# NVlabs/InstantSplat

Measured on AMD Instinct MI355X. Metric: train_iters_per_sec, higher is better.
Workload: dtype f32

## Files before the change

### include/mi355gs.h

```cpp
#ifndef MI355GS_H
#define MI355GS_H

#include <stddef.h>
#include <stdint.h>

#ifdef __cplusplus
extern "C" {
#endif

#define MI355GS_ABI_VERSION 10

#define MI355GS_OK 0
#define MI355GS_EINVAL (-1)
#define MI355GS_ELAUNCH (-2)
#define MI355GS_EOVERFLOW (-3)

int mi355gs_abi_version(void);
const char* mi355gs_error_string(int code);

size_t mi355gs_raster_geom_bytes(int P);
size_t mi355gs_raster_tiles_bytes(int W, int H);
size_t mi355gs_raster_binning_bytes(int64_t num_instances, int W, int H);

int mi355gs_raster_forward_preprocess(
    void* stream, int P, int D, int M, int W, int H,
    const float* means3D, const float* shs, const float* shs_rest, const float* colors_precomp, const float* opacities,
    const float* scales, float scale_modifier, const float* rotations, const float* cov3D_precomp,
    const float* viewmatrix, const float* projmatrix, const float* campos,
    float tanfovx, float tanfovy, int prefiltered,
    int32_t* radii, void* geom, void* tiles, int32_t* num_rendered, uint8_t* visible, void* grad_scratch, int debug);

int mi355gs_raster_forward_render(
    void* stream, int P, int W, int H, int64_t capacity, const float* bg,
    const void* geom, void* tiles, void* binning, float* out_color, int debug);

size_t mi355gs_raster_binning_bytes_render_only(int64_t num_instances, int W, int H);
int mi355gs_raster_forward_render_only(
    void* stream, int P, int W, int H, int64_t capacity, const float* bg,
    const void* geom, void* tiles, void* binning, float* out_color, int debug);

size_t mi355gs_raster_grad_scratch_bytes(int P);
size_t mi355gs_raster_grad_gate_offset(int P);
int mi355gs_raster_backward(
    void* stream, int P, int D, int M, int W, int H, const float* bg,
    const float* means3D, const float* shs, const float* shs_rest, const float* colors_precomp, const float* opacities,
    const float* scales, float scale_modifier, const float* rotations, const float* cov3D_precomp,
    const float* viewmatrix, const float* projmatrix, const float* campos,
    float tanfovx, float tanfovy,
    const void* geom, void* tiles, const void* binning, int64_t capacity, const int32_t* radii,
    const float* out_color, const float* dL_dpix, void* grad_scratch,
    float* dL_dmeans3D, float* dL_dmeans2D, float* dL_dshs, float* dL_dshs_rest, float* dL_dcolors, float* dL_dopacities,
    float* dL_dscales, float* dL_drotations, float* dL_dcov3D, int grad_scratch_is_clear, int debug);

int mi355gs_raster_mark_visible(void* stream, int P, const float* means3D, const float* viewmatrix,
                                const float* projmatrix, uint8_t* present);

int mi355gs_raster_frame_stats(void* stream, int W, int H, const void* tiles, int64_t* stats);

int mi355gs_tune_min_units(int min_units);

int mi355gs_tune_deterministic(int on);

int mi355gs_tune_scale_grad(int mode);

int mi355gs_profile_begin(void);
int mi355gs_profile_set_period(int every);
int mi355gs_profile_work_counters(void* counters);
int mi355gs_profile_read(int kind, double* total_ms, int* launches);
int mi355gs_profile_end(void);
int mi355gs_profile_ranges(int on);

size_t mi355gs_ssim_scratch_bytes(int B, int C, int H, int W);
int mi355gs_ssim_forward(void* stream, int B, int C, int H, int W, const float* img1, const float* img2,
                         float* dm_dmu1, float* dm_dsigma1_sq, float* dm_dsigma12,
                         void* scratch, float* ssim_mean, float* l1_mean, int padding_valid);
int mi355gs_ssim_backward(void* stream, int B, int C, int H, int W, const float* img1, const float* img2,
                          const float* dm_dmu1, const float* dm_dsigma1_sq, const float* dm_dsigma12,
                          const float* ssim_grad_scale, const float* l1_grad_scale, float* dL_dimg1, int padding_valid);
int mi355gs_l1_ssim_loss_fused(void* stream, int B, int C, int H, int W, const float* img1, const float* img2, void* scratch,
                               float lambda_dssim, float* ssim_mean, float* l1_mean, float* loss, float* dloss_dimg1);

size_t mi355gs_l1_scratch_bytes(int64_t n);
int mi355gs_l1_loss_forward(void* stream, int64_t n, const float* a, const float* b, void* scratch, float* mean_out);
int mi355gs_l1_loss_backward(void* stream, int64_t n, const float* a, const float* b, const float* grad_scale, float* d_a);
#define MI355GS_LOSS_PROGRAM_MAX 16
#define MI355GS_LOSS_OP_L1 0
#define MI355GS_LOSS_OP_SSIM 1
#define MI355GS_LOSS_OP_MULK 2
#define MI355GS_LOSS_OP_ADDK 3
#define MI355GS_LOSS_OP_RSUBK 4
#define MI355GS_LOSS_OP_DIVK 5
#define MI355GS_LOSS_OP_NEG 6
#define MI355GS_LOSS_OP_ADD 7
#define MI355GS_LOSS_OP_SUB 8
int mi355gs_l1_ssim_pair_forward(void* stream, int B, int C, int H, int W, const float* img1, const float* img2, void* scratch,
                                 float* dssim_dimg1);
int mi355gs_l1_ssim_pair_backward(void* stream, int64_t n, const float* img1, const float* img2, const float* dssim_dimg1,
                                  const float* g_l1, float c_l1, const float* g_ssim, float c_ssim, float* d_img1);
int mi355gs_loss_program_eval(void* stream, int n_ops, const int32_t* ops, const float* consts, int B, int C, int H, int W,
                              const void* scratch, float* ssim_mean, float* l1_mean, float* out, float* host_out, float ticket);
int mi355gs_loss_program_eval_grad(void* stream, int n_ops, const int32_t* ops, const float* consts, int B, int C, int H, int W,
                                   const void* scratch, float* ssim_mean, float* l1_mean, float* out, float* host_out, float ticket,
                                   const float* img1, const float* img2, const float* dssim_dimg1, float c_l1, float c_ssim, float* d_img1);

size_t mi355gs_knn_scratch_bytes(int N);
int mi355gs_knn_dist2(void* stream, int N, const float* points, float* mean_dist2, void* scratch);

int mi355gs_adam_step(void* stream, int64_t n, int row, float* param, const float* grad, float* exp_avg,
                      float* exp_avg_sq, const float* per_point_lr, const float* grad_sumsq,
                      float lr, float beta1, float beta2, float eps, int step);

int mi355gs_adam_multi_step(void* stream, int ntensors, const int64_t* numel, const int32_t* row, float* const* params,
                            const float* const* grads, float* const* exp_avg, float* const* exp_avg_sq,
                            const float* const* per_point_lr, const float* lr, float beta1, float beta2, float eps,
                            const int32_t* step, float* scratch, const float* gate, const int32_t* gate_index,
                            uint32_t* live, uint32_t seq);

int mi355gs_pose_forward(void* stream, int P, const float* xyz, const float* rot, const float* scaling,
                         const float* opacity_logit, const float* pose, float* means_cam, float* rot_cam, float* scales,
                         float* opac);
int mi355gs_pose_backward(void* stream, int P, const float* xyz, const float* rot, const float* scales, const float* opac,
                          const float* pose, const float* g_means, const float* g_rot, const float* g_scales,
                          const float* g_opac, float* d_xyz, float* d_rot, float* d_scaling, float* d_opacity_logit,
                          float* d_pose, float* scratch);

int mi355gs_posed_forward_preprocess(void* stream, int P, int D, int W, int H, const float* xyz, const float* f_dc,
                                     const float* f_rest, const float* opacity_logit, const float* log_scales, float scale_modifier,
                                     const float* rotation, const float* pose, const float* view_identity, const float* projmatrix,
                                     const float* origin, float tanfovx, float tanfovy, int32_t* radii, void* geom, void* tiles,
                                     int32_t* num_rendered, uint8_t* visible, void* grad_scratch, int debug);
int mi355gs_posed_backward(void* stream, int P, int D, int W, int H, const float* bg, const float* xyz, const float* f_dc,
                           const float* f_rest, const float* opacity_logit, const float* log_scales, float scale_modifier,
                           const float* rotation, const float* pose, const float* view_identity, const float* projmatrix,
                           const float* origin, float tanfovx, float tanfovy, const void* geom, void* tiles, const void* binning,
                           int64_t capacity, const int32_t* radii, const float* out_color, const float* dL_dpix,
                           void* grad_scratch, float* pose_scratch, float* d_xyz, float* d_means2D, float* d_f_dc, float* d_f_rest,
                           float* d_opacity_logit, float* d_log_scales, float* d_rotation, float* d_pose, int pose_rows, int pose_row,
                           int grad_scratch_is_clear, int debug);

size_t mi355gs_trainer_workspace_bytes(int P, int W, int H, int V, int64_t capacity);
void* mi355gs_trainer_create(int P, int W, int H, int V, int64_t capacity, float* xyz, float* f_dc, float* f_rest, float* opacity,
                             float* scaling, float* rotation, float* poses, float* const* exp_avg, float* const* exp_avg_sq,
                             const float* per_point_lr, void* workspace);
int mi355gs_trainer_step(void* trainer, void* stream, int view, int sh_degree, const float* gt_image, const float* projmatrix,
                         float tanfovx, float tanfovy, const float* bg, const float* lr, const int32_t* step, float beta1, float beta2, float eps,
                         float lambda_dssim, int do_optimizer_step, float* loss_out, int32_t* num_rendered_out);
int mi355gs_trainer_optimizer_step(void* trainer, void* stream, const float* lr, const int32_t* step, float beta1, float beta2,
                                   float eps, int commit_gate);
void mi355gs_trainer_destroy(void* trainer);
const float* mi355gs_trainer_grad(void* trainer, int k);

#define MI355GS_TRACKER_STATE_FLOATS 40
#define MI355GS_TRACKER_POSE 0
#define MI355GS_TRACKER_EXP_AVG 8
#define MI355GS_TRACKER_EXP_AVG_SQ 16
#define MI355GS_TRACKER_BEST 24
#define MI355GS_TRACKER_INITIAL 25
#define MI355GS_TRACKER_FLAG 26
#define MI355GS_TRACKER_COUNT 27
#define MI355GS_TRACKER_CAND 32
size_t mi355gs_tracker_workspace_bytes(int P, int W, int H, int64_t capacity);
void* mi355gs_tracker_create(int P, int M, int W, int H, int64_t capacity, const float* xyz, const float* f_dc, const float* f_rest,
                             const float* opacity, const float* scaling, const float* rotation, void* workspace);
int mi355gs_tracker_count(void* tracker, void* stream, int sh_degree, const float* projmatrix, float tanfovx, float tanfovy,
                          const float* pose, int32_t* count_out);
int mi355gs_tracker_run(void* tracker, void* stream, int sh_degree, const float* gt_image, const float* projmatrix, float tanfovx,
                        float tanfovy, const float* bg, const float* sched, int num_iter, int first_iter, int n_iters, float* state,
                        float* pose_trace, float* loss_trace, float* grad_trace);
void mi355gs_tracker_destroy(void* tracker);

int mi355gs_rgb8_from_planar(void* stream, int H, int W, const float* img, uint8_t* out);
size_t mi355gs_path_workspace_bytes(int P, int W, int H, int64_t capacity);
void* mi355gs_path_create(int P, int M, int W, int H, int64_t capacity, const float* xyz, const float* f_dc, const float* f_rest,
                          const float* opacity, const float* scaling, const float* rotation, void* workspace);
int mi355gs_path_render(void* path, void* stream, int sh_degree, const float* projmatrix, float tanfovx, float tanfovy,
                        const float* bg, const float* poses, int first, int n, uint8_t* frames, int32_t* counts);
void mi355gs_path_destroy(void* path);

size_t mi355gs_metrics_rgb8_scratch_bytes(int N, int H, int W);
int mi355gs_metrics_rgb8(void* stream, int N, int H, int W, const uint8_t* a, const uint8_t* b, void* scratch, int64_t* sq_sum,
                         float* ssim_mean);

size_t mi355gs_lpips_vgg_scratch_bytes(int N, int H, int W, const int channels[5]);
int mi355gs_lpips_vgg_rgb8(void* stream, int N, int H, int W, const uint8_t* a, const uint8_t* b, const int channels[5],
                           const float* weights, void* scratch, float* lpips, float* taps);

typedef struct mi355gs_vit_config {
  int enc_dim, enc_depth, enc_heads;
  int dec_dim, dec_depth, dec_heads;
  int patch;
  int hooks[4];
} mi355gs_vit_config;
size_t mi355gs_vit_encode_scratch_bytes(const mi355gs_vit_config* cfg, int Ht, int Wt, int V);
int mi355gs_vit_encode(void* stream, const mi355gs_vit_config* cfg, const float* weights, const float* rope, int Ht, int Wt, int V,
                       const float* images, void* scratch, float* feat);
size_t mi355gs_vit_decode_scratch_bytes(const mi355gs_vit_config* cfg, int Ht, int Wt, int E);
int mi355gs_vit_decode(void* stream, const mi355gs_vit_config* cfg, const float* weights, const float* rope, int Ht, int Wt, int V, int E,
                       const int32_t* edges, const float* feat, void* scratch, float* const out1[4], float* const out2[4]);

typedef struct mi355gs_dpt_config {
  int dim_tokens[4];
  int layer_dims[4];
  int feature_dim, last_dim;
  int mlp_hidden, local_feat_dim, two_confs;
  float conf_vmin, conf_vmax;
  float desc_conf_vmin, desc_conf_vmax;
} mi355gs_dpt_config;
size_t mi355gs_dpt_head_scratch_bytes(const mi355gs_dpt_config* cfg, int Ht, int Wt, int E);
size_t mi355gs_dpt_head_tap_offset(const mi355gs_dpt_config* cfg, int Ht, int Wt, int E, int which);
int mi355gs_dpt_head(void* stream, const mi355gs_dpt_config* cfg, const float* weights, int Ht, int Wt, int E, const float* const hooks[4],
                     void* scratch, float* pts3d, float* conf, float* raw4);
size_t mi355gs_local_features_scratch_bytes(const mi355gs_dpt_config* cfg, int Ht, int Wt, int E);
int mi355gs_local_features(void* stream, const mi355gs_dpt_config* cfg, const float* weights, int Ht, int Wt, int E, const float* hook0,
                           const float* hook3, void* scratch, float* desc, float* desc_conf);

size_t mi355gs_png_rgb8_scratch_bytes(int N, int H, int W, int rows_per_block);
size_t mi355gs_png_rgb8_stream_bytes(int N, int H, int W, int rows_per_block);
int mi355gs_png_rgb8(void* stream, int N, int H, int W, int rows_per_block, const uint8_t* frames, void* scratch, uint8_t* out,
                     int64_t* offsets);

size_t mi355gs_jpeg_rgb8_scratch_bytes(int N, int H, int W, int subsampling);
size_t mi355gs_jpeg_rgb8_stream_bytes(int N, int H, int W, int subsampling);
int mi355gs_jpeg_rgb8(void* stream, int N, int H, int W, int subsampling, const uint8_t* qtables, const uint8_t* frames, void* scratch,
                      uint8_t* out, size_t out_bytes, int64_t* offsets);

size_t mi355gs_pointmap_stats_scratch_bytes(int V, int H, int W);
int mi355gs_pointmap_stats(void* stream, int V, int H, int W, const float* depthmaps, const float* confidences, uint8_t* overlap,
                           void* scratch, double* stats);
int mi355gs_covis_masks(void* stream, int V, int H, int W, const int32_t* order, const float* pointmaps, const float* depthmaps,
                        const float* intrinsics, const float* w2c, const double* stats, float depth_threshold, uint8_t* overlap);
size_t mi355gs_compact_scratch_bytes(int64_t n);
int mi355gs_compact_pointmaps(void* stream, int64_t n, const uint8_t* overlap, const float* pointmaps, const float* images,
                              const float* confidences, void* scratch, float* out_points, uint8_t* out_rgb8, float* out_confidence,
                              int32_t* count_dev, int32_t* count_host);

#define MI355GS_ALIGN_OPT_DEPTH 1
#define MI355GS_ALIGN_OPT_IM_POSES 2
#define MI355GS_ALIGN_OPT_FOCALS 4
#define MI355GS_ALIGN_OPT_PW_POSES 8
#define MI355GS_ALIGN_NORM_PW_SCALE 16
size_t mi355gs_align_workspace_bytes(int V, int H, int W, int E, int flags);
void* mi355gs_align_create(void* workspace, int V, int H, int W, const int32_t* edges, int E, int flags, float base_scale);
void mi355gs_align_destroy(void* handle);
int mi355gs_align_pack(void* handle, void* stream, const float* pred_i, const float* pred_j, const float* conf_i, const float* conf_j);
int mi355gs_align_grad(void* handle, void* stream, const float* depth_log, const float* im_pose, const float* focal_log, const float* pp_raw,
                       const float* pw_pose, float* g_depth_log, float* g_im_pose, float* g_focal_log, float* g_pw_pose, float* loss);
int mi355gs_align_run(void* handle, void* stream, int niter, const float* step_table, float* depth_log, float* im_pose, float* focal_log,
                      const float* pp_raw, float* pw_pose, float* m_depth_log, float* v_depth_log, float* m_im_pose, float* v_im_pose,
                      float* m_focal_log, float* v_focal_log, float* m_pw_pose, float* v_pw_pose, float* losses);
int mi355gs_align_points(void* handle, void* stream, const float* depth_log, const float* im_pose, const float* focal_log,
                         const float* pp_raw, const float* pw_pose, float* pts3d, float* depth);
const float* mi355gs_align_records(void* handle);

size_t mi355gs_align_init_workspace_bytes(int B, int n);
int mi355gs_align_init_means(void* workspace, void* stream, int rows, int n, const float* x, float* means);
int mi355gs_align_init_register(void* workspace, void* stream, int B, int n, const float* src, const int32_t* src_idx, long long src_job_stride,
                                int src_pt_stride, const float* tgt, const int32_t* tgt_idx, long long tgt_job_stride, const float* weights,
                                const int32_t* w_idx, long long w_job_stride, float* srt, float* pw_pose);
int mi355gs_align_init_apply(void* stream, int n, const float* src, int src_pt_stride, const float* srt, float* dst);
int mi355gs_align_init_focals(void* workspace, void* stream, int B, int H, int W, const float* src, const int32_t* src_idx,
                              long long src_job_stride, int src_pt_stride, float* focals);
int mi355gs_align_init_state(void* workspace, void* stream, int V, int E, int H, int W, int norm_pw_scale, float base_scale, int focal_mode,
                             float known_focal, const float* srt, const int32_t* pose_row, const float* focals, const int32_t* focal_row,
                             const float* pw_pose, float* pts3d, float* depth_log, float* im_pose, float* focal_log);

#define MI355GS_DENSITY_CLONE 1
#define MI355GS_DENSITY_SPLIT 2
#define MI355GS_DENSITY_PRUNE 4
#define MI355GS_DENSITY_SCREEN 8
#define MI355GS_DENSITY_XYZ 0
#define MI355GS_DENSITY_F_DC 1
#define MI355GS_DENSITY_F_REST 2
#define MI355GS_DENSITY_OPACITY 3
#define MI355GS_DENSITY_SCALING 4
#define MI355GS_DENSITY_ROTATION 5
#define MI355GS_DENSITY_EXP_AVG 6
#define MI355GS_DENSITY_EXP_AVG_SQ 12
#define MI355GS_DENSITY_PER_POINT_LR 18
#define MI355GS_DENSITY_GRAD_ACCUM 19
#define MI355GS_DENSITY_DENOM 20
#define MI355GS_DENSITY_MAX_RADII 21
#define MI355GS_DENSITY_TENSORS 22
int mi355gs_density_stats(void* stream, int P, const float* grad, int grad_stride, const uint8_t* filter, const int32_t* radii,
                          float* grad_accum, float* denom, float* max_radii);
size_t mi355gs_density_scratch_bytes(int P, int N);
int mi355gs_density_plan(void* stream, int P, int N, int flags, const float* grad_accum, const float* denom, const float* grads,
                         int64_t n_grads, const uint8_t* mask, const float* max_radii, const float* scaling, const float* opacity,
                         float max_grad, float dense_limit, float min_opacity, float max_screen_size, float world_limit,
                         float child_div, uint32_t* code, void* scratch, int32_t* totals_host);
int mi355gs_density_apply(void* stream, int P, int N, int flags, int rest_width, const uint32_t* code, const void* scratch,
                          const float* noise, int64_t noise_rows, int64_t n_selected, float child_div, const void* const* in,
                          void* const* out, int64_t out_rows);
int mi355gs_reset_opacity(void* stream, int P, float* opacity, float* exp_avg, float* exp_avg_sq);

size_t mi355gs_resample_rgb8_scratch_bytes(int N, int rows, int w);
int mi355gs_resample_rgb8(void* stream, int N, int H, int W, int Hout, int Wout, const uint8_t* images, const int32_t* kx,
                          const int32_t* bx, int ksize_x, const int32_t* ky, const int32_t* by, int ksize_y, int x0, int y0, int w,
                          int h, int row0, int rows, void* scratch, uint8_t* rgb8, float* unit, float* normalized);

#ifdef __cplusplus
}
#endif
#endif
```

### instantsplat_amd/_lib.py

```python
from __future__ import annotations

import ctypes
import os
from ctypes import c_float, c_int, c_int64, c_size_t, c_void_p

import torch

_HERE = os.path.dirname(os.path.abspath(__file__))
LIB_PATH = os.path.join(_HERE, "lib", "libmi355gs.so")
_LIB = None
_TEST_MODE = False

_P = c_void_p
_SIGNATURES = {
    "mi355gs_abi_version": (c_int, []),
    "mi355gs_error_string": (ctypes.c_char_p, [c_int]),
    "mi355gs_raster_geom_bytes": (c_size_t, [c_int]),
    "mi355gs_raster_tiles_bytes": (c_size_t, [c_int, c_int]),
    "mi355gs_raster_binning_bytes": (c_size_t, [c_int64, c_int, c_int]),
    "mi355gs_raster_grad_scratch_bytes": (c_size_t, [c_int]),
    "mi355gs_raster_grad_gate_offset": (c_size_t, [c_int]),
    "mi355gs_raster_forward_preprocess": (c_int, [_P, c_int, c_int, c_int, c_int, c_int, _P, _P, _P, _P, _P, _P, c_float, _P, _P,
                                                  _P, _P, _P, c_float, c_float, c_int, _P, _P, _P, _P, _P, _P, c_int]),
    "mi355gs_raster_forward_render": (c_int, [_P, c_int, c_int, c_int, c_int64, _P, _P, _P, _P, _P, c_int]),
    "mi355gs_raster_binning_bytes_render_only": (c_size_t, [c_int64, c_int, c_int]),
    "mi355gs_raster_forward_render_only": (c_int, [_P, c_int, c_int, c_int, c_int64, _P, _P, _P, _P, _P, c_int]),
    "mi355gs_raster_backward": (c_int, [_P, c_int, c_int, c_int, c_int, c_int, _P, _P, _P, _P, _P, _P, _P, c_float, _P, _P, _P, _P,
                                        _P, c_float, c_float, _P, _P, _P, c_int64, _P, _P, _P, _P, _P, _P, _P, _P, _P, _P, _P, _P, _P,
                                        c_int, c_int]),
    "mi355gs_raster_mark_visible": (c_int, [_P, c_int, _P, _P, _P, _P]),
    "mi355gs_raster_frame_stats": (c_int, [_P, c_int, c_int, _P, _P]),
    "mi355gs_tune_min_units": (c_int, [c_int]),
    "mi355gs_tune_scale_grad": (c_int, [c_int]),
    "mi355gs_tune_deterministic": (c_int, [c_int]),
    "mi355gs_profile_begin": (c_int, []),
    "mi355gs_profile_set_period": (c_int, [c_int]),
    "mi355gs_profile_work_counters": (c_int, [_P]),
    "mi355gs_profile_read": (c_int, [c_int, ctypes.POINTER(ctypes.c_double), ctypes.POINTER(c_int)]),
    "mi355gs_profile_end": (c_int, []),
    "mi355gs_profile_ranges": (c_int, [c_int]),
    "mi355gs_ssim_scratch_bytes": (c_size_t, [c_int, c_int, c_int, c_int]),
    "mi355gs_ssim_forward": (c_int, [_P, c_int, c_int, c_int, c_int, _P, _P, _P, _P, _P, _P, _P, _P, c_int]),
    "mi355gs_ssim_backward": (c_int, [_P, c_int, c_int, c_int, c_int, _P, _P, _P, _P, _P, _P, _P, _P, c_int]),
    "mi355gs_l1_ssim_loss_fused": (c_int, [_P, c_int, c_int, c_int, c_int, _P, _P, _P, c_float, _P, _P, _P, _P]),
    "mi355gs_l1_ssim_pair_forward": (c_int, [_P, c_int, c_int, c_int, c_int, _P, _P, _P, _P]),
    "mi355gs_l1_ssim_pair_backward": (c_int, [_P, c_int64, _P, _P, _P, _P, c_float, _P, c_float, _P]),
    "mi355gs_loss_program_eval": (c_int, [_P, c_int, _P, _P, c_int, c_int, c_int, c_int, _P, _P, _P, _P, _P, c_float]),
    "mi355gs_loss_program_eval_grad": (c_int, [_P, c_int, _P, _P, c_int, c_int, c_int, c_int, _P, _P, _P, _P, _P, c_float, _P, _P, _P, c_float,
                                               c_float, _P]),
    "mi355gs_knn_scratch_bytes": (c_size_t, [c_int]),
    "mi355gs_knn_dist2": (c_int, [_P, c_int, _P, _P, _P]),
    "mi355gs_adam_step": (c_int, [_P, c_int64, c_int, _P, _P, _P, _P, _P, _P, c_float, c_float, c_float, c_float, c_int]),
    "mi355gs_adam_multi_step": (c_int, [_P, c_int, _P, _P, _P, _P, _P, _P, _P, _P, c_float, c_float, c_float, _P, _P, _P, _P, _P,
                                        ctypes.c_uint32]),
    "mi355gs_pose_forward": (c_int, [_P, c_int, _P, _P, _P, _P, _P, _P, _P, _P, _P]),
    "mi355gs_pose_backward": (c_int, [_P, c_int, _P, _P, _P, _P, _P, _P, _P, _P, _P, _P, _P, _P, _P, _P, _P]),
    "mi355gs_posed_forward_preprocess": (c_int, [_P, c_int, c_int, c_int, c_int, _P, _P, _P, _P, _P, c_float, _P, _P, _P, _P, _P,
                                                 c_float, c_float, _P, _P, _P, _P, _P, _P, c_int]),
    "mi355gs_posed_backward": (c_int, [_P, c_int, c_int, c_int, c_int, _P, _P, _P, _P, _P, _P, c_float, _P, _P, _P, _P, _P, c_float,
                                       c_float, _P, _P, _P, c_int64, _P, _P, _P, _P, _P, _P, _P, _P, _P, _P, _P, _P, _P, c_int, c_int, c_int, c_int]),
    "mi355gs_l1_scratch_bytes": (c_size_t, [c_int64]),
    "mi355gs_l1_loss_forward": (c_int, [_P, c_int64, _P, _P, _P, _P]),
    "mi355gs_l1_loss_backward": (c_int, [_P, c_int64, _P, _P, _P, _P]),
    "mi355gs_trainer_workspace_bytes": (c_size_t, [c_int, c_int, c_int, c_int, c_int64]),
    "mi355gs_trainer_create": (c_void_p, [c_int, c_int, c_int, c_int, c_int64, _P, _P, _P, _P, _P, _P, _P, _P, _P, _P, _P]),
    "mi355gs_trainer_step": (c_int, [_P, _P, c_int, c_int, _P, _P, c_float, c_float, _P, _P, _P, c_float, c_float, c_float, c_float,
                                     c_int, _P, _P]),
    "mi355gs_trainer_optimizer_step": (c_int, [_P, _P, _P, _P, c_float, c_float, c_float, c_int]),
    "mi355gs_trainer_destroy": (None, [_P]),
    "mi355gs_trainer_grad": (_P, [_P, c_int]),
    "mi355gs_tracker_workspace_bytes": (c_size_t, [c_int, c_int, c_int, c_int64]),
    "mi355gs_tracker_create": (c_void_p, [c_int, c_int, c_int, c_int, c_int64, _P, _P, _P, _P, _P, _P, _P]),
    "mi355gs_tracker_count": (c_int, [_P, _P, c_int, _P, c_float, c_float, _P, _P]),
    "mi355gs_tracker_run": (c_int, [_P, _P, c_int, _P, _P, c_float, c_float, _P, _P, c_int, c_int, c_int, _P, _P, _P, _P]),
    "mi355gs_tracker_destroy": (None, [_P]),
    "mi355gs_rgb8_from_planar": (c_int, [_P, c_int, c_int, _P, _P]),
    "mi355gs_path_workspace_bytes": (c_size_t, [c_int, c_int, c_int, c_int64]),
    "mi355gs_path_create": (c_void_p, [c_int, c_int, c_int, c_int, c_int64, _P, _P, _P, _P, _P, _P, _P]),
    "mi355gs_path_render": (c_int, [_P, _P, c_int, _P, c_float, c_float, _P, _P, c_int, c_int, _P, _P]),
    "mi355gs_path_destroy": (None, [_P]),
    "mi355gs_metrics_rgb8_scratch_bytes": (c_size_t, [c_int, c_int, c_int]),
    "mi355gs_metrics_rgb8": (c_int, [_P, c_int, c_int, c_int, _P, _P, _P, _P, _P]),
    "mi355gs_png_rgb8_scratch_bytes": (c_size_t, [c_int, c_int, c_int, c_int]),
    "mi355gs_png_rgb8_stream_bytes": (c_size_t, [c_int, c_int, c_int, c_int]),
    "mi355gs_png_rgb8": (c_int, [_P, c_int, c_int, c_int, c_int, _P, _P, _P, _P]),
    "mi355gs_jpeg_rgb8_scratch_bytes": (c_size_t, [c_int, c_int, c_int, c_int]),
    "mi355gs_jpeg_rgb8_stream_bytes": (c_size_t, [c_int, c_int, c_int, c_int]),
    "mi355gs_jpeg_rgb8": (c_int, [_P, c_int, c_int, c_int, c_int, _P, _P, _P, _P, c_size_t, _P]),
    "mi355gs_lpips_vgg_scratch_bytes": (c_size_t, [c_int, c_int, c_int, _P]),
    "mi355gs_lpips_vgg_rgb8": (c_int, [_P, c_int, c_int, c_int, _P, _P, _P, _P, _P, _P, _P]),
    "mi355gs_vit_encode_scratch_bytes": (c_size_t, [_P, c_int, c_int, c_int]),
    "mi355gs_vit_encode": (c_int, [_P, _P, _P, _P, c_int, c_int, c_int, _P, _P, _P]),
    "mi355gs_vit_decode_scratch_bytes": (c_size_t, [_P, c_int, c_int, c_int]),
    "mi355gs_vit_decode": (c_int, [_P, _P, _P, _P, c_int, c_int, c_int, c_int, _P, _P, _P, _P, _P]),
    "mi355gs_dpt_head_scratch_bytes": (c_size_t, [_P, c_int, c_int, c_int]),
    "mi355gs_dpt_head_tap_offset": (c_size_t, [_P, c_int, c_int, c_int, c_int]),
    "mi355gs_dpt_head": (c_int, [_P, _P, _P, c_int, c_int, c_int, _P, _P, _P, _P, _P]),
    "mi355gs_local_features_scratch_bytes": (c_size_t, [_P, c_int, c_int, c_int]),
    "mi355gs_local_features": (c_int, [_P, _P, _P, c_int, c_int, c_int, _P, _P, _P, _P, _P]),
    "mi355gs_pointmap_stats_scratch_bytes": (c_size_t, [c_int, c_int, c_int]),
    "mi355gs_pointmap_stats": (c_int, [_P, c_int, c_int, c_int, _P, _P, _P, _P, _P]),
    "mi355gs_covis_masks": (c_int, [_P, c_int, c_int, c_int, _P, _P, _P, _P, _P, _P, c_float, _P]),
    "mi355gs_compact_scratch_bytes": (c_size_t, [c_int64]),
    "mi355gs_compact_pointmaps": (c_int, [_P, c_int64, _P, _P, _P, _P, _P, _P, _P, _P, _P, _P]),
    "mi355gs_align_workspace_bytes": (c_size_t, [c_int, c_int, c_int, c_int, c_int]),
    "mi355gs_align_create": (c_void_p, [_P, c_int, c_int, c_int, _P, c_int, c_int, c_float]),
    "mi355gs_align_destroy": (None, [_P]),
    "mi355gs_align_pack": (c_int, [_P, _P, _P, _P, _P, _P]),
    "mi355gs_align_grad": (c_int, [_P] * 12),
    "mi355gs_align_run": (c_int, [_P, _P, c_int] + [_P] * 15),
    "mi355gs_align_points": (c_int, [_P] * 9),
    "mi355gs_align_records": (c_void_p, [_P]),
    "mi355gs_align_init_workspace_bytes": (c_size_t, [c_int, c_int]),
    "mi355gs_align_init_means": (c_int, [_P, _P, c_int, c_int, _P, _P]),
    "mi355gs_align_init_register": (c_int, [_P, _P, c_int, c_int, _P, _P, c_int64, c_int, _P, _P, c_int64, _P, _P, c_int64, _P, _P]),
    "mi355gs_align_init_apply": (c_int, [_P, c_int, _P, c_int, _P, _P]),
    "mi355gs_align_init_focals": (c_int, [_P, _P, c_int, c_int, c_int, _P, _P, c_int64, c_int, _P]),
    "mi355gs_align_init_state": (c_int, [_P, _P, c_int, c_int, c_int, c_int, c_int, c_float, c_int, c_float] + [_P] * 9),
    "mi355gs_density_stats": (c_int, [_P, c_int, _P, c_int, _P, _P, _P, _P, _P]),
    "mi355gs_density_scratch_bytes": (c_size_t, [c_int, c_int]),
    "mi355gs_density_plan": (c_int, [_P, c_int, c_int, c_int, _P, _P, _P, c_int64, _P, _P, _P, _P, c_float, c_float, c_float, c_float,
                                     c_float, c_float, _P, _P, _P]),
    "mi355gs_density_apply": (c_int, [_P, c_int, c_int, c_int, c_int, _P, _P, _P, c_int64, c_int64, c_float, _P, _P, c_int64]),
    "mi355gs_reset_opacity": (c_int, [_P, c_int, _P, _P, _P]),
    "mi355gs_resample_rgb8_scratch_bytes": (c_size_t, [c_int, c_int, c_int]),
    "mi355gs_resample_rgb8": (c_int, [_P, c_int, c_int, c_int, c_int, c_int, _P, _P, _P, c_int, _P, _P, c_int, c_int, c_int, c_int, c_int,
                                      c_int, c_int, _P, _P, _P, _P]),
}
EXPORTED_SYMBOLS = tuple(_SIGNATURES)


ABI_VERSION = 10


def _bind(path: str):
    lib = ctypes.CDLL(path)
    for name, (res, args) in _SIGNATURES.items():
        fn = getattr(lib, name)
        fn.restype, fn.argtypes = res, args
    got = lib.mi355gs_abi_version()
    if got != ABI_VERSION:
        raise RuntimeError(f"{path} implements ABI v{got}, this package binds v{ABI_VERSION}: rebuild it with "
                           "`python -c 'import __graft_entry__ as g; g.build()'`")
    return lib


def lib():
    global _LIB
    if _LIB is None:
        if not os.path.exists(LIB_PATH):
            raise RuntimeError(
                f"{LIB_PATH} is missing: build it with `python -c 'import __graft_entry__ as g; g.build()'` "
                "(hipcc --offload-arch=gfx950). instantsplat_amd has no CPU or PyTorch fallback.")
        _LIB = _bind(LIB_PATH)
        if os.environ.get("MI355GS_DETERMINISTIC", "0") == "1":
            _LIB.mi355gs_tune_deterministic(1)
    return _LIB


def _use_library_for_testing(path: str | None):
    global _LIB, _TEST_MODE, _EXT_BOUND_TO
    if path is None:
        _LIB, _TEST_MODE = None, False
    else:
        _LIB, _TEST_MODE = _bind(path), True
    _EXT_BOUND_TO = None


BINDING = os.environ.get("MI355GS_BINDING", "compiled")
EXT_PATH = os.path.join(_HERE, "lib", "_mi355gs_torch.so")
_EXT = None
_EXT_BOUND_TO = None


def compiled():
    global _EXT, _EXT_BOUND_TO
    if BINDING != "compiled":
        return None
    L = lib()
    if _EXT_BOUND_TO is L:
        return _EXT
    if _EXT is None:
        if not os.path.exists(EXT_PATH):
            raise RuntimeError(f"{EXT_PATH} is missing: build it with `python -c 'import __graft_entry__ as g; g.build()'` "
                               "(or set MI355GS_BINDING=ctypes to use the Python binding)")
        import importlib.util
        spec = importlib.util.spec_from_file_location("_mi355gs_torch", EXT_PATH)
        _EXT = importlib.util.module_from_spec(spec)
        spec.loader.exec_module(_EXT)
    _EXT.forget_gates()
    _EXT.bind({name: ctypes.cast(getattr(L, name), ctypes.c_void_p).value for name in _EXT.abi_symbols()}, _TEST_MODE)
    _EXT_BOUND_TO = L
    return _EXT


def check(code: int, what: str):
    if code != 0:
        raise RuntimeError(f"mi355gs: {what} failed: {lib().mi355gs_error_string(code).decode()} ({code})")


def ptr(t: torch.Tensor | None):
    return None if t is None else t.data_ptr()


STREAM = object()


def call(dev, name: str, *args):
    fn = getattr(lib(), "mi355gs_" + name)
    with on_device(dev):
        check(fn(*[stream_ptr(dev) if a is STREAM else a.data_ptr() if isinstance(a, torch.Tensor) else a for a in args]), name)


def scratch(dev, name: str, *sizes, what: str | None):
    nbytes = int(getattr(lib(), "mi355gs_" + name)(*sizes))
    if not nbytes and what is not None:
        raise ValueError(what)
    return torch.empty(max(nbytes, 1), dtype=torch.uint8, device=dev)


def gpu_only(who: str = "instantsplat_amd operators run") -> str:
    return f"{who} on the GPU only (got a CPU tensor; there is no CPU fallback)"


_F32 = torch.float32


def f32c_on_one_device(*tensors):
    out, dev = [], None
    for t in tensors:
        if t.dtype is not _F32:
            raise RuntimeError(f"expected float32, got {t.dtype}")
        if not t.is_contiguous():
            t = t.contiguous()
        d = t.device
        if dev is None:
            if d.type != "cuda" and not _TEST_MODE:
                raise RuntimeError(gpu_only())
            dev = d
        elif d != dev:
            raise RuntimeError(f"tensors on different devices: {dev} vs {d}")
        out.append(t)
    return out, dev


def require_device(*tensors: torch.Tensor | None):
    dev = None
    for t in tensors:
        if t is None:
            continue
        if not t.is_cuda and not _TEST_MODE:
            raise RuntimeError(gpu_only())
        if not t.is_contiguous():
            raise RuntimeError("instantsplat_amd operators need contiguous tensors")
        if dev is None:
            dev = t.device
        elif t.device != dev:
            raise RuntimeError(f"tensors on different devices: {dev} vs {t.device}")
    return dev


class _NoGuard:
    def __enter__(self):
        return None

    def __exit__(self, *a):
        return False


_NO_GUARD = _NoGuard()


def on_device(device):
    if device is not None and device.type == "cuda" and device.index is not None and device.index != torch.cuda.current_device():
        return torch.cuda.device(device)
    return _NO_GUARD


def stream_ptr(device):
    if device is not None and device.type == "cuda":
        return torch.cuda.current_stream(device).cuda_stream
    return None


def f32c(t: torch.Tensor | None):
    if t is None:
        return None
    if t.dtype != torch.float32:
        raise RuntimeError(f"expected float32, got {t.dtype}")
    return t.contiguous()
```

### instantsplat_amd/csrc/api.hip

```cpp
#include <stdio.h>
#include "common.h"
#include <dlfcn.h>
#include <cstdlib>

int gs_launch_preprocess_fwd(hipStream_t, int, int, int, const float*, const float*, const float*, const float*, const float*, const float*,
                             const float*, const float*, const CamParams&, int32_t*, GsRec*, float*, uint2*, uint8_t*, float*, uint8_t*,
                             const GsPosed&, const GsPrologue&);
int gs_launch_count_tiles(hipStream_t, int, int, int, const uint2*, uint32_t*, uint32_t*, uint32_t*);
int gs_launch_preprocess_bwd(hipStream_t, int, int, int, const float*, const float*, const float*, const float*, const float*, int, int,
                             const CamParams&, const int32_t*, const GsRec*, const float*, const uint8_t*, const GsGrad*, float*, float*,
                             float*, float*, float*, float*, float*, float*, float*, const GsPosed&, float*, bool);
int gs_launch_mark_visible(hipStream_t, int, const float*, const float*, uint8_t*);
int gs_launch_scan_tiles(hipStream_t, int, const uint32_t*, uint32_t*, int32_t*, uint32_t*, uint32_t*, uint32_t*, uint32_t*, int);
int gs_launch_binning(hipStream_t, int, int, int, const float*, const uint2*, const uint32_t*, uint32_t*, uint64_t*, uint32_t*, uint32_t,
                      const uint32_t*, const uint32_t*, const uint32_t*);
int gs_launch_composite_fwd(hipStream_t, int, int, int, int, uint32_t, const uint32_t*, const uint32_t*, const GsRec*, const float*,
                            float*, float*, uint32_t*, const uint32_t*, const uint32_t*, const uint32_t*, uint4*, float4*, uint32_t,
                            const uint32_t*, unsigned long long*, uint32_t, uint32_t*, unsigned long long*, bool);
int gs_launch_composite_bwd(hipStream_t, int, int, int, uint32_t, const uint32_t*, const uint32_t*, const GsRec*, const float*,
                            const float*, const uint32_t*, const float*, GsGrad*, const float*, const uint4*,
                            const float4*, const uint32_t*, uint32_t, bool, const unsigned long long*, uint32_t, const uint32_t*,
                            unsigned long long*, const uint32_t*, float*);
int gs_launch_det_prepare(hipStream_t, int, int, int, uint32_t, const uint32_t*, const uint32_t*, const uint2*, char*, uint32_t*, float*);
int gs_launch_det_gather(hipStream_t, int, uint32_t, const char*, const float*, GsGrad*);
int gs_launch_frame_stats(hipStream_t, int, int, int, int, const uint32_t*, const uint32_t*, int64_t*);

namespace {
constexpr int PROF_KINDS = 6, PROF_MAX = 8192;
struct ProfState {
  bool on = false;
  unsigned long long* work_counters = nullptr;
  hipEvent_t ev[PROF_KINDS][PROF_MAX][2];
  int created[PROF_KINDS] = {};
  int used[PROF_KINDS] = {};
  int period = 1;
  int seen[PROF_KINDS] = {};
} g_prof;
}

GsProfScope::GsProfScope(int kind, hipStream_t stream) : s(stream) {
  if (!g_prof.on || kind < 0 || kind >= PROF_KINDS || g_prof.used[kind] >= PROF_MAX) return;
  if (g_prof.seen[kind]++ % g_prof.period != 0) return;
  const int i = g_prof.used[kind];
  if (i >= g_prof.created[kind]) {
    if (hipEventCreate(&g_prof.ev[kind][i][0]) != hipSuccess || hipEventCreate(&g_prof.ev[kind][i][1]) != hipSuccess) return;
    g_prof.created[kind] = i + 1;
  }
  (void)hipEventRecord(g_prof.ev[kind][i][0], s);
  stop = g_prof.ev[kind][i][1];
  g_prof.used[kind] = i + 1;
  active = true;
}
GsProfScope::~GsProfScope() { if (active) (void)hipEventRecord(stop, s); }
typedef GsProfScope ProfScope;

bool g_ranges_on = false;
thread_local bool g_krange_open = false;
namespace {
struct Roctx {
  int (*push)(const char*) = nullptr;
  int (*pop)() = nullptr;
  bool tried = false;
  unsigned long long pushed = 0;
} g_roctx;
bool roctx_open() {
  if (!g_roctx.tried) {
    g_roctx.tried = true;
    for (const char* name : {"librocprofiler-sdk-roctx.so", "librocprofiler-sdk-roctx.so.1", "libroctx64.so", "libroctx64.so.4"}) {
      void* h = dlopen(name, RTLD_NOW | RTLD_GLOBAL);
      if (!h) continue;
      g_roctx.push = (int (*)(const char*))dlsym(h, "roctxRangePushA");
      g_roctx.pop = (int (*)())dlsym(h, "roctxRangePop");
      if (g_roctx.push && g_roctx.pop) break;
      g_roctx.push = nullptr; g_roctx.pop = nullptr;
    }
  }
  return g_roctx.push != nullptr;
}
struct RoctxEnv {
  RoctxEnv() { const char* e = getenv("MI355GS_ROCTX"); if (e && e[0] == '1' && roctx_open()) g_ranges_on = true; }
} g_roctx_env;
}
void gs_range_push(const char* name) { ++g_roctx.pushed; (void)g_roctx.push(name); }
void gs_range_pop() { (void)g_roctx.pop(); }

void gs_log_error(const char* where, const char* what) { fprintf(stderr, "[mi355gs] %s failed: %s\n", where, what); }

static int g_scale_grad_exact = 0;
static int g_deterministic = 0;
GsKnobs gs_knobs() { return GsKnobs{gs_min_units(), g_deterministic}; }

static CamParams make_cam(const float* view, const float* proj, const float* campos, float tanfovx, float tanfovy,
                          float scale_modifier, int W, int H) {
  CamParams cp;
  cp.view = view; cp.proj = proj; cp.campos = campos;
  cp.tanfovx = tanfovx; cp.tanfovy = tanfovy;
  cp.focal_x = W / (2.0f * tanfovx); cp.focal_y = H / (2.0f * tanfovy);
  cp.scale_modifier = scale_modifier;
  cp.scale_grad_factor = g_scale_grad_exact ? scale_modifier : 1.0f;
  cp.W = W; cp.H = H;
  cp.gx = (W + GS_TILE - 1) / GS_TILE; cp.gy = (H + GS_TILE - 1) / GS_TILE;
  return cp;
}

static inline uint32_t clamp_capacity(int64_t c) { return c <= 0 ? 0u : (c > 0x7fffffffLL ? 0x7fffffffu : (uint32_t)c); }

namespace {
__global__ void k_view_consts(float* consts) {
  const int i = threadIdx.x;
  if (i < 16) consts[i] = (i % 5 == 0) ? 1.f : 0.f;
  else if (i < 19) consts[i] = 0.f;
}
}
int gs_write_view_consts(hipStream_t stream, float* consts, const char* name) {
  const int debug = 0;
  GS_KRANGE(name);
  hipLaunchKernelGGL(k_view_consts, dim3(1), dim3(64), 0, stream, consts);
  GS_CHECK_LAUNCH(name);
  return MI355GS_OK;
}


int gs_frame_project(hipStream_t stream, const GsScene& sc, const GsView& vw, const GsFrameBufs& fb, const GsFrameCtx& cx,
                     int32_t* num_rendered, uint8_t* visible, int debug) {
  GsRange range("mi355gs_raster_forward_preprocess");
  const int P = sc.P, D = sc.D, M = sc.M, W = vw.W, H = vw.H;
  if (P < 0 || W <= 0 || H <= 0 || W > 65535 * GS_TILE || H > 65535 * GS_TILE || D < 0 || D > 3) return MI355GS_EINVAL;
  if (!fb.geom || !fb.tiles || !num_rendered || !vw.view || !vw.proj || !vw.campos) return MI355GS_EINVAL;
  if (P > 0 && (!sc.means3D || !sc.opacities || !fb.radii)) return MI355GS_EINVAL;
  if (P > 0 && ((sc.shs == nullptr) == (sc.colors_precomp == nullptr))) return MI355GS_EINVAL;
  if (P > 0 && sc.shs && M < (D + 1) * (D + 1)) return MI355GS_EINVAL;
  if (sc.shs_rest && (!sc.shs || M < 2)) return MI355GS_EINVAL;
  if (P > 0 && !sc.cov3D_precomp && (!sc.scales || !sc.rotations)) return MI355GS_EINVAL;
  const GeomLayout gl(P);
  const TilesLayout tl(W, H);
  char* g = (char*)fb.geom;
  char* t = (char*)fb.tiles;
  GsPrologue pro;
  if (cx.prologue) {
    pro = *cx.prologue;
  } else {
    pro.tile_counters = (uint32_t*)(t + tl.count); pro.n_counters = (int)((tl.start - tl.count) / 4);
    if (fb.grad_scratch) { pro.grad_records = (float4*)fb.grad_scratch; pro.n_vec = gs_grad_gate_offset(P) / 16 + 2; }
    if (P <= 0) {
      if (hipMemsetAsync(t + tl.count, 0, tl.start - tl.count, stream) != hipSuccess) return MI355GS_ELAUNCH;
      if (fb.grad_scratch && hipMemsetAsync(fb.grad_scratch, 0, gs_grad_gate_offset(P) + 32, stream) != hipSuccess) return MI355GS_ELAUNCH;
    }
  }
  const CamParams cp = make_cam(vw.view, vw.proj, vw.campos, vw.tanfovx, vw.tanfovy, sc.scale_modifier, W, H);
  GS_KRANGE("preprocess_fwd");
  gs_launch_preprocess_fwd(stream, P, D, M, sc.means3D, sc.shs, sc.shs_rest, sc.colors_precomp, sc.opacities, sc.scales, sc.rotations,
                           sc.cov3D_precomp, cp, fb.radii, (GsRec*)(g + gl.rec), (float*)(g + gl.cov3D), (uint2*)(g + gl.rect),
                           (uint8_t*)(g + gl.clamped), (float*)(g + gl.depth), visible, cx.posed, pro);
  GS_CHECK_LAUNCH("preprocess_fwd");
  GS_KRANGE("count_tiles");
  gs_launch_count_tiles(stream, P, tl.T, tl.gx, (const uint2*)(g + gl.rect), (uint32_t*)(t + tl.count), (uint32_t*)(g + gl.bin_entries),
                        (uint32_t*)(g + gl.bin_n));
  GS_CHECK_LAUNCH("count_tiles");
  GS_KRANGE("scan_tiles");
  gs_launch_scan_tiles(stream, tl.T, (const uint32_t*)(t + tl.count), (uint32_t*)(t + tl.start), num_rendered,
                       (uint32_t*)(t + tl.order), (uint32_t*)(t + tl.meta), (uint32_t*)(t + tl.seg_first), (uint32_t*)(t + tl.part_first),
                       fb.knobs.min_units);
  GS_CHECK_LAUNCH("scan_tiles");
  return MI355GS_OK;
}

int gs_frame_render(hipStream_t stream, int P, const GsView& vw, const GsFrameBufs& fb, const float* bg, float* out_color, bool train,
                    int debug) {
  GsRange range(train ? "mi355gs_raster_forward_render" : "mi355gs_raster_forward_render_only");
  const int W = vw.W, H = vw.H;
  if (P < 0 || W <= 0 || H <= 0 || !fb.geom || !fb.tiles || !bg || !out_color) return MI355GS_EINVAL;
  const uint32_t cap = clamp_capacity(fb.capacity);
  if (cap > 0 && !fb.binning) return MI355GS_EINVAL;
  const GeomLayout gl(P);
  const TilesLayout tl(W, H);
  const BinningLayout bl(fb.capacity, tl.T, fb.knobs);
  const char* g = (const char*)fb.geom;
  char* t = (char*)fb.tiles;
  char* b = (char*)fb.binning;
  GS_KRANGE("binning");
  gs_launch_binning(stream, P, tl.T, tl.gx, (const float*)(g + gl.depth), (const uint2*)(g + gl.rect),
                    (const uint32_t*)(t + tl.start), (uint32_t*)(t + tl.cursor), (uint64_t*)(b + bl.keys),
                    (uint32_t*)(b + bl.list), cap, (const uint32_t*)(t + tl.order), (const uint32_t*)(g + gl.bin_entries),
                    (const uint32_t*)(g + gl.bin_n));
  GS_CHECK_LAUNCH("binning");
  {
    ProfScope prof(train ? 0 : 2, stream);
    GS_KRANGE("composite_fwd");
    gs_launch_composite_fwd(stream, tl.T, tl.gx, W, H, cap, (const uint32_t*)(t + tl.start), (const uint32_t*)(b + bl.list),
                            (const GsRec*)(g + gl.rec), bg, out_color, (float*)(t + tl.final_T), (uint32_t*)(t + tl.n_contrib),
                            (const uint32_t*)(t + tl.order), (const uint32_t*)(t + tl.seg_first), (const uint32_t*)(t + tl.part_first),
                            train ? (uint4*)(b + bl.unit_tile) : nullptr, train ? (float4*)(b + bl.bstate) : nullptr, bl.max_units,
                            (const uint32_t*)(t + tl.meta), train ? (unsigned long long*)(b + bl.hitmask) : nullptr, bl.max_chunks,
                            (uint32_t*)(t + tl.qmax), train ? g_prof.work_counters : nullptr, train);
  }
  GS_CHECK_LAUNCH("composite_fwd");
  return MI355GS_OK;
}

int gs_frame_backward(hipStream_t stream, const GsScene& sc, const GsView& vw, const GsFrameBufs& fb, const GsFrameCtx& cx,
                      const float* bg, const float* out_color, const float* dL_dpix, const GsGradOut& o, bool grad_scratch_is_clear,
                      int debug) {
  GsRange range("mi355gs_raster_backward");
  const int P = sc.P, D = sc.D, W = vw.W, H = vw.H;
  if (P < 0 || W <= 0 || H <= 0 || D < 0 || D > 3) return MI355GS_EINVAL;
  if (!fb.geom || !fb.tiles || !dL_dpix || !out_color || !fb.grad_scratch || !bg || !vw.view || !vw.proj || !vw.campos) return MI355GS_EINVAL;
  const bool outs = !(cx.pose_only && cx.posed.pose);
  if (P > 0 && (!sc.means3D || !fb.radii || (outs && (!o.means3D || !o.means2D || !o.opacities)))) return MI355GS_EINVAL;
  const int use_shs = sc.shs != nullptr, use_cov = sc.cov3D_precomp != nullptr;
  if (P > 0 && outs && use_shs && !o.shs) return MI355GS_EINVAL;
  if (sc.shs_rest && !use_shs) return MI355GS_EINVAL;
  if (P > 0 && outs && !use_shs && !o.colors) return MI355GS_EINVAL;
  if (P > 0 && !use_cov && (!sc.scales || !sc.rotations || (outs && (!o.scales || !o.rotations)))) return MI355GS_EINVAL;
  if (P > 0 && outs && use_cov && !o.cov3D) return MI355GS_EINVAL;
  if (P == 0) return MI355GS_OK;
  const uint32_t cap = clamp_capacity(fb.capacity);
  if (cap > 0 && !fb.binning) return MI355GS_EINVAL;
  const GeomLayout gl(P);
  const TilesLayout tl(W, H);
  const BinningLayout bl(fb.capacity, tl.T, fb.knobs);
  const char* g = (const char*)fb.geom;
  const char* t = (const char*)fb.tiles;
  char* b = (char*)fb.binning;
  GsGrad* grads = (GsGrad*)fb.grad_scratch;
  const size_t clear_bytes = cx.gate_tail ? gs_grad_gate_offset(P) + 8 * sizeof(float) : (size_t)P * sizeof(GsGrad);
  if (!cx.prologue && !grad_scratch_is_clear && hipMemsetAsync(grads, 0, clear_bytes, stream) != hipSuccess) return MI355GS_ELAUNCH;
  if (cap > 0) {
    const bool det = fb.knobs.det != 0;
    char* det_scratch = (char*)fb.grad_scratch + gs_grad_gate_offset(P) + 256;
    uint32_t* rowidx = det ? (uint32_t*)(b + bl.det_rowidx) : nullptr;
    float* rows = det ? (float*)(b + bl.det_rows) : nullptr;
    if (det) {
      GS_KRANGE("det_prepare");
      const int rc = gs_launch_det_prepare(stream, P, tl.T, tl.gx, cap, (const uint32_t*)(t + tl.start), (const uint32_t*)(b + bl.list),
                                           (const uint2*)(g + gl.rect), det_scratch, rowidx, rows);
      GS_CHECK_LAUNCH("det_prepare");
      if (rc != 0) return MI355GS_ELAUNCH;
    }
    {
      ProfScope prof(1, stream);
      GS_KRANGE("composite_bwd");
      gs_launch_composite_bwd(stream, tl.gx, W, H, cap, (const uint32_t*)(t + tl.start), (const uint32_t*)(b + bl.list),
                              (const GsRec*)(g + gl.rec), bg, (const float*)(t + tl.final_T), (const uint32_t*)(t + tl.n_contrib),
                              dL_dpix, grads, out_color, (const uint4*)(b + bl.unit_tile),
                              (const float4*)(b + bl.bstate), (const uint32_t*)(t + tl.meta), bl.max_units, bl.may_loop,
                              (const unsigned long long*)(b + bl.hitmask), bl.max_chunks, (const uint32_t*)(t + tl.qmax),
                              det ? nullptr : g_prof.work_counters, rowidx, rows);
    }
    GS_CHECK_LAUNCH("composite_bwd");
    if (det) {
      GS_KRANGE("det_gather");
      gs_launch_det_gather(stream, P, cap, det_scratch, rows, grads);
      GS_CHECK_LAUNCH("det_gather");
    }
  }
  const CamParams cp = make_cam(vw.view, vw.proj, vw.campos, vw.tanfovx, vw.tanfovy, sc.scale_modifier, W, H);
  GS_KRANGE("preprocess_bwd");
  gs_launch_preprocess_bwd(stream, P, D, sc.M, sc.means3D, sc.shs, sc.shs_rest, sc.scales, sc.rotations, use_shs, use_cov, cp, fb.radii,
                           (const GsRec*)(g + gl.rec), (const float*)(g + gl.cov3D), (const uint8_t*)(g + gl.clamped), grads, o.means3D,
                           o.means2D, o.shs, o.shs_rest, o.colors, o.opacities, o.scales, o.rotations, o.cov3D, cx.posed, cx.gate,
                           cx.pose_only);
  GS_CHECK_LAUNCH("preprocess_bwd");
  return MI355GS_OK;
}

extern "C" {

int mi355gs_abi_version(void) { return MI355GS_ABI_VERSION; }

const char* mi355gs_error_string(int code) {
  switch (code) {
    case MI355GS_OK: return "ok";
    case MI355GS_EINVAL: return "invalid argument";
    case MI355GS_ELAUNCH: return "HIP launch or runtime failure";
    case MI355GS_EOVERFLOW: return "instance capacity exceeded";
    default: return "unknown error";
  }
}

size_t mi355gs_raster_geom_bytes(int P) { return GeomLayout(P).total; }
size_t mi355gs_raster_tiles_bytes(int W, int H) { return (W > 0 && H > 0) ? TilesLayout(W, H).total : 0; }
size_t mi355gs_raster_binning_bytes(int64_t n, int W, int H) { return (W > 0 && H > 0) ? gs_binning_bytes(n, W, H, gs_knobs(), true) : 0; }
size_t mi355gs_raster_binning_bytes_render_only(int64_t n, int W, int H) { return (W > 0 && H > 0) ? gs_binning_bytes(n, W, H, gs_knobs(), false) : 0; }
size_t mi355gs_raster_grad_gate_offset(int P) { return gs_grad_gate_offset(P); }
size_t mi355gs_raster_grad_scratch_bytes(int P) { return gs_grad_scratch_bytes(P, g_deterministic); }

int mi355gs_raster_forward_preprocess(void* stream, int P, int D, int M, int W, int H, const float* means3D, const float* shs,
                                      const float* shs_rest, const float* colors_precomp, const float* opacities, const float* scales,
                                      float scale_modifier, const float* rotations, const float* cov3D_precomp,
                                      const float* viewmatrix, const float* projmatrix, const float* campos, float tanfovx,
                                      float tanfovy, int prefiltered, int32_t* radii, void* geom, void* tiles,
                                      int32_t* num_rendered, uint8_t* visible, void* grad_scratch, int debug) {
  (void)prefiltered;
  return gs_frame_project((hipStream_t)stream, {P, D, M, means3D, shs, shs_rest, colors_precomp, opacities, scales, rotations, cov3D_precomp, scale_modifier},
                          {W, H, viewmatrix, projmatrix, campos, tanfovx, tanfovy}, {geom, tiles, nullptr, 0, radii, grad_scratch, gs_knobs()},
                          GsFrameCtx(), num_rendered, visible, debug);
}

int mi355gs_raster_forward_render(void* stream, int P, int W, int H, int64_t capacity, const float* bg, const void* geom,
                                  void* tiles, void* binning, float* out_color, int debug) {
  return gs_frame_render((hipStream_t)stream, P, {W, H}, {const_cast<void*>(geom), tiles, binning, capacity, nullptr, nullptr, gs_knobs()}, bg,
                         out_color, true, debug);
}

int mi355gs_raster_forward_render_only(void* stream, int P, int W, int H, int64_t capacity, const float* bg, const void* geom,
                                       void* tiles, void* binning, float* out_color, int debug) {
  return gs_frame_render((hipStream_t)stream, P, {W, H}, {const_cast<void*>(geom), tiles, binning, capacity, nullptr, nullptr, gs_knobs()}, bg,
                         out_color, false, debug);
}

int mi355gs_raster_backward(void* stream, int P, int D, int M, int W, int H, const float* bg, const float* means3D,
                            const float* shs, const float* shs_rest, const float* colors_precomp, const float* opacities, const float* scales,
                            float scale_modifier, const float* rotations, const float* cov3D_precomp, const float* viewmatrix,
                            const float* projmatrix, const float* campos, float tanfovx, float tanfovy, const void* geom,
                            void* tiles, const void* binning, int64_t capacity, const int32_t* radii, const float* out_color,
                            const float* dL_dpix, void* grad_scratch, float* dL_dmeans3D, float* dL_dmeans2D, float* dL_dshs,
                            float* dL_dshs_rest, float* dL_dcolors, float* dL_dopacities, float* dL_dscales, float* dL_drotations, float* dL_dcov3D,
                            int grad_scratch_is_clear, int debug) {
  const GsGradOut o = {dL_dmeans3D, dL_dmeans2D, dL_dshs, dL_dshs_rest, dL_dcolors, dL_dopacities, dL_dscales, dL_drotations, dL_dcov3D};
  return gs_frame_backward((hipStream_t)stream, {P, D, M, means3D, shs, shs_rest, colors_precomp, opacities, scales, rotations, cov3D_precomp, scale_modifier},
                           {W, H, viewmatrix, projmatrix, campos, tanfovx, tanfovy},
                           {const_cast<void*>(geom), tiles, const_cast<void*>(binning), capacity, const_cast<int32_t*>(radii), grad_scratch, gs_knobs()},
                           GsFrameCtx(), bg, out_color, dL_dpix, o, grad_scratch_is_clear != 0, debug);
}

int mi355gs_tune_deterministic(int on) {
  const int old = g_deterministic;
  if (on >= 0) g_deterministic = on ? 1 : 0;
  return old;
}

int mi355gs_tune_scale_grad(int mode) {
  const int old = g_scale_grad_exact;
  if (mode >= 0) g_scale_grad_exact = mode ? 1 : 0;
  return old;
}

int mi355gs_raster_frame_stats(void* stream_, int W, int H, const void* tiles, int64_t* stats) {
  GS_RANGE();
  hipStream_t stream = (hipStream_t)stream_;
  const int debug = 0;
  if (W <= 0 || H <= 0 || !tiles || !stats) return MI355GS_EINVAL;
  const TilesLayout tl(W, H);
  const char* t = (const char*)tiles;
  if (hipMemsetAsync(stats, 0, 2 * sizeof(int64_t), stream) != hipSuccess) return MI355GS_ELAUNCH;
  GS_KRANGE("frame_stats");
  gs_launch_frame_stats(stream, tl.T, tl.gx, W, H, (const uint32_t*)(t + tl.start), (const uint32_t*)(t + tl.n_contrib), stats);
  GS_CHECK_LAUNCH("frame_stats");
  return MI355GS_OK;
}

int mi355gs_profile_begin(void) {
  g_prof.on = true;
  for (int k = 0; k < PROF_KINDS; ++k) g_prof.used[k] = g_prof.seen[k] = 0;
  return MI355GS_OK;
}

int mi355gs_profile_set_period(int every) {
  const int old = g_prof.period;
  if (every > 0) g_prof.period = every;
  return old;
}

int mi355gs_profile_work_counters(void* counters) {
  g_prof.work_counters = (unsigned long long*)counters;
  return MI355GS_OK;
}

int mi355gs_profile_read(int kind, double* total_ms, int* launches) {
  if (kind < 0 || kind >= PROF_KINDS || !total_ms || !launches) return MI355GS_EINVAL;
  double tot = 0.0;
  for (int i = 0; i < g_prof.used[kind]; ++i) {
    float ms = 0.f;
    if (hipEventSynchronize(g_prof.ev[kind][i][1]) != hipSuccess) return MI355GS_ELAUNCH;
    if (hipEventElapsedTime(&ms, g_prof.ev[kind][i][0], g_prof.ev[kind][i][1]) != hipSuccess) return MI355GS_ELAUNCH;
    tot += ms;
  }
  *total_ms = tot;
  *launches = g_prof.used[kind];
  return MI355GS_OK;
}

int mi355gs_profile_end(void) {
  g_prof.on = false;
  return MI355GS_OK;
}

int mi355gs_profile_ranges(int on) {
  if (on == 1) {
    if (!roctx_open()) return MI355GS_EINVAL;
    g_ranges_on = true;
  } else if (on == 0) {
    g_ranges_on = false;
  }
  return (int)(g_roctx.pushed & 0x7fffffffull);
}

int mi355gs_raster_mark_visible(void* stream_, int P, const float* means3D, const float* viewmatrix, const float* projmatrix,
                                uint8_t* present) {
  GS_RANGE();
  (void)projmatrix;
  const int debug = 0;
  void* stream = stream_;
  if (P < 0 || (P > 0 && (!means3D || !viewmatrix || !present))) return MI355GS_EINVAL;
  GS_KRANGE("mark_visible");
  gs_launch_mark_visible((hipStream_t)stream, P, means3D, viewmatrix, present);
  GS_CHECK_LAUNCH("mark_visible");
  return MI355GS_OK;
}

}
```

### instantsplat_amd/csrc/binning.hip

```cpp
#include "common.h"

namespace {

constexpr int SCAN_THREADS = 1024;
constexpr size_t SCAN_STAGE_MAX_BYTES = 48 * 1024;
constexpr int SORT_THREADS = 256;
constexpr int SORT_SMALL_CAP = GS_SORT_SMALL_CAP;
constexpr int SORT_LDS_CAP = 8192;

#ifdef GS_SCAN_PROBE
__device__ long long g_scan_probe[16];
#define SCAN_STAMP(k) do { if (threadIdx.x == 0) g_scan_probe[k] = wall_clock64(); } while (0)
#else
#define SCAN_STAMP(k) do { } while (0)
#endif
constexpr int SCAN_PER_MAX = (int)(SCAN_STAGE_MAX_BYTES / (SCAN_THREADS * 4));

template <bool STAGED>
__global__ __launch_bounds__(SCAN_THREADS) void k_scan_tiles(int T, const uint32_t* count, uint32_t* start, int32_t* num_rendered,
                                                               uint32_t* __restrict__ order, uint32_t* __restrict__ meta,
                                                               uint32_t* __restrict__ seg_first, uint32_t* __restrict__ part_first,
                                                               uint32_t min_units) {
  __shared__ uint32_t wave_tot[SCAN_THREADS / GS_WAVE];
  HIP_DYNAMIC_SHARED(uint32_t, s_stage)
  const int tid = threadIdx.x, lane = tid & 63, wave = tid >> 6;
  const int per = (T + SCAN_THREADS - 1) / SCAN_THREADS;
  const int lo = tid * per, hi = min(T, lo + per);
  SCAN_STAMP(0);
  uint32_t own[STAGED ? SCAN_PER_MAX : 1];
  if constexpr (STAGED) {
    for (int e = tid; e < T; e += SCAN_THREADS) s_stage[e] = count[e];
    __syncthreads();
#pragma unroll
    for (int k = 0; k < SCAN_PER_MAX; ++k) own[k] = lo + k < hi ? s_stage[lo + k] : 0u;
  }
  auto for_own = [&](auto&& f) {
    if constexpr (STAGED) {
#pragma unroll
      for (int k = 0; k < SCAN_PER_MAX; ++k)
        if (lo + k < hi) f(lo + k, own[k]);
    } else {
      for (int i = lo; i < hi; ++i) f(i, count[i]);
    }
  };
  auto emit = [&](uint32_t* out, auto&& value) {
    if constexpr (STAGED) {
      __syncthreads();
      for_own([&](int i, uint32_t c) { s_stage[i] = value(i, c); });
      __syncthreads();
      for (int e = tid; e < T; e += SCAN_THREADS) out[e] = s_stage[e];
    } else {
      for_own([&](int i, uint32_t c) { out[i] = value(i, c); });
    }
  };
  SCAN_STAMP(1);
  uint32_t local = 0;
  for_own([&](int, uint32_t c) { local += c; });
  const uint32_t incl = gs_wave_scan_incl_u32(local);
  if (lane == 63) wave_tot[wave] = incl;
  __syncthreads();
  uint32_t wave_off = 0, total = 0;
#pragma unroll
  for (int w = 0; w < SCAN_THREADS / GS_WAVE; ++w) {
    const uint32_t v = wave_tot[w];
    if (w < wave) wave_off += v;
    total += v;
  }
  SCAN_STAMP(2);
  if (order) {
    __shared__ uint32_t hist[SCAN_THREADS];
    __shared__ uint32_t s_max;
    uint32_t mx = 0;
    for_own([&](int, uint32_t c) { mx = max(mx, c); });
    mx = gs_wave_max_u32(mx);
    hist[tid] = 0u;
    if (tid == 0) s_max = 0u;
    __syncthreads();
    if (lane == 0) atomicMax(&s_max, mx);
    __syncthreads();
    const uint32_t cmax = max(s_max, 1u);
    const float bscale = (float)(SCAN_THREADS - 1) / (float)cmax;
    auto bucket = [&](uint32_t c) { return (uint32_t)(SCAN_THREADS - 1) - min((uint32_t)(SCAN_THREADS - 1), (uint32_t)((float)c * bscale)); };
    SCAN_STAMP(3);
    for_own([&](int, uint32_t c) { atomicAdd(&hist[bucket(c)], 1u); });
    __syncthreads();
    SCAN_STAMP(4);
    const uint32_t h = hist[tid];
    const uint32_t hi_ = gs_wave_scan_incl_u32(h);
    __shared__ uint32_t hist_wave[SCAN_THREADS / GS_WAVE];
    if (lane == 63) hist_wave[wave] = hi_;
    __syncthreads();
    uint32_t hoff = 0;
#pragma unroll
    for (int w = 0; w < SCAN_THREADS / GS_WAVE; ++w)
      if (w < wave) hoff += hist_wave[w];
    hist[tid] = hoff + hi_ - h;
    __syncthreads();
    SCAN_STAMP(5);
    if constexpr (STAGED) {
      for_own([&](int i, uint32_t c) { s_stage[atomicAdd(&hist[bucket(c)], 1u)] = (uint32_t)i; });
      __syncthreads();
      for (int e = tid; e < T; e += SCAN_THREADS) order[e] = s_stage[e];
    } else {
      for_own([&](int i, uint32_t c) { order[atomicAdd(&hist[bucket(c)], 1u)] = (uint32_t)i; });
    }
    __syncthreads();
    SCAN_STAMP(6);
  }
  if (seg_first) {
    const uint32_t level = (uint32_t)gs_unit_level_for((long long)total, (long long)min_units);
    const uint32_t chunks = 1u << level;
    const uint32_t seg_len = chunks * GS_SEG;
    static_assert((GS_SEG & (GS_SEG - 1)) == 0, "GS_SEG must be a power of two");
    const uint32_t seg_shift = level + (uint32_t)__builtin_ctz(GS_SEG), seg_mask = seg_len - 1u;
    auto units_of = [&](uint32_t c) { return (c + seg_mask) >> seg_shift; };
    auto short_of = [&](uint32_t c) { return (uint32_t)((c & seg_mask) != 0u); };
    uint32_t lseg = 0, lpart = 0;
    for_own([&](int, uint32_t c) { lseg += units_of(c); lpart += short_of(c); });
    const uint32_t iseg = gs_wave_scan_incl_u32(lseg), ipart = gs_wave_scan_incl_u32(lpart);
    __shared__ uint32_t seg_wave[SCAN_THREADS / GS_WAVE];
    __shared__ uint32_t part_wave[SCAN_THREADS / GS_WAVE];
    if (lane == 63) { seg_wave[wave] = iseg; part_wave[wave] = ipart; }
    __syncthreads();
    uint32_t soff = 0, stot = 0, poff = 0, ptot = 0;
#pragma unroll
    for (int w = 0; w < SCAN_THREADS / GS_WAVE; ++w) {
      if (w < wave) { soff += seg_wave[w]; poff += part_wave[w]; }
      stot += seg_wave[w]; ptot += part_wave[w];
    }
    uint32_t srun = soff + iseg - lseg, prun = poff + ipart - lpart;
    emit(seg_first, [&](int, uint32_t c) { const uint32_t v = srun; srun += units_of(c); return v; });
    emit(part_first, [&](int, uint32_t c) { const uint32_t v = prun; prun += short_of(c); return v; });
    if (tid == 0) { part_first[T] = ptot; meta[3] = ptot; }
    if (tid == 0) { seg_first[T] = stot; meta[1] = stot; meta[2] = chunks; }
  }
  SCAN_STAMP(7);
  uint32_t run = wave_off + incl - local;
  emit(start, [&](int, uint32_t c) { const uint32_t v = run; run += c; return v; });
  if (tid == 0) {
    start[T] = total;
    *num_rendered = (int32_t)total;
  }
  SCAN_STAMP(8);
}

constexpr int SCAN_CHUNK = 4096;

template <bool RECT>
__device__ __forceinline__ uint32_t scan_input(const uint32_t* __restrict__ in, int i, int n) {
  if (i >= n) return 0u;
  if constexpr (!RECT) return in[i];
  else {
    if (i == n - 1) return 0u;
    const uint2 r = reinterpret_cast<const uint2*>(in)[i];
    const int x0 = r.x & 0xffff, y0 = r.x >> 16, x1 = r.y & 0xffff, y1 = r.y >> 16;
    return (x1 > x0 && y1 > y0) ? (uint32_t)((x1 - x0) * (y1 - y0)) : 0u;
  }
}

template <bool RECT>
__global__ __launch_bounds__(256) void k_scan_block_sums(int n, const uint32_t* __restrict__ in, uint32_t* __restrict__ sums) {
  __shared__ uint32_t s_red[4];
  const int base = blockIdx.x * SCAN_CHUNK;
  uint32_t acc = 0;
  for (int i = threadIdx.x; i < SCAN_CHUNK; i += 256) acc += scan_input<RECT>(in, base + i, n);
#pragma unroll
  for (int m = 32; m >= 1; m >>= 1) acc += __shfl_xor(acc, m);
  if ((threadIdx.x & 63) == 0) s_red[threadIdx.x >> 6] = acc;
  __syncthreads();
  if (threadIdx.x == 0) sums[blockIdx.x] = s_red[0] + s_red[1] + s_red[2] + s_red[3];
}

template <bool RECT>
__global__ __launch_bounds__(256) void k_scan_apply(int n, const uint32_t* __restrict__ in, const uint32_t* __restrict__ block_off,
                                                    uint32_t* __restrict__ out) {
  __shared__ uint32_t s_wave[4];
  const int tid = threadIdx.x, lane = tid & 63, wave = tid >> 6;
  uint32_t run = block_off[blockIdx.x];
  for (int it = 0; it < SCAN_CHUNK / 256; ++it) {
    const int i = blockIdx.x * SCAN_CHUNK + it * 256 + tid;
    const uint32_t v = scan_input<RECT>(in, i, n);
    const uint32_t incl = gs_wave_scan_incl_u32(v);
    __syncthreads();
    if (lane == 63) s_wave[wave] = incl;
    __syncthreads();
    uint32_t woff = 0;
#pragma unroll
    for (int w = 0; w < 4; ++w) woff += w < wave ? s_wave[w] : 0u;
    if (i < n) out[i] = run + woff + incl - v;
    run += s_wave[0] + s_wave[1] + s_wave[2] + s_wave[3];
  }
}

constexpr int BIN_CHUNK = GS_BIN_CHUNK;
static_assert(BIN_CHUNK == 512, "two Gaussians per thread (own_depth selection in k_scatter_lds)");
constexpr int BIN_MAX_LDS_TILES = 16384;
static_assert(BIN_MAX_LDS_TILES <= 64 * 256, "k_count_tiles_lds keeps one bit per bin of a thread in a 64-bit mask");

__device__ __forceinline__ bool unpack_rect(uint2 r, int& x0, int& y0, int& x1, int& y1) {
  x0 = r.x & 0xffff; y0 = r.x >> 16; x1 = r.y & 0xffff; y1 = r.y >> 16;
  return x1 > x0 && y1 > y0;
}

constexpr int BIN_WIDE = 8;

constexpr int BIN_PER_THREAD = BIN_CHUNK / 256;

template <class F>
__device__ __forceinline__ void for_each_instance(int lo, int hi, const uint2 (&own)[BIN_PER_THREAD], const uint2* __restrict__ rects,
                                                  uint32_t* s_wide, uint2* s_wide_rect, uint32_t* s_nwide, F&& f) {
  const int tid = threadIdx.x;
#pragma unroll
  for (int j = 0; j < BIN_PER_THREAD; ++j) {
    const int i = lo + tid + 256 * j;
    int x0, y0, x1, y1;
    if (i >= hi || !unpack_rect(own[j], x0, y0, x1, y1)) continue;
    if ((x1 - x0) * (y1 - y0) > BIN_WIDE) {
      const uint32_t slot = atomicAdd(s_nwide, 1u);
      s_wide[slot] = (uint32_t)i; s_wide_rect[slot] = own[j];
      continue;
    }
    for (int y = y0; y < y1; ++y)
      for (int x = x0; x < x1; ++x) f(i, j, x, y);
  }
  __syncthreads();
  const int nwide = (int)*s_nwide;
  for (int q = tid >> 4; q < nwide; q += 16) {
    const int i = (int)s_wide[q];
    int x0, y0, x1, y1;
    unpack_rect(s_wide_rect[q], x0, y0, x1, y1);
    const int w = x1 - x0, n = w * (y1 - y0);
    const int dq = 16 / w, dr = 16 - dq * w;
    int j = tid & 15, row = j / w, col = j - row * w;
    for (; j < n; j += 16) {
      f(i, -1, x0 + col, y0 + row);
      col += dr; row += dq;
      if (col >= w) { col -= w; row += 1; }
    }
  }
}

__global__ __launch_bounds__(256) void k_count_tiles_lds(int P, int T, int gx, const uint2* __restrict__ rects,
                                                          uint32_t* __restrict__ tile_count, uint32_t* __restrict__ entries,
                                                          uint32_t* __restrict__ entry_n) {
  HIP_DYNAMIC_SHARED(uint32_t, s_bins)
  __shared__ uint32_t s_wide[BIN_CHUNK];
  __shared__ uint2 s_wide_rect[BIN_CHUNK];
  __shared__ uint32_t s_nwide;
  __shared__ uint32_t s_wave_nz[4];
  const int tid = threadIdx.x;
  const int lo = blockIdx.x * BIN_CHUNK, hi = min(P, lo + BIN_CHUNK);
  uint2 own[BIN_PER_THREAD];
#pragma unroll
  for (int j = 0; j < BIN_PER_THREAD; ++j) own[j] = rects[min(lo + tid + 256 * j, P - 1)];
  for (int t = tid; t < T; t += 256) s_bins[t] = 0;
  if (tid == 0) s_nwide = 0;
  __syncthreads();
  for_each_instance(lo, hi, own, rects, s_wide, s_wide_rect, &s_nwide, [&](int, int, int x, int y) { atomicAdd(&s_bins[y * gx + x], 1u); });
  __syncthreads();
  unsigned long long mask = 0ull;
  {
    int k = 0;
    for (int t = tid; t < T; t += 256, ++k) {
      const uint32_t c = s_bins[t];
      if (c) { atomicAdd(&tile_count[t], c); mask |= 1ull << k; }
    }
  }
  const uint32_t nz = (uint32_t)__popcll(mask);
  const uint32_t incl = gs_wave_scan_incl_u32(nz);
  if ((tid & 63) == 63) s_wave_nz[tid >> 6] = incl;
  __syncthreads();
  uint32_t off = incl - nz, total = 0;
#pragma unroll
  for (int w = 0; w < 4; ++w) {
    if (w < (tid >> 6)) off += s_wave_nz[w];
    total += s_wave_nz[w];
  }
  if (tid == 0) entry_n[blockIdx.x] = total <= (uint32_t)GS_BIN_ENTRIES ? total : 0xffffffffu;
  if (total > (uint32_t)GS_BIN_ENTRIES) return;
  uint32_t* mine = entries + (size_t)blockIdx.x * GS_BIN_ENTRIES + off;
  while (mask) {
    const int t = tid + 256 * (__ffsll((long long)mask) - 1);
    mask &= mask - 1ull;
    *mine++ = (uint32_t)t | (s_bins[t] << 16);
  }
}

__global__ __launch_bounds__(256) void k_scatter_lds(int P, int T, int gx, const float* __restrict__ depths,
                                                      const uint2* __restrict__ rects, const uint32_t* __restrict__ start,
                                                      uint32_t* __restrict__ cursor, uint64_t* __restrict__ keys, uint32_t capacity,
                                                      const uint32_t* __restrict__ entries, const uint32_t* __restrict__ entry_n) {
  HIP_DYNAMIC_SHARED(uint32_t, s_bins)
  __shared__ uint32_t s_wide[BIN_CHUNK];
  __shared__ uint2 s_wide_rect[BIN_CHUNK];
  __shared__ uint32_t s_nwide;
  const int tid = threadIdx.x;
  const int lo = blockIdx.x * BIN_CHUNK, hi = min(P, lo + BIN_CHUNK);
  uint2 own[BIN_PER_THREAD];
  uint32_t own_depth[BIN_PER_THREAD];
#pragma unroll
  for (int j = 0; j < BIN_PER_THREAD; ++j) {
    const int ic = min(lo + tid + 256 * j, P - 1);
    own[j] = rects[ic];
    own_depth[j] = __float_as_uint(depths[ic]);
  }
  const uint32_t n_entries = entry_n[blockIdx.x];
  if (n_entries != 0xffffffffu) {
    const uint32_t* mine = entries + (size_t)blockIdx.x * GS_BIN_ENTRIES;
    for (uint32_t e0 = 0; e0 < n_entries; e0 += 1024) {
      uint32_t en[4], r[4], st[4];
#pragma unroll
      for (int j = 0; j < 4; ++j) {
        const uint32_t e = e0 + tid + 256 * j;
        en[j] = e < n_entries ? mine[e] : 0u;
      }
#pragma unroll
      for (int j = 0; j < 4; ++j) {
        r[j] = 0u; st[j] = 0u;
        if (en[j]) { r[j] = atomicAdd(&cursor[en[j] & 0xffffu], en[j] >> 16); st[j] = start[en[j] & 0xffffu]; }
      }
#pragma unroll
      for (int j = 0; j < 4; ++j)
        if (en[j]) s_bins[en[j] & 0xffffu] = st[j] + r[j];
    }
  } else {
    for (int t = tid; t < T; t += 256) s_bins[t] = 0;
    if (tid == 0) s_nwide = 0;
    __syncthreads();
    for_each_instance(lo, hi, own, rects, s_wide, s_wide_rect, &s_nwide, [&](int, int, int x, int y) { atomicAdd(&s_bins[y * gx + x], 1u); });
    __syncthreads();
    for (int t0 = 0; t0 < T; t0 += 1024) {
      uint32_t c[4], r[4], st[4];
#pragma unroll
      for (int j = 0; j < 4; ++j) {
        const int t = t0 + tid + 256 * j;
        c[j] = t < T ? s_bins[t] : 0u;
      }
#pragma unroll
      for (int j = 0; j < 4; ++j) {
        const int t = t0 + tid + 256 * j;
        r[j] = 0u; st[j] = 0u;
        if (c[j]) { r[j] = atomicAdd(&cursor[t], c[j]); st[j] = start[t]; }
      }
#pragma unroll
      for (int j = 0; j < 4; ++j)
        if (c[j]) s_bins[t0 + tid + 256 * j] = st[j] + r[j];
    }
  }
  if (tid == 0) s_nwide = 0;
  __syncthreads();
  for_each_instance(lo, hi, own, rects, s_wide, s_wide_rect, &s_nwide, [&](int i, int j, int x, int y) {
    const uint32_t depth = j == 0 ? own_depth[0] : (j == 1 ? own_depth[BIN_PER_THREAD - 1] : __float_as_uint(depths[i]));
    const uint64_t key = ((uint64_t)depth << 32) | (uint32_t)i;
    const uint32_t pos = atomicAdd(&s_bins[y * gx + x], 1u);
    if (pos < capacity) keys[pos] = key;
  });
}

__global__ __launch_bounds__(256) void k_count_tiles_direct(int P, int gx, const uint2* __restrict__ rects,
                                                             uint32_t* __restrict__ tile_count) {
  const int i = blockIdx.x * blockDim.x + threadIdx.x;
  if (i >= P) return;
  int x0, y0, x1, y1;
  if (!unpack_rect(rects[i], x0, y0, x1, y1)) return;
  for (int y = y0; y < y1; ++y)
    for (int x = x0; x < x1; ++x) atomicAdd(&tile_count[y * gx + x], 1u);
}

__global__ __launch_bounds__(256) void k_scatter_direct(int P, int gx, const float* __restrict__ depths, const uint2* __restrict__ rects,
                                                         const uint32_t* __restrict__ start, uint32_t* __restrict__ cursor,
                                                         uint64_t* __restrict__ keys, uint32_t capacity) {
  const int i = blockIdx.x * blockDim.x + threadIdx.x;
  if (i >= P) return;
  int x0, y0, x1, y1;
  if (!unpack_rect(rects[i], x0, y0, x1, y1)) return;
  const uint64_t key = ((uint64_t)__float_as_uint(depths[i]) << 32) | (uint32_t)i;
  for (int y = y0; y < y1; ++y)
    for (int x = x0; x < x1; ++x) {
      const int t = y * gx + x;
      const uint32_t pos = start[t] + atomicAdd(&cursor[t], 1u);
      if (pos < capacity) keys[pos] = key;
    }
}

template <class KeyPtr>
__device__ __forceinline__ void bitonic_sort_any(KeyPtr a, int n, int tid, int nthreads) {
  int np2 = 1;
  while (np2 < n) np2 <<= 1;
  const int half = np2 >> 1;
  for (int k = 2; k <= np2; k <<= 1) {
    const int hk = k >> 1;
    for (int t = tid; t < half; t += nthreads) {
      const int blk = t / hk, off = t - blk * hk;
      const int i = blk * k + off, j = blk * k + (k - 1 - off);
      if (j < n) {
        const uint64_t x = a[i], y = a[j];
        if (x > y) { a[i] = y; a[j] = x; }
      }
    }
    __syncthreads();
    for (int d = hk >> 1; d >= 1; d >>= 1) {
      for (int t = tid; t < half; t += nthreads) {
        const int i = (t / d) * (2 * d) + (t % d), j = i + d;
        if (j < n) {
          const uint64_t x = a[i], y = a[j];
          if (x > y) { a[i] = y; a[j] = x; }
        }
      }
      __syncthreads();
    }
  }
}

template <int CTRL>
__device__ __forceinline__ uint32_t sort_dpp(uint32_t v) {
  return (uint32_t)__builtin_amdgcn_update_dpp(0, (int)v, CTRL, 0xF, 0xF, true);
}
template <int LM>
__device__ __forceinline__ uint32_t lane_xchg32(uint32_t v) {
  if constexpr (LM >= 16) return (uint32_t)__builtin_amdgcn_ds_bpermute((int)(((threadIdx.x & 63) ^ LM) << 2), (int)v);
  else if constexpr (LM == 1) return sort_dpp<0xB1>(v);
  else if constexpr (LM == 2) return sort_dpp<0x4E>(v);
  else if constexpr (LM == 3) return sort_dpp<0x1B>(v);
  else if constexpr (LM == 4) {
    const int lo = __builtin_amdgcn_update_dpp(0, (int)v, 0x104, 0xF, 0x5, false);
    return (uint32_t)__builtin_amdgcn_update_dpp(lo, (int)v, 0x114, 0xF, 0xA, false);
  }
  else if constexpr (LM == 7) return sort_dpp<0x141>(v);
  else if constexpr (LM == 8) return sort_dpp<0x128>(v);
  else {
    static_assert(LM == 15, "lane mask of a bitonic network inside a wave64");
    return sort_dpp<0x140>(v);
  }
}
template <int LM>
__device__ __forceinline__ uint64_t lane_xchg64(uint64_t v) {
  return ((uint64_t)lane_xchg32<LM>((uint32_t)(v >> 32)) << 32) | lane_xchg32<LM>((uint32_t)v);
}

template <int E, int KK>
__device__ __forceinline__ void sort_flip_stage(uint64_t (&k)[E], uint64_t* __restrict__ s_keys, int base) {
  constexpr int m = KK - 1;
  if constexpr (KK <= E) {
#pragma unroll
    for (int e = 0; e < E; ++e) {
      const int pe = e ^ (m & (E - 1));
      if (e < pe) { const uint64_t a = k[e], b = k[pe]; if (a > b) { k[e] = b; k[pe] = a; } }
    }
  } else if constexpr (KK <= 64 * E) {
    constexpr int lm = (m / E) & 63;
    uint64_t other[E];
#pragma unroll
    for (int e = 0; e < E; ++e) other[e] = lane_xchg64<lm>(k[E - 1 - e]);
    const bool lower = (base & (KK >> 1)) == 0;
#pragma unroll
    for (int e = 0; e < E; ++e) { const uint64_t a = k[e], b = other[e]; k[e] = ((b < a) == lower) ? b : a; }
  } else {
    __syncthreads();
#pragma unroll
    for (int e = 0; e < E; ++e) s_keys[base + e] = k[e];
    __syncthreads();
    const bool lower = (base & (KK >> 1)) == 0;
#pragma unroll
    for (int e = 0; e < E; ++e) { const uint64_t a = k[e], b = s_keys[(base + e) ^ m]; k[e] = ((b < a) == lower) ? b : a; }
  }
}

template <int E, int D>
__device__ __forceinline__ void sort_disperse_from(uint64_t (&k)[E], uint64_t* __restrict__ s_keys, int base) {
  if constexpr (D >= 1) {
    if constexpr (D < E) {
#pragma unroll
      for (int e = 0; e < E; ++e) {
        const int pe = e ^ D;
        if (e < pe) { const uint64_t a = k[e], b = k[pe]; if (a > b) { k[e] = b; k[pe] = a; } }
      }
    } else if constexpr (D < 64 * E) {
      const bool lower = (base & D) == 0;
#pragma unroll
      for (int e = 0; e < E; ++e) { const uint64_t a = k[e], b = lane_xchg64<D / E>(a); k[e] = ((b < a) == lower) ? b : a; }
    } else {
      __syncthreads();
#pragma unroll
      for (int e = 0; e < E; ++e) s_keys[base + e] = k[e];
      __syncthreads();
      const bool lower = (base & D) == 0;
#pragma unroll
      for (int e = 0; e < E; ++e) { const uint64_t a = k[e], b = s_keys[(base + e) ^ D]; k[e] = ((b < a) == lower) ? b : a; }
    }
    sort_disperse_from<E, D / 2>(k, s_keys, base);
  }
}

template <int E, int KK, int NP2>
__device__ __forceinline__ void sort_merge_from(uint64_t (&k)[E], uint64_t* __restrict__ s_keys, int base) {
  if constexpr (KK <= NP2) {
    sort_flip_stage<E, KK>(k, s_keys, base);
    sort_disperse_from<E, KK / 4>(k, s_keys, base);
    sort_merge_from<E, KK * 2, NP2>(k, s_keys, base);
  }
}

template <int E>
__device__ __forceinline__ void sort_tile_regs(uint64_t* __restrict__ s_keys, const uint64_t* keys, uint32_t* __restrict__ list,
                                               uint32_t s, int n, uint64_t* keys_out = nullptr) {
  const int tid = threadIdx.x, lane = tid & 63, wave = tid >> 6;
  const int base = wave * (64 * E) + lane * E;
  uint64_t k[E];
#pragma unroll
  for (int e = 0; e < E; ++e) k[e] = (base + e < n) ? keys[s + base + e] : ~0ull;
  sort_merge_from<E, 2, SORT_THREADS * E>(k, s_keys, base);
  if (keys_out) {
#pragma unroll
    for (int e = 0; e < E; ++e)
      if (base + e < n) keys_out[s + base + e] = k[e];
  } else {
#pragma unroll
    for (int e = 0; e < E; ++e)
      if (base + e < n) list[s + base + e] = (uint32_t)k[e];
  }
}

template <int NMAX>
__device__ __forceinline__ uint32_t sort_count_below(const uint64_t* __restrict__ run, int n, uint64_t key) {
  int lo = 0;
#pragma unroll
  for (int step = NMAX; step >= 1; step >>= 1)
    if (lo + step <= n && run[lo + step - 1] < key) lo += step;
  return (uint32_t)lo;
}
template <int EA, int EB>
__device__ __forceinline__ void sort_tile_two_runs(uint64_t* __restrict__ s_keys, const uint64_t* keys, uint32_t* __restrict__ list,
                                                   uint32_t s, int n) {
  constexpr int NA = SORT_THREADS * EA, NBMAX = SORT_THREADS * EB;
  static_assert(NA + NBMAX <= SORT_SMALL_CAP, "both sorted runs are parked in the kernel's LDS array");
  const int tid = threadIdx.x, lane = tid & 63, wave = tid >> 6;
  const int base_a = wave * (64 * EA) + lane * EA, base_b = wave * (64 * EB) + lane * EB, nb = n - NA;
  uint64_t ka[EA], kb[EB];
#pragma unroll
  for (int e = 0; e < EA; ++e) ka[e] = keys[s + base_a + e];
#pragma unroll
  for (int e = 0; e < EB; ++e) kb[e] = (base_b + e < nb) ? keys[s + NA + base_b + e] : ~0ull;
  sort_merge_from<EA, 2, NA>(ka, s_keys, base_a);
  sort_merge_from<EB, 2, NBMAX>(kb, s_keys, base_b);
  __syncthreads();
#pragma unroll
  for (int e = 0; e < EA; ++e) s_keys[base_a + e] = ka[e];
#pragma unroll
  for (int e = 0; e < EB; ++e) s_keys[NA + base_b + e] = kb[e];
  __syncthreads();
#pragma unroll
  for (int e = 0; e < EA; ++e) list[s + base_a + e + sort_count_below<NBMAX>(s_keys + NA, nb, ka[e])] = (uint32_t)ka[e];
#pragma unroll
  for (int e = 0; e < EB; ++e)
    if (base_b + e < nb) list[s + base_b + e + sort_count_below<NA>(s_keys, NA, kb[e])] = (uint32_t)kb[e];
}

__device__ __forceinline__ void sort_long_tile(uint64_t* __restrict__ s_keys, uint64_t* keys, uint32_t* __restrict__ list, uint32_t s, int n) {
  constexpr int RUN = SORT_SMALL_CAP, E = RUN / SORT_THREADS;
  const int nrun = (n + RUN - 1) / RUN, tid = threadIdx.x;
  for (int r = 0; r < nrun; ++r) {
    __syncthreads();
    sort_tile_regs<E>(s_keys, keys, list, s + (uint32_t)r * RUN, min(RUN, n - r * RUN), keys);
  }
  for (int r = 0; r < nrun; ++r) {
    const int rn = min(RUN, n - r * RUN);
    uint64_t k[E];
    uint32_t rank[E];
    __syncthreads();
#pragma unroll
    for (int e = 0; e < E; ++e) {
      const int i = tid * E + e;
      k[e] = i < rn ? keys[s + (uint32_t)r * RUN + i] : ~0ull;
      rank[e] = (uint32_t)i;
    }
    for (int r2 = 0; r2 < nrun; ++r2) {
      if (r2 == r) continue;
      const int n2 = min(RUN, n - r2 * RUN);
      __syncthreads();
      for (int i = tid; i < n2; i += SORT_THREADS) s_keys[i] = keys[s + (uint32_t)r2 * RUN + i];
      __syncthreads();
#pragma unroll
      for (int e = 0; e < E; ++e) {
        int lo = 0, hi = n2;
        while (lo < hi) {
          const int mid = (lo + hi) >> 1;
          if (s_keys[mid] < k[e]) lo = mid + 1; else hi = mid;
        }
        rank[e] += (uint32_t)lo;
      }
    }
#pragma unroll
    for (int e = 0; e < E; ++e)
      if (tid * E + e < rn) list[s + rank[e]] = (uint32_t)k[e];
  }
}

__device__ __forceinline__ void sort_one_tile(int tile, const uint32_t* __restrict__ start, uint64_t* keys,
                                              uint32_t* __restrict__ list, uint32_t capacity) {
  __shared__ uint64_t s_keys[SORT_SMALL_CAP];
  const uint32_t s = min(start[tile], capacity), e = min(start[tile + 1], capacity);
  const int n = (int)(e - s);
  if (n <= 0) return;
  if (n <= SORT_THREADS) sort_tile_regs<1>(s_keys, keys, list, s, n);
  else if (n <= SORT_THREADS * 2) sort_tile_regs<2>(s_keys, keys, list, s, n);
  else if (n <= SORT_THREADS * 3) sort_tile_two_runs<2, 1>(s_keys, keys, list, s, n);
  else if (n <= SORT_THREADS * 4) sort_tile_regs<4>(s_keys, keys, list, s, n);
  else if (n <= SORT_THREADS * 5) sort_tile_two_runs<4, 1>(s_keys, keys, list, s, n);
  else if (n <= SORT_THREADS * 6) sort_tile_two_runs<4, 2>(s_keys, keys, list, s, n);
  else if (n <= SORT_SMALL_CAP) sort_tile_regs<8>(s_keys, keys, list, s, n);
  else if (n <= SORT_LDS_CAP) sort_long_tile(s_keys, keys, list, s, n);
  else {
    uint64_t* seg = keys + s;
    bitonic_sort_any(seg, n, (int)threadIdx.x, SORT_THREADS);
    for (int i = threadIdx.x; i < n; i += SORT_THREADS) list[s + i] = (uint32_t)seg[i];
  }
}

__global__ __launch_bounds__(SORT_THREADS) void k_sort_tiles(int T, const uint32_t* __restrict__ start, uint64_t* keys,
                                                              uint32_t* __restrict__ list, uint32_t capacity,
                                                              const uint32_t* __restrict__ order) {
  sort_one_tile((int)order[blockIdx.x], start, keys, list, capacity);
}

}

static int g_min_units = GS_MIN_UNITS;
extern "C" int mi355gs_tune_min_units(int min_units) {
  const int old = g_min_units;
  if (min_units > 0) g_min_units = min_units;
  return old;
}
int gs_min_units() { return g_min_units; }

int gs_launch_scan_tiles(hipStream_t stream, int T, const uint32_t* count, uint32_t* start, int32_t* num_rendered, uint32_t* order,
                         uint32_t* meta, uint32_t* seg_first, uint32_t* part_first, int min_units) {
  const size_t stage_bytes = (size_t)((T + SCAN_THREADS - 1) / SCAN_THREADS) * SCAN_THREADS * 4;
  if (T > SCAN_THREADS && stage_bytes <= SCAN_STAGE_MAX_BYTES)
    hipLaunchKernelGGL(k_scan_tiles<true>, dim3(1), dim3(SCAN_THREADS), stage_bytes, stream, T, count, start, num_rendered, order, meta,
                       seg_first, part_first, (uint32_t)min_units);
  else
    hipLaunchKernelGGL(k_scan_tiles<false>, dim3(1), dim3(SCAN_THREADS), 0, stream, T, count, start, num_rendered, order, meta, seg_first,
                       part_first, (uint32_t)min_units);
  return 0;
}

template <bool RECT>
static int scan_large(hipStream_t stream, int n, const uint32_t* in, uint32_t* out, uint32_t* block_sums, int32_t* total) {
  const int nb = (n + SCAN_CHUNK - 1) / SCAN_CHUNK;
  hipLaunchKernelGGL(k_scan_block_sums<RECT>, dim3(nb), dim3(256), 0, stream, n, in, block_sums);
  hipLaunchKernelGGL(k_scan_tiles<false>, dim3(1), dim3(SCAN_THREADS), 0, stream, nb, (const uint32_t*)block_sums, block_sums, total,
                     (uint32_t*)nullptr, (uint32_t*)nullptr, (uint32_t*)nullptr, (uint32_t*)nullptr, 0u);
  hipLaunchKernelGGL(k_scan_apply<RECT>, dim3(nb), dim3(256), 0, stream, n, in, (const uint32_t*)block_sums, out);
  return 0;
}
int gs_launch_scan_large(hipStream_t stream, int n, const uint32_t* in, uint32_t* out, uint32_t* block_sums, int32_t* total) {
  return scan_large<false>(stream, n, in, out, block_sums, total);
}
int gs_launch_scan_rect_areas(hipStream_t stream, int P, const uint2* rects, uint32_t* off, uint32_t* block_sums, int32_t* total) {
  return scan_large<true>(stream, P + 1, reinterpret_cast<const uint32_t*>(rects), off, block_sums, total);
}

int gs_launch_count_tiles(hipStream_t stream, int P, int T, int gx, const uint2* rects, uint32_t* tile_count, uint32_t* entries,
                          uint32_t* entry_n) {
  if (P <= 0) return 0;
  if (T <= BIN_MAX_LDS_TILES) {
    GsProfScope prof(5, stream);
    hipLaunchKernelGGL(k_count_tiles_lds, dim3((P + BIN_CHUNK - 1) / BIN_CHUNK), dim3(256), (size_t)T * 4, stream, P, T, gx, rects, tile_count,
                       entries, entry_n);
  }
  else
    hipLaunchKernelGGL(k_count_tiles_direct, dim3((P + 255) / 256), dim3(256), 0, stream, P, gx, rects, tile_count);
  return 0;
}

int gs_launch_binning(hipStream_t stream, int P, int T, int gx, const float* depths, const uint2* rects, const uint32_t* start,
                      uint32_t* cursor, uint64_t* keys, uint32_t* list, uint32_t capacity, const uint32_t* order, const uint32_t* entries,
                      const uint32_t* entry_n) {
  if (P <= 0 || capacity == 0) return 0;
  if (T <= BIN_MAX_LDS_TILES)
    hipLaunchKernelGGL(k_scatter_lds, dim3((P + BIN_CHUNK - 1) / BIN_CHUNK), dim3(256), (size_t)T * 4, stream, P, T, gx, depths, rects,
                       start, cursor, keys, capacity, entries, entry_n);
  else
    hipLaunchKernelGGL(k_scatter_direct, dim3((P + 255) / 256), dim3(256), 0, stream, P, gx, depths, rects, start, cursor, keys, capacity);
  {
    GsProfScope prof(4, stream);
    hipLaunchKernelGGL(k_sort_tiles, dim3(T), dim3(SORT_THREADS), 0, stream, T, start, keys, list, capacity, order);
  }
  return 0;
}
```

### instantsplat_amd/csrc/common.h

```cpp
#pragma once
#include <hip/hip_runtime.h>
#include <stdint.h>
#include <stddef.h>
#include "../../include/mi355gs.h"
#include <type_traits>

#define GS_LOG2E 1.4426950408889634f
#define GS_TILE 16
#define GS_TILE_PIX 256
#define GS_WAVE 64

struct alignas(16) GsRec {
  float4 q0;
  float4 q1;
  float4 q2;
};

struct alignas(16) GsGrad {
  float4 g0;
  float4 g1;
  float4 g2;
};

static inline size_t gs_align(size_t x) { return (x + 255) & ~(size_t)255; }
// ... 8 lines not shown
  }
};
int gs_write_view_consts(hipStream_t stream, float* consts, const char* name);

constexpr int GS_BIN_CHUNK = 512;
constexpr int GS_BIN_ENTRIES = 1024;

struct GeomLayout {
  size_t rec, cov3D, rect, clamped, depth, bin_entries, bin_n, total;
  __host__ explicit GeomLayout(int P) {
    size_t n = P > 0 ? (size_t)P : 1, o = 0;
    rec = o; o += gs_align(n * sizeof(GsRec));
    cov3D = o; o += gs_align(n * 6 * sizeof(float));
    rect = o; o += gs_align(n * sizeof(uint2));
    clamped = o; o += gs_align(n);
    depth = o; o += gs_align(n * sizeof(float));
    const size_t chunks = (n + GS_BIN_CHUNK - 1) / GS_BIN_CHUNK;
    bin_entries = o; o += gs_align(chunks * GS_BIN_ENTRIES * sizeof(uint32_t));
    bin_n = o; o += gs_align(chunks * sizeof(uint32_t));
    total = o;
  }
};

constexpr int GS_SORT_SMALL_CAP = 2048;

constexpr int GS_UNIT_LEVELS = 4;
__host__ __device__ inline int gs_unit_level_for(long long instances, long long min_units) {
  int level = 0;
  while (level + 1 < GS_UNIT_LEVELS && (instances >> (7 + level)) >= min_units) ++level;
  return level;
}
struct GsKnobs {
  int min_units;
  int det;
};
GsKnobs gs_knobs();
struct DetScratchLayout {
  size_t off, block_sums, total;
  __host__ explicit DetScratchLayout(int P) {
    const size_t n = (size_t)(P > 0 ? P : 1) + 1;
    size_t o = 0;
    off = o; o += gs_align((n + 1) * 4);
    block_sums = o; o += gs_align(((n + 4095) / 4096 + 2) * 4);
    total = o;
  }
};
int gs_min_units();
constexpr int GS_MIN_UNITS = 40960;

struct TilesLayout {
  size_t count, start, cursor, final_T, n_contrib, order, seg_first, part_first, meta, qmax, total;
  int gx, gy, T;
  __host__ TilesLayout(int W, int H) {
    gx = (W + GS_TILE - 1) / GS_TILE; gy = (H + GS_TILE - 1) / GS_TILE; T = gx * gy;
    size_t o = 0, npix = (size_t)W * H;
    count = o; o += gs_align((size_t)T * 4);
    cursor = o; o += gs_align((size_t)T * 4);
    start = o; o += gs_align(((size_t)T + 1) * 4);
    final_T = o; o += gs_align(npix * 4);
    n_contrib = o; o += gs_align(npix * 4);
    order = o; o += gs_align((size_t)T * 4);
    seg_first = o; o += gs_align(((size_t)T + 1) * 4);
    part_first = o; o += gs_align(((size_t)T + 1) * 4);
    meta = o; o += gs_align(16);
    qmax = o; o += gs_align((size_t)T * 4 * 4);
    total = o;
  }
};

constexpr int GS_SEG = 64;

struct BinningLayout {
  size_t keys, list, unit_tile, bstate, hitmask, det_rows, det_rowidx, total;
  uint32_t max_chunks;
  uint32_t max_units;
  bool may_loop;
  __host__ BinningLayout(int64_t R, int T, const GsKnobs& knobs) {
    size_t n = R > 0 ? (size_t)R : 1, o = 0;
    keys = o; o += gs_align(n * 8);
    list = o; o += gs_align(n * 4);
    const size_t mu = (size_t)knobs.min_units, top = (size_t)GS_SEG << (GS_UNIT_LEVELS - 1);
    const size_t by_chunks = (n + GS_SEG - 1) / GS_SEG, by_rule = 2 * mu + 1, by_top = (n + top - 1) / top;
    const size_t lim = by_chunks < by_rule ? by_chunks : by_rule;
    may_loop = gs_unit_level_for((long long)n, (long long)mu) > 0;
    max_units = (uint32_t)((lim > by_top ? lim : by_top) + (size_t)(T > 0 ? T : 1));
    unit_tile = o; o += gs_align((size_t)max_units * 16);
    bstate = o; o += gs_align((size_t)max_units * 256 * sizeof(float4));
    max_chunks = (uint32_t)(by_chunks + 8 * (size_t)(T > 0 ? T : 1) + 8);
    hitmask = o; o += gs_align((size_t)max_chunks * 4 * sizeof(uint64_t));
    det_rows = det_rowidx = o;
    if (knobs.det) {
      det_rows = o; o += gs_align(n * sizeof(GsGrad));
      det_rowidx = o; o += gs_align(n * 4);
    }
    total = o;
  }
};


__device__ __forceinline__ float3 gs_tp43(const float* m, float3 p) {
  return make_float3(m[0] * p.x + m[4] * p.y + m[8] * p.z + m[12], m[1] * p.x + m[5] * p.y + m[9] * p.z + m[13],
                     m[2] * p.x + m[6] * p.y + m[10] * p.z + m[14]);
}
__device__ __forceinline__ float4 gs_tp44(const float* m, float3 p) {
  return make_float4(m[0] * p.x + m[4] * p.y + m[8] * p.z + m[12], m[1] * p.x + m[5] * p.y + m[9] * p.z + m[13],
                     m[2] * p.x + m[6] * p.y + m[10] * p.z + m[14], m[3] * p.x + m[7] * p.y + m[11] * p.z + m[15]);
}

struct CamParams {
  const float* view;
  const float* proj;
  const float* campos;
  float tanfovx, tanfovy, focal_x, focal_y, scale_modifier;
  float scale_grad_factor;
  int W, H, gx, gy;
};

template <int CTRL, int ROW_MASK = 0xF, class T>
__device__ __forceinline__ T gs_dpp(T v) {
  static_assert(sizeof(T) == 4 || sizeof(T) == 8, "one or two 32-bit moves");
  uint32_t w[sizeof(T) / 4];
  __builtin_memcpy(w, &v, sizeof(T));
  for (size_t i = 0; i < sizeof(T) / 4; ++i) w[i] = (uint32_t)__builtin_amdgcn_update_dpp(0, (int)w[i], CTRL, ROW_MASK, 0xF, false);
  __builtin_memcpy(&v, w, sizeof(T));
  return v;
}
template <class T>
__device__ __forceinline__ T gs_wave_sum_row3(T v) {
  v += gs_dpp<0xB1>(v);
  v += gs_dpp<0x4E>(v);
  v += gs_dpp<0x141>(v);
  v += gs_dpp<0x140>(v);
  v += gs_dpp<0x142, 0xA>(v);
  v += gs_dpp<0x143, 0xC>(v);
  return v;
}
__device__ __forceinline__ double gs_wave_sum_row3_f64(double v) { return gs_wave_sum_row3(v); }

__device__ __forceinline__ void gs_finish_two_means(int nblocks, double inv_n, const float* __restrict__ partial, float& mean0, float& mean1) {
  __shared__ double s_a[16], s_b[16];
  double a = 0.0, b = 0.0;
  for (int i = threadIdx.x; i < nblocks; i += 1024) { a += (double)partial[2 * i]; b += (double)partial[2 * i + 1]; }
  a = gs_wave_sum_row3(a); b = gs_wave_sum_row3(b);
  if ((threadIdx.x & 63) == 63) { s_a[threadIdx.x >> 6] = a; s_b[threadIdx.x >> 6] = b; }
  __syncthreads();
  if (threadIdx.x != 0) return;
  double ta = 0.0, tb = 0.0;
  for (int w = 0; w < 16; ++w) { ta += s_a[w]; tb += s_b[w]; }
  mean0 = (float)(ta * inv_n); mean1 = (float)(tb * inv_n);
}
__device__ __forceinline__ float gs_l1_ssim_loss(float lambda_dssim, float l1_mean, float ssim_mean) {
  return (1.0f - lambda_dssim) * l1_mean + lambda_dssim * (1.0f - ssim_mean);
}

typedef float gs_v2f __attribute__((vector_size(8)));
__device__ __forceinline__ gs_v2f gs_fma2(gs_v2f a, gs_v2f b, gs_v2f c) { return a * b + c; }

__device__ __forceinline__ uint32_t gs_wave_max_u32(uint32_t v) {
  auto dpp = [](uint32_t x, auto ctrl) { return (uint32_t)__builtin_amdgcn_update_dpp(0, (int)x, decltype(ctrl)::value, 0xF, 0xF, true); };
  v = max(v, dpp(v, std::integral_constant<int, 0xB1>{}));
  v = max(v, dpp(v, std::integral_constant<int, 0x4E>{}));
  v = max(v, dpp(v, std::integral_constant<int, 0x141>{}));
  v = max(v, dpp(v, std::integral_constant<int, 0x140>{}));
  const auto a = __builtin_amdgcn_permlane16_swap(v, v, false, false);
  v = max(a[0], a[1]);
  const auto b = __builtin_amdgcn_permlane32_swap(v, v, false, false);
  return max(b[0], b[1]);
}

__device__ __forceinline__ uint32_t gs_wave_scan_incl_u32(uint32_t v) {
  auto up = [](uint32_t x, auto ctrl, auto rows) {
    return (uint32_t)__builtin_amdgcn_update_dpp(0, (int)x, decltype(ctrl)::value, decltype(rows)::value, 0xF, false);
  };
  using all = std::integral_constant<int, 0xF>;
  v += up(v, std::integral_constant<int, 0x111>{}, all{});
  v += up(v, std::integral_constant<int, 0x112>{}, all{});
  v += up(v, std::integral_constant<int, 0x114>{}, all{});
  v += up(v, std::integral_constant<int, 0x118>{}, all{});
  v += up(v, std::integral_constant<int, 0x142>{}, std::integral_constant<int, 0xA>{});
  v += up(v, std::integral_constant<int, 0x143>{}, std::integral_constant<int, 0xC>{});
  return v;
}

__device__ __forceinline__ float gs_sum_rows(float v) {
  const unsigned u = __float_as_uint(v);
  const auto a = __builtin_amdgcn_permlane16_swap(u, u, false, false);
  const float s = __uint_as_float(a[0]) + __uint_as_float(a[1]);
  const unsigned w = __float_as_uint(s);
  const auto b = __builtin_amdgcn_permlane32_swap(w, w, false, false);
  return __uint_as_float(b[0]) + __uint_as_float(b[1]);
}

__device__ __forceinline__ uint32_t gs_physical_cu() {
  const uint32_t hw = __builtin_amdgcn_s_getreg(4 | (31 << 11));
  const uint32_t xcc = __builtin_amdgcn_s_getreg(20 | (3 << 11));
  return ((xcc & 7u) << 6) | (((hw >> 13) & 3u) << 4) | ((hw >> 8) & 15u);
}

#ifdef __clang__
typedef float lp_acc16 __attribute__((ext_vector_type(16)));
#else
struct lp_acc16 {
  float v[16];
  float& operator[](int i) { return v[i]; }
  float operator[](int i) const { return v[i]; }
};
#endif
#ifdef __clang__
typedef float lp_f4 __attribute__((ext_vector_type(4)));
#define LP_AT(v, k) ((v)[k])
#define LP_ATC(v, k) ((v)[k])
#else
typedef float4 lp_f4;
#define LP_AT(v, k) (((float*)&(v))[k])
#define LP_ATC(v, k) (((const float*)&(v))[k])
#endif

__device__ __forceinline__ void lp_mfma_32x32x2(lp_acc16& c, const float* As, int lda, const float* Bs, int ldb, int lane) {
#if defined(__HIP_DEVICE_COMPILE__)
  c = __builtin_amdgcn_mfma_f32_32x32x2f32(As[(lane & 31) * lda + (lane >> 5)], Bs[(lane >> 5) * ldb + (lane & 31)], c, 0, 0, 0);
#else
  for (int k = 0; k < 2; ++k) {
    const float b = Bs[k * ldb + (lane & 31)];
    for (int r = 0; r < 16; ++r) c[r] = fmaf(As[((r & 3) + 8 * (r >> 2) + 4 * (lane >> 5)) * lda + k], b, c[r]);
  }
#endif
}

__device__ __forceinline__ int lp_acc_row(int r, int lane) { return (r & 3) + 8 * (r >> 2) + 4 * (lane >> 5); }

extern thread_local bool g_krange_open;
void gs_range_pop();
#define GS_CHECK_LAUNCH(name)                                                   \
  do {                                                                          \
    if (g_krange_open) { g_krange_open = false; gs_range_pop(); }               \
    hipError_t e_ = hipGetLastError();                                          \
    if (e_ == hipSuccess && debug) e_ = hipStreamSynchronize((hipStream_t)stream); \
    if (e_ != hipSuccess) {                                                     \
      gs_log_error(name, hipGetErrorString(e_));                                \
      return MI355GS_ELAUNCH;                                                   \
    }                                                                           \
  } while (0)

void gs_log_error(const char* where, const char* what);

extern bool g_ranges_on;
void gs_range_push(const char* name);
void gs_range_pop();
struct GsRange {
  bool active;
  explicit GsRange(const char* name) : active(g_ranges_on) { if (active) gs_range_push(name); }
  ~GsRange() { if (active) gs_range_pop(); }
  GsRange(const GsRange&) = delete;
  GsRange& operator=(const GsRange&) = delete;
};
#define GS_RANGE() GsRange gs_range_(__func__)
extern thread_local bool g_krange_open;
#define GS_KRANGE(name) do { if (g_ranges_on) { gs_range_push(name); g_krange_open = true; } } while (0)

struct GsProfScope {
  hipStream_t s; hipEvent_t stop; bool active = false;
  GsProfScope(int kind, hipStream_t stream);
  ~GsProfScope();
};


struct GsPrologue {
  float4* grad_records = nullptr; size_t n_vec = 0;
  uint32_t* tile_counters = nullptr; int n_counters = 0;
  float* g_poses = nullptr; int n_pose = 0;
  float* pose_scratch = nullptr;
  float* adam_scratch = nullptr;
};
struct GsPosed {
  const float* pose = nullptr;
  float* acc = nullptr;
  float* partial = nullptr;
};
enum { GS_GATE_XYZ = 0, GS_GATE_SH = 1, GS_GATE_SH_REST = 2, GS_GATE_OPACITY = 3, GS_GATE_SCALING = 4, GS_GATE_ROT = 5, GS_GATE_POSE = 6 };

struct GsScene {
  int P, D, M;
  const float *means3D, *shs, *shs_rest, *colors_precomp, *opacities, *scales, *rotations, *cov3D_precomp;
  float scale_modifier;
};
struct GsView {
  int W, H;
  const float *view, *proj, *campos;
  float tanfovx, tanfovy;
};
struct GsFrameBufs {
  void *geom, *tiles, *binning;
  int64_t capacity;
  int32_t* radii;
  void* grad_scratch;
  GsKnobs knobs;
};
struct GsFrameCtx {
  const GsPrologue* prologue = nullptr;
  GsPosed posed;
  float* gate = nullptr;
  bool gate_tail = false;
  bool pose_only = false;
};
struct GsGradOut { float *means3D, *means2D, *shs, *shs_rest, *colors, *opacities, *scales, *rotations, *cov3D; };
static inline size_t gs_grad_gate_offset(int P) { return gs_align((size_t)(P > 0 ? P : 1) * sizeof(GsGrad)); }
static inline size_t gs_grad_scratch_bytes(int P, int det) { return gs_grad_gate_offset(P) + 256 + (det ? DetScratchLayout(P).total : 0); }
static inline size_t gs_binning_bytes(int64_t n, int W, int H, const GsKnobs& k, bool train) {
  const BinningLayout bl(n, TilesLayout(W, H).T, k);
  return train ? bl.total : bl.unit_tile;
}
static inline const uint32_t* gs_frame_count(const void* tiles, int W, int H) {
  const TilesLayout tl(W, H);
  return (const uint32_t*)((const char*)tiles + tl.start) + tl.T;
}
int gs_frame_project(hipStream_t stream, const GsScene& sc, const GsView& vw, const GsFrameBufs& fb, const GsFrameCtx& cx,
                     int32_t* num_rendered, uint8_t* visible, int debug);
int gs_frame_render(hipStream_t stream, int P, const GsView& vw, const GsFrameBufs& fb, const float* bg, float* out_color, bool train,
                    int debug);
int gs_frame_backward(hipStream_t stream, const GsScene& sc, const GsView& vw, const GsFrameBufs& fb, const GsFrameCtx& cx,
                      const float* bg, const float* out_color, const float* dL_dpix, const GsGradOut& out, bool grad_scratch_is_clear,
                      int debug);

struct GsAdamFused {
  uint32_t* live; uint32_t seq;
  const uint32_t* commit_count; unsigned long long commit_capacity;
  uint32_t* commit_poison;
};
int gs_adam_multi(hipStream_t stream, int ntensors, const int64_t* numel, const int32_t* row, float* const* params,
                  const float* const* grads, float* const* exp_avg, float* const* exp_avg_sq, const float* const* per_point_lr,
                  const float* lr, float beta1, float beta2, float eps, const int32_t* step, float* scratch, const float* gate,
                  const int32_t* gate_index, uint32_t* live, uint32_t seq, const GsAdamFused* fused);

struct GsFrozenScene {
  int P, M, W, H;
  int64_t capacity;
  const float *xyz, *f_dc, *f_rest, *opacity, *scaling, *rotation;
  char *geom, *tiles, *binning;
  float *image, *consts;
  int32_t *radii, *num_rendered;

  bool init(int P_, int M_, int W_, int H_, int64_t capacity_, const float* xyz_, const float* f_dc_, const float* f_rest_,
            const float* opacity_, const float* scaling_, const float* rotation_, const void* workspace) {
    if (P_ <= 0 || M_ < 1 || M_ > 16 || W_ <= 0 || H_ <= 0 || W_ > 65535 * GS_TILE || H_ > 65535 * GS_TILE || capacity_ <= 0 || !workspace)
      return false;
    if (!xyz_ || !f_dc_ || (M_ > 1 && !f_rest_) || !opacity_ || !scaling_ || !rotation_) return false;
    P = P_; M = M_; W = W_; H = H_; capacity = capacity_;
    xyz = xyz_; f_dc = f_dc_; f_rest = M_ > 1 ? f_rest_ : nullptr; opacity = opacity_; scaling = scaling_; rotation = rotation_;
    return true;
  }
  void carve(GsCarver& c, const GsKnobs& knobs, bool train) {
    geom = c.take<char>(GeomLayout(P).total);
    tiles = c.take<char>(TilesLayout(W, H).total);
    binning = c.take<char>(gs_binning_bytes(capacity, W, H, knobs, train));
    image = c.take<float>(3 * (size_t)W * H);
    consts = c.take<float>(32);
    radii = c.take<int32_t>((size_t)P);
    num_rendered = c.take<int32_t>(1);
  }
  bool degree_ok(int D) const { return D >= 0 && D <= 3 && (D + 1) * (D + 1) <= M; }
  GsScene scene(int D) const {
    return {P, D, D == 0 ? 1 : M, xyz, f_dc, D == 0 ? nullptr : f_rest, nullptr, opacity, scaling, rotation, nullptr, 1.0f};
  }
  GsView view(const float* proj, float tanfovx, float tanfovy) const { return {W, H, consts, proj, consts + 16, tanfovx, tanfovy}; }
  GsFrameBufs bufs(const GsKnobs& knobs, void* grad_scratch) const { return {geom, tiles, binning, capacity, radii, grad_scratch, knobs}; }
  const uint32_t* count() const { return gs_frame_count(tiles, W, H); }
};
```

### instantsplat_amd/csrc/trainer.hip

```cpp
#include <stdlib.h>
#include <string.h>
#include "common.h"

int gs_loss_fused(hipStream_t, int, int, int, const float*, const float*, float, float*, void*);
int gs_loss_fused_nblocks(int, int, int);
int gs_launch_pose_finish_partials(hipStream_t, const float*, const float*, int, float*, float*, const float*, int, double, float, float*, int,
                                   int);

namespace {

struct Trainer {
  int P, W, H, V;
  int64_t capacity;
  float *xyz, *f_dc, *f_rest, *opacity, *scaling, *rotation, *poses;
  float* m[7];
  float* v[7];
  const float* pplr;
  char *geom, *tiles, *binning, *grad_scratch, *ssim_scratch;
  float *image, *dL_dimg;
  int32_t* radii;
  float *g_means2D, *g_colors;
  float *g_xyz, *g_rot, *g_scaling, *g_opacity, *g_fdc, *g_frest, *g_poses;
  float *pose_scratch, *pose_partial, *adam_scratch, *consts;
  uint32_t* adam_live;
  uint32_t adam_seq;
  bool consts_ready;
  GsKnobs knobs;
};

size_t carve(Trainer& t, void* workspace) {
  GsCarver c{(char*)workspace};
  const size_t P = (size_t)(t.P > 0 ? t.P : 1), npix = (size_t)t.W * t.H;
  t.geom = c.take<char>(GeomLayout(t.P).total);
  t.tiles = c.take<char>(TilesLayout(t.W, t.H).total);
  t.binning = c.take<char>(gs_binning_bytes(t.capacity, t.W, t.H, t.knobs, true));
  t.grad_scratch = c.take<char>(gs_grad_scratch_bytes(t.P, t.knobs.det));
  t.ssim_scratch = c.take<char>(mi355gs_ssim_scratch_bytes(1, 3, t.H, t.W));
  t.image = c.take<float>(3 * npix); t.dL_dimg = c.take<float>(3 * npix);
  t.radii = c.take<int32_t>(P);
  t.g_means2D = c.take<float>(3 * P); t.g_colors = c.take<float>(3 * P);
  t.g_xyz = c.take<float>(3 * P); t.g_rot = c.take<float>(4 * P); t.g_scaling = c.take<float>(3 * P); t.g_opacity = c.take<float>(P);
  t.g_fdc = c.take<float>(3 * P); t.g_frest = c.take<float>(45 * P); t.g_poses = c.take<float>(7 * (size_t)t.V);
  t.pose_scratch = c.take<float>(32); t.pose_partial = c.take<float>(16 * ((P + 255) / 256)); t.adam_scratch = c.take<float>(8); t.consts = c.take<float>(32);
  t.adam_live = c.take<uint32_t>(16);
  return c.off;
}

int trainer_adam(Trainer* t, hipStream_t stream, const float* lr, const int32_t* step, float beta1, float beta2, float eps,
                 bool commit_gate) {
  const int P = t->P;
  const int64_t numel[7] = {3LL * P, 3LL * P, 45LL * P, (int64_t)P, 3LL * P, 4LL * P, 7LL * t->V};
  const int32_t row[7] = {3, 1, 1, 1, 1, 1, 1};
  float* params[7] = {t->xyz, t->f_dc, t->f_rest, t->opacity, t->scaling, t->rotation, t->poses};
  const float* grads[7] = {t->g_xyz, t->g_fdc, t->g_frest, t->g_opacity, t->g_scaling, t->g_rot, t->g_poses};
  const float* pplr[7] = {t->pplr, nullptr, nullptr, nullptr, nullptr, nullptr, nullptr};
  if (++t->adam_seq == 0u) t->adam_seq = 1u;
  GsAdamFused fused = {t->adam_live, t->adam_seq, nullptr, 0, nullptr};
  if (commit_gate) {
    fused.commit_count = gs_frame_count(t->tiles, t->W, t->H);
    fused.commit_capacity = (unsigned long long)t->capacity;
    fused.commit_poison = t->adam_live + 15;
  }
  return gs_adam_multi(stream, 7, numel, row, params, grads, t->m, t->v, pplr, lr, beta1, beta2, eps, step, t->adam_scratch, nullptr, nullptr,
                       nullptr, 0u, &fused);
}

GsScene posed_scene(int P, int D, const float* xyz, const float* f_dc, const float* f_rest, const float* opacity_logit,
                    const float* log_scales, float scale_modifier, const float* rotation) {
  return {P, D, D == 0 ? 1 : 16, xyz, f_dc, D == 0 ? nullptr : f_rest, nullptr, opacity_logit, log_scales, rotation, nullptr, scale_modifier};
}

}

extern "C" {

int mi355gs_posed_forward_preprocess(void* stream, int P, int D, int W, int H, const float* xyz, const float* f_dc,
                                     const float* f_rest, const float* opacity_logit, const float* log_scales, float scale_modifier,
                                     const float* rotation, const float* pose, const float* view_identity, const float* projmatrix,
                                     const float* origin, float tanfovx, float tanfovy, int32_t* radii, void* geom, void* tiles,
                                     int32_t* num_rendered, uint8_t* visible, void* grad_scratch, int debug) {
  GS_RANGE();
  if (!pose || D < 0 || D > 3 || (D > 0 && !f_rest)) return MI355GS_EINVAL;
  GsFrameCtx cx;
  cx.posed.pose = pose;
  return gs_frame_project((hipStream_t)stream, posed_scene(P, D, xyz, f_dc, f_rest, opacity_logit, log_scales, scale_modifier, rotation),
                          {W, H, view_identity, projmatrix, origin, tanfovx, tanfovy}, {geom, tiles, nullptr, 0, radii, grad_scratch, gs_knobs()},
                          cx, num_rendered, visible, debug);
}

int mi355gs_posed_backward(void* stream_, int P, int D, int W, int H, const float* bg, const float* xyz, const float* f_dc,
                           const float* f_rest, const float* opacity_logit, const float* log_scales, float scale_modifier,
                           const float* rotation, const float* pose, const float* view_identity, const float* projmatrix,
                           const float* origin, float tanfovx, float tanfovy, const void* geom, void* tiles, const void* binning,
                           int64_t capacity, const int32_t* radii, const float* out_color, const float* dL_dpix,
                           void* grad_scratch, float* pose_scratch, float* d_xyz, float* d_means2D, float* d_f_dc, float* d_f_rest,
                           float* d_opacity_logit, float* d_log_scales, float* d_rotation, float* d_pose, int pose_rows, int pose_row,
                           int grad_scratch_is_clear, int debug) {
  GS_RANGE();
  hipStream_t stream = (hipStream_t)stream_;
  if (!pose || !pose_scratch || !d_pose || D < 0 || D > 3 || (D > 0 && (!f_rest || !d_f_rest))) return MI355GS_EINVAL;
  if (pose_rows < 0 || (pose_rows > 0 && (pose_row < 0 || pose_row >= pose_rows))) return MI355GS_EINVAL;
  if (P <= 0)
    return hipMemsetAsync(d_pose, 0, (size_t)(pose_rows > 0 ? pose_rows : 1) * 7 * sizeof(float), stream) == hipSuccess ? MI355GS_OK : MI355GS_ELAUNCH;
  const int rows = (P + 255) / 256;
  float* gate = (float*)((char*)grad_scratch + gs_grad_gate_offset(P));
  GsFrameCtx cx;
  cx.posed.pose = pose;
  cx.posed.acc = pose_scratch + (size_t)16 * rows;
  cx.posed.partial = pose_scratch;
  cx.gate = gate; cx.gate_tail = true;
  const GsGradOut o = {d_xyz, d_means2D, d_f_dc, D == 0 ? nullptr : d_f_rest, nullptr, d_opacity_logit, d_log_scales, d_rotation, nullptr};
  const int rc = gs_frame_backward(stream, posed_scene(P, D, xyz, f_dc, f_rest, opacity_logit, log_scales, scale_modifier, rotation),
                                   {W, H, view_identity, projmatrix, origin, tanfovx, tanfovy},
                                   {const_cast<void*>(geom), tiles, const_cast<void*>(binning), capacity, const_cast<int32_t*>(radii), grad_scratch, gs_knobs()},
                                   cx, bg, out_color, dL_dpix, o, grad_scratch_is_clear != 0, debug);
  if (rc) return rc;
  GS_KRANGE("pose_finish");
  gs_launch_pose_finish_partials(stream, pose, pose_scratch, rows, d_pose, gate + GS_GATE_POSE, nullptr, 0, 0.0, 0.f, nullptr, pose_rows, pose_row);
  GS_CHECK_LAUNCH("pose_finish");
  return MI355GS_OK;
}

size_t mi355gs_trainer_workspace_bytes(int P, int W, int H, int V, int64_t capacity) {
  if (P < 0 || W <= 0 || H <= 0 || V <= 0 || capacity < 0) return 0;
  Trainer t;
  memset(&t, 0, sizeof(t));
  t.P = P; t.W = W; t.H = H; t.V = V; t.capacity = capacity; t.knobs = gs_knobs();
  return carve(t, nullptr);
}

void* mi355gs_trainer_create(int P, int W, int H, int V, int64_t capacity, float* xyz, float* f_dc, float* f_rest, float* opacity,
                             float* scaling, float* rotation, float* poses, float* const* exp_avg, float* const* exp_avg_sq,
                             const float* per_point_lr, void* workspace) {
  if (P <= 0 || W <= 0 || H <= 0 || V <= 0 || capacity <= 0 || !workspace || !exp_avg || !exp_avg_sq) return nullptr;
  if (!xyz || !f_dc || !f_rest || !opacity || !scaling || !rotation || !poses) return nullptr;
  Trainer* t = (Trainer*)calloc(1, sizeof(Trainer));
  if (!t) return nullptr;
  t->P = P; t->W = W; t->H = H; t->V = V; t->capacity = capacity;
  t->xyz = xyz; t->f_dc = f_dc; t->f_rest = f_rest; t->opacity = opacity; t->scaling = scaling; t->rotation = rotation; t->poses = poses;
  for (int k = 0; k < 7; ++k) {
    if (!exp_avg[k] || !exp_avg_sq[k]) { free(t); return nullptr; }
    t->m[k] = exp_avg[k]; t->v[k] = exp_avg_sq[k];
  }
  t->pplr = per_point_lr;
  t->knobs = gs_knobs();
  carve(*t, workspace);
  t->consts_ready = false;
  return t;
}

void mi355gs_trainer_destroy(void* handle) { free(handle); }

const float* mi355gs_trainer_grad(void* handle, int k) {
  Trainer* t = (Trainer*)handle;
  if (!t || k < 0 || k > 6) return nullptr;
  const float* g[7] = {t->g_xyz, t->g_fdc, t->g_frest, t->g_opacity, t->g_scaling, t->g_rot, t->g_poses};
  return g[k];
}

int mi355gs_trainer_step(void* handle, void* stream_, int view, int sh_degree, const float* gt_image, const float* projmatrix,
                         float tanfovx, float tanfovy, const float* bg, const float* lr, const int32_t* step, float beta1, float beta2, float eps,
                         float lambda_dssim, int do_optimizer_step, float* loss_out, int32_t* num_rendered_out) {
  GS_RANGE();
  Trainer* t = (Trainer*)handle;
  hipStream_t stream = (hipStream_t)stream_;
  const int debug = 0;
  if (!t || view < 0 || view >= t->V || sh_degree < 0 || sh_degree > 3 || !gt_image || !projmatrix || !bg || !lr || !step || !loss_out || !num_rendered_out)
    return MI355GS_EINVAL;
  const int P = t->P, W = t->W, H = t->H;
  if (!t->consts_ready) {
    if (int rc = gs_write_view_consts(stream, t->consts, "trainer_consts")) return rc;
    if (hipMemsetAsync(t->g_frest, 0, (size_t)P * 45 * sizeof(float), stream) != hipSuccess) return MI355GS_ELAUNCH;
    if (hipMemsetAsync(t->adam_live, 0, 16 * sizeof(uint32_t), stream) != hipSuccess) return MI355GS_ELAUNCH;
    t->consts_ready = true;
  }
  GsPrologue pro;
  {
    const TilesLayout tl(W, H);
    pro.grad_records = (float4*)t->grad_scratch; pro.n_vec = (size_t)P * 3;
    pro.tile_counters = (uint32_t*)(t->tiles + tl.count); pro.n_counters = (int)((tl.start - tl.count) / 4);
    pro.g_poses = t->g_poses; pro.n_pose = 7 * t->V; pro.pose_scratch = t->pose_scratch; pro.adam_scratch = t->adam_scratch;
  }
  const float* pose = t->poses + 7 * (size_t)view;
  GsFrameCtx cx;
  cx.prologue = &pro;
  cx.posed.pose = pose; cx.posed.acc = t->pose_scratch; cx.posed.partial = t->pose_partial;
  cx.gate = t->adam_scratch;
  const int D = sh_degree;
  const GsScene scene = posed_scene(P, D, t->xyz, t->f_dc, t->f_rest, t->opacity, t->scaling, 1.0f, t->rotation);
  const GsView vw = {W, H, t->consts, projmatrix, t->consts + 16, tanfovx, tanfovy};
  const GsFrameBufs bufs = {t->geom, t->tiles, t->binning, t->capacity, t->radii, t->grad_scratch, t->knobs};
  int rc;
  if ((rc = gs_frame_project(stream, scene, vw, bufs, cx, num_rendered_out, nullptr, 0))) return rc;
  if ((rc = gs_frame_render(stream, P, vw, bufs, bg, t->image, true, 0))) return rc;
  if ((rc = gs_loss_fused(stream, 3, H, W, t->image, gt_image, lambda_dssim, t->dL_dimg, t->ssim_scratch))) return rc;
  const GsGradOut o = {t->g_xyz, t->g_means2D, t->g_fdc, D == 0 ? nullptr : t->g_frest, t->g_colors, t->g_opacity, t->g_scaling, t->g_rot, nullptr};
  if ((rc = gs_frame_backward(stream, scene, vw, bufs, cx, bg, t->image, t->dL_dimg, o, false, 0))) return rc;
  GS_KRANGE("pose_finish");
  gs_launch_pose_finish_partials(stream, pose, t->pose_partial, (P + 255) / 256, t->g_poses + 7 * (size_t)view, t->adam_scratch + GS_GATE_POSE,
                                 (const float*)t->ssim_scratch, gs_loss_fused_nblocks(3, H, W), 1.0 / (3.0 * H * W), lambda_dssim, loss_out, 0, 0);
  GS_CHECK_LAUNCH("pose_finish");
  if (do_optimizer_step) return trainer_adam(t, stream, lr, step, beta1, beta2, eps, true);
  return MI355GS_OK;
}

int mi355gs_trainer_optimizer_step(void* handle, void* stream_, const float* lr, const int32_t* step, float beta1, float beta2,
                                   float eps, int commit_gate) {
  GS_RANGE();
  Trainer* t = (Trainer*)handle;
  if (!t || !lr || !step || !t->consts_ready) return MI355GS_EINVAL;
  return trainer_adam(t, (hipStream_t)stream_, lr, step, beta1, beta2, eps, commit_gate != 0);
}

}
```

### instantsplat_amd/csrc_torch/binding.cpp

```cpp
#include <torch/extension.h>
#include <ATen/hip/impl/HIPGuardImplMasqueradingAsCUDA.h>
#include <c10/hip/HIPStream.h>

#include <chrono>
#include <optional>
#include <map>
#include <mutex>

#include "../../include/mi355gs.h"

namespace {

using torch::Tensor;
using torch::autograd::AutogradContext;
using torch::autograd::variable_list;

#define GS_ABI_LIST(X)                                                 \
  X(geom_bytes, mi355gs_raster_geom_bytes)                             \
  X(tiles_bytes, mi355gs_raster_tiles_bytes)                           \
  X(binning_bytes, mi355gs_raster_binning_bytes)                       \
  X(grad_scratch_bytes, mi355gs_raster_grad_scratch_bytes)             \
  X(grad_gate_offset, mi355gs_raster_grad_gate_offset)                 \
  X(posed_forward_preprocess, mi355gs_posed_forward_preprocess)        \
  X(forward_preprocess, mi355gs_raster_forward_preprocess)             \
  X(raster_backward, mi355gs_raster_backward)                          \
  X(forward_render, mi355gs_raster_forward_render)                     \
  X(binning_bytes_render_only, mi355gs_raster_binning_bytes_render_only) \
  X(forward_render_only, mi355gs_raster_forward_render_only)           \
  X(posed_backward, mi355gs_posed_backward)                            \
  X(ssim_scratch_bytes, mi355gs_ssim_scratch_bytes)                    \
  X(l1_ssim_loss_fused, mi355gs_l1_ssim_loss_fused)                    \
  X(l1_scratch_bytes, mi355gs_l1_scratch_bytes)                        \
  X(l1_loss_forward, mi355gs_l1_loss_forward)                          \
  X(l1_loss_backward, mi355gs_l1_loss_backward)                        \
  X(pair_forward, mi355gs_l1_ssim_pair_forward)                        \
  X(pair_backward, mi355gs_l1_ssim_pair_backward)                      \
  X(program_eval, mi355gs_loss_program_eval)                           \
  X(program_eval_grad, mi355gs_loss_program_eval_grad)                 \
  X(ssim_forward, mi355gs_ssim_forward)                                \
  X(ssim_backward, mi355gs_ssim_backward)                              \
  X(adam_multi_step, mi355gs_adam_multi_step)                          \
  X(error_string, mi355gs_error_string)

struct Abi {
#define GS_MEMBER(field, name) decltype(&name) field = nullptr;
  GS_ABI_LIST(GS_MEMBER)
#undef GS_MEMBER
  bool bound = false;
  bool allow_cpu = false;
} g_abi;

std::vector<std::string> abi_symbols() {
#define GS_NAME(field, name) #name,
  return {GS_ABI_LIST(GS_NAME)};
#undef GS_NAME
}

void bind_abi(const std::map<std::string, uintptr_t>& sym, bool allow_cpu_tensors) {
  g_abi.allow_cpu = allow_cpu_tensors;
  auto get = [&](const char* name) {
    auto it = sym.find(name);
    TORCH_CHECK(it != sym.end() && it->second, "mi355gs torch binding: entry point ", name, " was not provided");
    return it->second;
  };
#define GS_BIND(field, name) g_abi.field = reinterpret_cast<decltype(&name)>(get(#name));
  GS_ABI_LIST(GS_BIND)
#undef GS_BIND
  g_abi.bound = true;
}

void check(int code, const char* what) {
  TORCH_CHECK(code == 0, "mi355gs: ", what, " failed: ", g_abi.error_string ? g_abi.error_string(code) : "?", " (", code, ")");
}

struct DeviceScope {
  c10::hip::OptionalHIPGuardMasqueradingAsCUDA guard;
  void* stream = nullptr;
  explicit DeviceScope(const Tensor& t) {
    if (t.is_cuda()) {
      guard.set_device(t.device());
      stream = (void*)c10::hip::getCurrentHIPStream(t.device().index()).stream();
    }
  }
  void synchronize(const Tensor& t) const {
    if (t.is_cuda()) c10::hip::getCurrentHIPStream(t.device().index()).synchronize();
  }
};

void wait_for_count(const int32_t* count, const DeviceScope& dev, const Tensor& t) {
  if (!t.is_cuda()) return;
  std::optional<py::gil_scoped_release> nogil;
  if (PyGILState_Check()) nogil.emplace();
  const auto t0 = std::chrono::steady_clock::now();
  for (unsigned spin = 0;; ++spin) {
    if (*reinterpret_cast<const volatile int32_t*>(count) >= 0) return;
    if ((spin & 1023u) == 1023u && std::chrono::steady_clock::now() - t0 > std::chrono::milliseconds(2)) break;
  }
  dev.synchronize(t);
  TORCH_CHECK(*reinterpret_cast<const volatile int32_t*>(count) >= 0, "mi355gs: the forward did not report its instance count");
}

void wait_for_words(Tensor words, int64_t sentinel, Tensor like, int64_t timeout_us) {
  TORCH_CHECK(words.scalar_type() == at::kInt && !words.is_cuda() && words.is_contiguous(), "wait_for_words: an int32 host tensor");
  const volatile int32_t* w = words.data_ptr<int32_t>();
  const int64_t n = words.numel();
  auto all_there = [&]() {
    for (int64_t i = 0; i < n; ++i)
      if (w[i] == (int32_t)sentinel) return false;
    return true;
  };
  if (all_there()) return;
  {
    std::optional<py::gil_scoped_release> nogil;
    if (PyGILState_Check()) nogil.emplace();
    const auto t0 = std::chrono::steady_clock::now();
    for (unsigned spin = 0;; ++spin) {
      if (all_there()) return;
      if ((spin & 1023u) == 1023u && std::chrono::steady_clock::now() - t0 > std::chrono::microseconds(timeout_us)) break;
    }
    if (like.is_cuda()) {
      const DeviceScope dev(like);
      dev.synchronize(like);
    }
  }
  TORCH_CHECK(all_there(), "mi355gs: the step did not report its results");
}

Tensor f32c(const Tensor& t, const char* name, const Tensor& like) {
  TORCH_CHECK(t.is_cuda() || g_abi.allow_cpu, "instantsplat_amd operators run on the GPU only (got a CPU tensor; there is no CPU fallback)");
  TORCH_CHECK(t.scalar_type() == at::kFloat, "expected float32, got ", t.scalar_type(), " (", name, ")");
  TORCH_CHECK(t.device() == like.device(), "tensors on different devices: ", like.device(), " vs ", t.device(), " (", name, ")");
  return t.is_contiguous() ? t : t.contiguous();
}
float* fp(const Tensor& t) { return t.defined() && t.numel() ? t.data_ptr<float>() : nullptr; }

Tensor empty_bytes(size_t n, const Tensor& like) {
  return at::empty({(int64_t)(n > 0 ? n : 1)}, like.options().dtype(at::kByte));
}

struct HostClock {
  std::chrono::steady_clock::time_point t0 = std::chrono::steady_clock::now();
  double* acc;
  explicit HostClock(double* a) : acc(a) {}
  ~HostClock() { *acc += std::chrono::duration<double, std::micro>(std::chrono::steady_clock::now() - t0).count(); }
};
double g_host_us[6] = {0, 0, 0, 0, 0, 0};

struct GateRecord {
  Tensor scratch;
  const float* gate = nullptr;
  std::vector<c10::weak_intrusive_ptr<c10::StorageImpl>> storage;
  int64_t numel[7] = {0, 0, 0, 0, 0, 0, 0};
  int64_t version[7] = {0, 0, 0, 0, 0, 0, 0};
  bool valid = false;
};
std::mutex g_gate_mutex;
GateRecord g_gates;

template <class... T> bool any_requires_grad(const T&... t) {
  if (!at::GradMode::is_enabled()) return false;
  bool any = false;
  ((any = any || (t.defined() && t.requires_grad())), ...);
  return any;
}
thread_local bool t_backward_follows = false;
struct BackwardFollows {
  explicit BackwardFollows(bool v) { t_backward_follows = v; }
  ~BackwardFollows() { t_backward_follows = false; }
};

struct ZeroGrad { Tensor buf; uint32_t version = 0; };
std::mutex g_zero_mutex;
std::map<std::string, ZeroGrad> g_zero_pool;
bool g_share_zero_grad = true;
Tensor zero_grad_like(const Tensor& like) {
  if (!g_share_zero_grad) return at::zeros_like(like);
  std::ostringstream key;
  key << like.device() << ":" << like.sizes() << "@" << like.data_ptr();
  std::lock_guard<std::mutex> lock(g_zero_mutex);
  if (g_zero_pool.size() > 8 && !g_zero_pool.count(key.str())) g_zero_pool.clear();
  ZeroGrad& z = g_zero_pool[key.str()];
  if (!z.buf.defined()) {
    z.buf = at::zeros_like(like, like.options().requires_grad(false), at::MemoryFormat::Contiguous);
    z.version = z.buf._version();
  } else if (z.buf._version() != z.version) {
    z.buf.zero_();
    z.version = z.buf._version();
  }
  return z.buf.detach();
}

struct PoseRowSeen {
  c10::weak_intrusive_ptr<c10::TensorImpl> row{c10::intrusive_ptr<c10::TensorImpl>()};
  int64_t rows = 0, index = 0;
};
thread_local PoseRowSeen t_pose_row;
struct PoseTableWritten {
  c10::weak_intrusive_ptr<c10::StorageImpl> storage{c10::intrusive_ptr<c10::StorageImpl>()};
  int64_t rows = 0, index = 0;
  bool valid = false;
};
PoseTableWritten g_pose_table;

struct PoseRowFn : public torch::autograd::Function<PoseRowFn> {
  static Tensor forward(AutogradContext* ctx, Tensor table, int64_t index) {
    TORCH_CHECK(table.dim() == 2 && table.size(1) == 7, "pose_row: the pose table must be [views, 7]");
    const int64_t rows = table.size(0);
    if (index < 0) index += rows;
    TORCH_CHECK(index >= 0 && index < rows, "pose_row: index ", index, " is out of range for ", rows, " poses");
    ctx->saved_data["rows"] = rows;
    ctx->saved_data["index"] = index;
    Tensor row = table.select(0, index).detach();
    t_pose_row.row = c10::weak_intrusive_ptr<c10::TensorImpl>(row.getIntrusivePtr());
    t_pose_row.rows = table.is_contiguous() && table.scalar_type() == at::kFloat ? rows : 0;
    t_pose_row.index = index;
    return row;
  }
  static variable_list backward(AutogradContext* ctx, variable_list grad_out) {
    const int64_t rows = ctx->saved_data["rows"].toInt(), index = ctx->saved_data["index"].toInt();
    const Tensor& g = grad_out[0];
    if (!g.defined()) return {Tensor(), Tensor()};
    {
      std::lock_guard<std::mutex> lock(g_gate_mutex);
      auto strong = g_pose_table.storage.lock();
      const bool mine = g_pose_table.valid && strong && strong.get() == g.storage().unsafeGetStorageImpl() && g_pose_table.rows == rows &&
                        g_pose_table.index == index && g.scalar_type() == at::kFloat && g.dim() == 1 && g.numel() == 7 && g.is_contiguous() &&
                        g.storage_offset() == 7 * index;
      g_pose_table.valid = false;
      if (mine) {
        Tensor full = at::empty({0}, g.options());
        full.set_(g.storage(), 0, {rows, 7}, {7, 1});
        if (g_gates.valid && g_gates.storage.size() == 7) {
          g_gates.storage[6] = full.storage().getWeakStorageImpl();
          g_gates.numel[6] = full.numel();
          g_gates.version[6] = (int64_t)full._version();
        }
        return {full, Tensor()};
      }
    }
    Tensor full = at::zeros({rows, 7}, g.options());
    full.select(0, index).copy_(g);
    return {full, Tensor()};
  }
};

Tensor pose_row(Tensor table, int64_t index) { return PoseRowFn::apply(table, index); }

void check_frame_buffers(const Tensor& binning, const Tensor& scratch, int64_t R, int P, int W, int H) {
  const size_t need_b = g_abi.binning_bytes(R, W, H), need_s = g_abi.grad_scratch_bytes(P);
  TORCH_CHECK(!binning.defined() || (size_t)binning.numel() >= need_b || R <= 0,
              "mi355gs: this frame's binning buffer (", binning.numel(), " bytes) is smaller than the backward's layout needs (", need_b,
              "): the deterministic-backward mode was switched on between the frame's forward and its backward");
  TORCH_CHECK(!scratch.defined() || (size_t)scratch.numel() >= need_s,
              "mi355gs: this frame's gradient scratch (", scratch.numel(), " bytes) is smaller than the backward needs (", need_s,
              "): the deterministic-backward mode was switched on between the frame's forward and its backward");
}

struct FrameForward {
  Tensor radii, color, geom, tiles, binning;
  Tensor scratch;
  int64_t R = 0;
  int32_t* count;

  FrameForward(const Tensor& like, int P, const Tensor& count_slot) {
    TORCH_CHECK(count_slot.scalar_type() == at::kInt && count_slot.numel() == 1, "count_slot must be one int32");
    count = count_slot.data_ptr<int32_t>();
    radii = at::empty({P}, like.options().dtype(at::kInt));
  }

  template <class Project>
  void run(const DeviceScope& dev, const Tensor& like, int P, int W, int H, const Tensor& bg, int64_t capacity, int64_t count_hint,
           const Project& project) {
    color = at::empty({3, H, W}, like.options());
    geom = empty_bytes(g_abi.geom_bytes(P), like);
    tiles = empty_bytes(g_abi.tiles_bytes(W, H), like);
    if (t_backward_follows) scratch = empty_bytes(g_abi.grad_scratch_bytes(P), like);
    auto preprocess = [&]() {
      *reinterpret_cast<volatile int32_t*>(count) = -1;
      project(*this);
    };
    auto stage2 = [&](int64_t cap) {
      if (t_backward_follows) {
        binning = empty_bytes(g_abi.binning_bytes(cap, W, H), like);
        check(g_abi.forward_render(dev.stream, P, W, H, cap, fp(bg), geom.data_ptr(), tiles.data_ptr(), binning.data_ptr(), fp(color), 0),
              "raster_forward_render");
      } else {
        binning = empty_bytes(g_abi.binning_bytes_render_only(cap, W, H), like);
        check(g_abi.forward_render_only(dev.stream, P, W, H, cap, fp(bg), geom.data_ptr(), tiles.data_ptr(), binning.data_ptr(), fp(color), 0),
              "raster_forward_render_only");
      }
    };
    preprocess();
    R = capacity;
    if (R >= 0) {
      stage2(R);
      return;
    }
    const int64_t guess = count_hint > 0 ? count_hint + count_hint / 2 + 16384 : -1;
    if (guess > 0) stage2(guess);
    {
      HostClock wait_clock(&g_host_us[5]);
      wait_for_count(count, dev, like);
    }
    R = *reinterpret_cast<volatile int32_t*>(count);
    if (guess > 0 && R <= guess) {
      R = guess;
    } else {
      if (guess > 0) {
        preprocess();
        wait_for_count(count, dev, like);
      }
      stage2(R);
    }
  }
};

std::pair<Tensor, int> backward_scratch(AutogradContext* ctx, Tensor scratch, const Tensor& like, const Tensor& binning, int64_t R, int P,
                                        int W, int H) {
  const int is_clear = (scratch.defined() && ctx->saved_data["scratch_is_clear"].toBool()) ? 1 : 0;
  ctx->saved_data["scratch_is_clear"] = false;
  if (!scratch.defined()) scratch = empty_bytes(g_abi.grad_scratch_bytes(P), like);
  check_frame_buffers(binning, scratch, R, P, W, H);
  return {scratch, is_clear};
}

struct RenderPosedFn : public torch::autograd::Function<RenderPosedFn> {
  static variable_list forward(AutogradContext* ctx, Tensor xyz_, Tensor rot_, Tensor scaling_, Tensor opl_, Tensor f_dc_,
                               Tensor f_rest_, Tensor pose_, Tensor means2D, Tensor bg_, Tensor view_, Tensor proj_, Tensor origin_,
                               int64_t H, int64_t W, double tanfovx, double tanfovy, double scale_modifier, int64_t D,
                               int64_t capacity, int64_t count_hint, Tensor count_slot) {
    TORCH_CHECK(g_abi.bound, "mi355gs torch binding: bind() has not been called");
    HostClock clock(&g_host_us[0]);
    (void)means2D;
    const Tensor xyz = f32c(xyz_, "xyz", xyz_), rot = f32c(rot_, "rotation", xyz), scaling = f32c(scaling_, "scaling", xyz),
                 opl = f32c(opl_, "opacity", xyz), f_dc = f32c(f_dc_, "features_dc", xyz), f_rest = f32c(f_rest_, "features_rest", xyz),
                 pose = f32c(pose_, "camera_pose", xyz), bg = f32c(bg_, "bg", xyz), view = f32c(view_, "viewmatrix", xyz),
                 proj = f32c(proj_, "projmatrix", xyz), origin = f32c(origin_, "campos", xyz);
    TORCH_CHECK(xyz.dim() == 2 && xyz.size(1) == 3, "means3D must have dimensions (num_points, 3)");
    const int P = (int)xyz.size(0);
    const DeviceScope dev(xyz);
    FrameForward f(xyz, P, count_slot);
    Tensor visible = at::empty({P}, xyz.options().dtype(at::kBool));
    f.run(dev, xyz, P, (int)W, (int)H, bg, capacity, count_hint, [&](const FrameForward& frame) {
      check(g_abi.posed_forward_preprocess(dev.stream, P, (int)D, (int)W, (int)H, fp(xyz), fp(f_dc), fp(f_rest), fp(opl), fp(scaling),
                                           (float)scale_modifier, fp(rot), fp(pose), fp(view), fp(proj), fp(origin), (float)tanfovx,
                                           (float)tanfovy, frame.radii.data_ptr<int32_t>(), frame.geom.data_ptr(), frame.tiles.data_ptr(), frame.count,
                                           P > 0 ? reinterpret_cast<uint8_t*>(visible.data_ptr<bool>()) : nullptr,
                                           frame.scratch.defined() ? frame.scratch.data_ptr() : nullptr, 0),
            "posed_forward_preprocess");
    });
    ctx->saved_data["dims"] = std::vector<int64_t>{P, D, W, H, f.R};
    ctx->saved_data["scalars"] = std::vector<double>{tanfovx, tanfovy, scale_modifier};
    ctx->saved_data["scratch_is_clear"] = f.scratch.defined();
    {
      auto seen = t_pose_row.row.lock();
      const bool is_row = seen && seen.get() == pose_.unsafeGetTensorImpl() && t_pose_row.rows > 0;
      ctx->saved_data["pose_table"] = std::vector<int64_t>{is_row ? t_pose_row.rows : 0, is_row ? t_pose_row.index : 0};
    }
    ctx->save_for_backward({xyz, rot, scaling, opl, f_dc, f_rest, pose, f.radii, f.geom, f.tiles, f.binning, bg, view, proj, origin, f.color,
                            f.scratch});
    ctx->mark_non_differentiable({f.radii, visible});
    ctx->set_materialize_grads(false);
    return {f.color, f.radii, visible};
  }

  static variable_list backward(AutogradContext* ctx, variable_list grad_out) {
    HostClock clock(&g_host_us[1]);
    const auto saved = ctx->get_saved_variables();
    const Tensor &xyz = saved[0], &rot = saved[1], &scaling = saved[2], &opl = saved[3], &f_dc = saved[4], &f_rest = saved[5],
                 &pose = saved[6], &radii = saved[7], &geom = saved[8], &tiles = saved[9], &binning = saved[10], &bg = saved[11],
                 &view = saved[12], &proj = saved[13], &origin = saved[14], &color = saved[15];
    const auto dims = ctx->saved_data["dims"].toIntVector();
    const auto sc = ctx->saved_data["scalars"].toDoubleVector();
    const int P = (int)dims[0], D = (int)dims[1], W = (int)dims[2], H = (int)dims[3];
    const int64_t R = dims[4];
    if (!grad_out[0].defined()) return variable_list(21);
    const Tensor g = f32c(grad_out[0], "grad_color", xyz);
    const DeviceScope dev(xyz);
    Tensor d_xyz = at::empty_like(xyz), d_rot = at::empty_like(rot), d_scaling = at::empty_like(scaling), d_opl = at::empty_like(opl),
           d_fdc = at::empty_like(f_dc), d_m2d = at::empty_like(xyz);
    Tensor d_frest = D == 0 ? zero_grad_like(f_rest) : at::empty_like(f_rest);
    const auto pose_table = ctx->saved_data["pose_table"].toIntVector();
    const int64_t pose_rows = pose_table[0], pose_index = pose_table[1];
    Tensor d_pose_store = at::empty({pose_rows > 0 ? pose_rows * 7 : 7}, xyz.options());
    Tensor d_pose = d_pose_store;
    if (pose_rows > 0) {
      d_pose = at::empty({0}, xyz.options());
      d_pose.set_(d_pose_store.storage(), 7 * pose_index, {7}, {1});
    }
    const auto [scratch, scratch_is_clear] = backward_scratch(ctx, saved[16], xyz, binning, R, P, W, H);
    Tensor pose_scratch = at::empty({16 * (((int64_t)P + 255) / 256) + 32}, xyz.options());
    check(g_abi.posed_backward(dev.stream, P, D, W, H, fp(bg), fp(xyz), fp(f_dc), fp(f_rest), fp(opl), fp(scaling), (float)sc[2], fp(rot),
                               fp(pose), fp(view), fp(proj), fp(origin), (float)sc[0], (float)sc[1], geom.data_ptr(), tiles.data_ptr(),
                               binning.data_ptr(), R, radii.data_ptr<int32_t>(), fp(color), fp(g), scratch.data_ptr(), fp(pose_scratch),
                               fp(d_xyz), fp(d_m2d), fp(d_fdc), D ? fp(d_frest) : nullptr, fp(d_opl), fp(d_scaling), fp(d_rot),
                               fp(d_pose_store), (int)pose_rows, (int)pose_index, scratch_is_clear, 0),
          "posed_backward");
    {
      std::lock_guard<std::mutex> lock(g_gate_mutex);
      g_pose_table.valid = pose_rows > 0;
      if (pose_rows > 0) {
        g_pose_table.storage = d_pose_store.storage().getWeakStorageImpl();
        g_pose_table.rows = pose_rows; g_pose_table.index = pose_index;
      }
      const Tensor* outs[7] = {&d_xyz, &d_fdc, &d_frest, &d_opl, &d_scaling, &d_rot, &d_pose};
      g_gates.storage.clear();
      for (int k = 0; k < 7; ++k) {
        g_gates.storage.push_back(outs[k]->storage().getWeakStorageImpl());
        g_gates.numel[k] = outs[k]->numel();
        g_gates.version[k] = (int64_t)outs[k]->_version();
      }
      g_gates.scratch = scratch;
      g_gates.gate = reinterpret_cast<const float*>(static_cast<const char*>(scratch.data_ptr()) + g_abi.grad_gate_offset(P));
      g_gates.valid = true;
    }
    Tensor none;
    return {d_xyz, d_rot, d_scaling, d_opl, d_fdc, d_frest, d_pose, d_m2d, none, none, none, none,
            none, none, none, none, none, none, none, none, none};
  }
};

std::vector<Tensor> render_posed(Tensor xyz, Tensor rot, Tensor scaling, Tensor opl, Tensor f_dc, Tensor f_rest, Tensor pose,
                                 Tensor means2D, Tensor bg, Tensor view, Tensor proj, Tensor origin, int64_t H, int64_t W,
                                 double tanfovx, double tanfovy, double scale_modifier, int64_t D, int64_t capacity, int64_t count_hint,
                                 Tensor count_slot) {
  const BackwardFollows scope(any_requires_grad(xyz, rot, scaling, opl, f_dc, f_rest, pose, means2D));
  return RenderPosedFn::apply(xyz, rot, scaling, opl, f_dc, f_rest, pose, means2D, bg, view, proj, origin, H, W, tanfovx, tanfovy,
                              scale_modifier, D, capacity, count_hint, count_slot);
}

struct RasterizeFn : public torch::autograd::Function<RasterizeFn> {
  using OptTensor = c10::optional<Tensor>;
  static variable_list forward(AutogradContext* ctx, Tensor means3D_, Tensor means2D, OptTensor sh_, OptTensor colors_, Tensor opac_,
                               OptTensor scales_, OptTensor rot_, OptTensor cov_, OptTensor sh_rest_, Tensor bg_, Tensor view_, Tensor proj_,
                               Tensor campos_,
                               int64_t H, int64_t W, double tanfovx, double tanfovy, double scale_modifier, int64_t D, bool prefiltered,
                               int64_t capacity, int64_t count_hint, Tensor count_slot) {
    TORCH_CHECK(g_abi.bound, "mi355gs torch binding: bind() has not been called");
    HostClock clock(&g_host_us[0]);
    (void)means2D;
    auto opt = [&](const OptTensor& t, const char* name, const Tensor& like) {
      return (t.has_value() && t->defined() && t->numel()) ? f32c(*t, name, like) : Tensor();
    };
    const Tensor means3D = f32c(means3D_, "means3D", means3D_), opac = f32c(opac_, "opacities", means3D);
    const Tensor sh = opt(sh_, "sh", means3D), colors = opt(colors_, "colors_precomp", means3D), scales = opt(scales_, "scales", means3D),
                 rot = opt(rot_, "rotations", means3D), cov = opt(cov_, "cov3Ds_precomp", means3D), sh_rest = opt(sh_rest_, "sh_rest", means3D);
    const Tensor bg = f32c(bg_, "bg", means3D), view = f32c(view_, "viewmatrix", means3D), proj = f32c(proj_, "projmatrix", means3D),
                 campos = f32c(campos_, "campos", means3D);
    TORCH_CHECK(means3D.dim() == 2 && means3D.size(1) == 3, "means3D must have dimensions (num_points, 3)");
    const int P = (int)means3D.size(0);
    const int M = sh.defined() ? (int)(sh.size(1) + (sh_rest.defined() ? sh_rest.size(1) : 0)) : 0;
    const DeviceScope dev(means3D);
    FrameForward f(means3D, P, count_slot);
    f.run(dev, means3D, P, (int)W, (int)H, bg, capacity, count_hint, [&](const FrameForward& frame) {
      check(g_abi.forward_preprocess(dev.stream, P, (int)D, M, (int)W, (int)H, fp(means3D), fp(sh), fp(sh_rest), fp(colors), fp(opac), fp(scales),
                                     (float)scale_modifier, fp(rot), fp(cov), fp(view), fp(proj), fp(campos), (float)tanfovx, (float)tanfovy,
                                     prefiltered ? 1 : 0, frame.radii.data_ptr<int32_t>(), frame.geom.data_ptr(), frame.tiles.data_ptr(), frame.count, nullptr,
                                     frame.scratch.defined() ? frame.scratch.data_ptr() : nullptr, 0),
            "raster_forward_preprocess");
    });
    ctx->saved_data["dims"] = std::vector<int64_t>{P, D, M, W, H, f.R};
    ctx->saved_data["scalars"] = std::vector<double>{tanfovx, tanfovy, scale_modifier};
    ctx->saved_data["opacity_shape"] = opac_.sizes().vec();
    ctx->saved_data["scratch_is_clear"] = f.scratch.defined();
    ctx->save_for_backward({means3D, sh, colors, opac, scales, rot, cov, sh_rest, f.radii, f.geom, f.tiles, f.binning, bg, view, proj, campos,
                            f.color, f.scratch});
    ctx->mark_non_differentiable({f.radii});
    ctx->set_materialize_grads(false);
    return {f.color, f.radii};
  }

  static variable_list backward(AutogradContext* ctx, variable_list grad_out) {
    if (!grad_out[0].defined()) return variable_list(23);
    const auto saved = ctx->get_saved_variables();
    const Tensor &means3D = saved[0], &sh = saved[1], &colors = saved[2], &opac = saved[3], &scales = saved[4], &rot = saved[5], &cov = saved[6],
                 &sh_rest = saved[7], &radii = saved[8], &geom = saved[9], &tiles = saved[10], &binning = saved[11], &bg = saved[12],
                 &view = saved[13], &proj = saved[14], &campos = saved[15], &color = saved[16];
    const auto dims = ctx->saved_data["dims"].toIntVector();
    const auto sc = ctx->saved_data["scalars"].toDoubleVector();
    const int P = (int)dims[0], D = (int)dims[1], M = (int)dims[2], W = (int)dims[3], H = (int)dims[4];
    const int64_t R = dims[5];
    const Tensor g = f32c(grad_out[0], "grad_color", means3D);
    const DeviceScope dev(means3D);
    const auto o = means3D.options();
    Tensor d_means3D = at::empty({P, 3}, o), d_means2D = at::empty({P, 3}, o), d_opac = at::empty({P}, o), d_col = at::empty({P, 3}, o);
    Tensor d_sh, d_shr, d_scales, d_rot, d_cov;
    if (sh.defined()) d_sh = at::empty({P, sh_rest.defined() ? 1 : M, 3}, o);
    if (sh_rest.defined()) d_shr = at::empty({P, M - 1, 3}, o);
    if (cov.defined()) d_cov = at::empty({P, 6}, o); else { d_scales = at::empty({P, 3}, o); d_rot = at::empty({P, 4}, o); }
    const auto [scratch, scratch_is_clear] = backward_scratch(ctx, saved[17], means3D, binning, R, P, W, H);
    check(g_abi.raster_backward(dev.stream, P, D, M, W, H, fp(bg), fp(means3D), fp(sh), fp(sh_rest), fp(colors), fp(opac), fp(scales), (float)sc[2],
                                fp(rot), fp(cov), fp(view), fp(proj), fp(campos), (float)sc[0], (float)sc[1], geom.data_ptr(), tiles.data_ptr(),
                                binning.data_ptr(), R, radii.data_ptr<int32_t>(), fp(color), fp(g), scratch.data_ptr(), fp(d_means3D), fp(d_means2D),
                                fp(d_sh), fp(d_shr), fp(d_col), fp(d_opac), fp(d_scales), fp(d_rot), fp(d_cov), scratch_is_clear, 0),
          "raster_backward");
    Tensor none;
    const auto shape = ctx->saved_data["opacity_shape"].toIntVector();
    return {d_means3D, d_means2D, d_sh, sh.defined() ? none : d_col, d_opac.reshape(shape), d_scales, d_rot, d_cov, d_shr,
            none, none, none, none, none, none, none, none, none, none, none, none, none, none};
  }
};

std::vector<Tensor> rasterize(Tensor means3D, Tensor means2D, c10::optional<Tensor> sh, c10::optional<Tensor> colors, Tensor opac,
                              c10::optional<Tensor> scales, c10::optional<Tensor> rot, c10::optional<Tensor> cov, c10::optional<Tensor> sh_rest,
                              Tensor bg, Tensor view, Tensor proj, Tensor campos, int64_t H, int64_t W, double tanfovx, double tanfovy,
                              double scale_modifier, int64_t D, bool prefiltered, int64_t capacity, int64_t count_hint, Tensor count_slot) {
  const Tensor none;
  auto val = [&](const c10::optional<Tensor>& t) -> const Tensor& { return t.has_value() ? *t : none; };
  const BackwardFollows scope(any_requires_grad(means3D, means2D, opac, val(sh), val(colors), val(scales), val(rot), val(cov), val(sh_rest)));
  return RasterizeFn::apply(means3D, means2D, sh, colors, opac, scales, rot, cov, sh_rest, bg, view, proj, campos, H, W,
                            tanfovx, tanfovy, scale_modifier, D, prefiltered, capacity, count_hint, count_slot);
}

struct L1SsimLossFn : public torch::autograd::Function<L1SsimLossFn> {
  static variable_list forward(AutogradContext* ctx, Tensor img1, Tensor img2, double lambda_dssim) {
    TORCH_CHECK(g_abi.bound, "mi355gs torch binding: bind() has not been called");
    HostClock clock(&g_host_us[2]);
    const Tensor a = f32c(img1, "img1", img1), b = f32c(img2, "img2", a);
    TORCH_CHECK(a.dim() == 4 && a.sizes() == b.sizes(), "fused_ssim expects two [B,C,H,W] tensors of equal shape");
    const int B = (int)a.size(0), C = (int)a.size(1), H = (int)a.size(2), W = (int)a.size(3);
    const DeviceScope dev(a);
    Tensor scratch = empty_bytes(g_abi.ssim_scratch_bytes(B, C, H, W), a);
    Tensor out = at::empty({2}, a.options());
    Tensor loss = at::empty({}, a.options());
    Tensor grad = at::empty_like(a);
    check(g_abi.l1_ssim_loss_fused(dev.stream, B, C, H, W, fp(a), fp(b), scratch.data_ptr(), (float)lambda_dssim, fp(out), fp(out) + 1,
                                   fp(loss), fp(grad)),
          "l1_ssim_loss_fused");
    ctx->save_for_backward({grad});
    ctx->mark_non_differentiable({out});
    ctx->set_materialize_grads(false);
    return {loss, out};
  }
  static variable_list backward(AutogradContext* ctx, variable_list grad_out) {
    HostClock clock(&g_host_us[3]);
    Tensor none;
    if (!grad_out[0].defined()) return {none, none, none};
    const auto saved = ctx->get_saved_variables();
    return {saved[0] * grad_out[0], none, none};
  }
};

std::vector<Tensor> l1_ssim_loss(Tensor img1, Tensor img2, double lambda_dssim) { return L1SsimLossFn::apply(img1, img2, lambda_dssim); }

struct L1LossFn : public torch::autograd::Function<L1LossFn> {
  static Tensor forward(AutogradContext* ctx, Tensor a_, Tensor b_) {
    TORCH_CHECK(g_abi.bound, "mi355gs torch binding: bind() has not been called");
    const Tensor a = f32c(a_, "network_output", a_), b = f32c(b_, "gt", a);
    TORCH_CHECK(a.sizes() == b.sizes() && a.numel() > 0, "l1_loss expects two non-empty tensors of equal shape");
    const DeviceScope dev(a);
    Tensor scratch = empty_bytes(g_abi.l1_scratch_bytes(a.numel()), a);
    Tensor out = at::empty({}, a.options());
    check(g_abi.l1_loss_forward(dev.stream, a.numel(), fp(a), fp(b), scratch.data_ptr(), fp(out)), "l1_loss_forward");
    ctx->save_for_backward({a, b});
    return out;
  }
  static variable_list backward(AutogradContext* ctx, variable_list grad_out) {
    const auto saved = ctx->get_saved_variables();
    const Tensor &a = saved[0], &b = saved[1];
    const Tensor g = f32c(grad_out[0], "grad", a);
    const DeviceScope dev(a);
    Tensor d = at::empty_like(a);
    check(g_abi.l1_loss_backward(dev.stream, a.numel(), fp(a), fp(b), fp(g), fp(d)), "l1_loss_backward");
    return {d, Tensor()};
  }
};

Tensor l1_loss(Tensor a, Tensor b) { return L1LossFn::apply(a, b); }

std::vector<Tensor> loss_pair_forward(Tensor img1, Tensor img2) {
  TORCH_CHECK(g_abi.bound, "mi355gs torch binding: bind() has not been called");
  HostClock clock(&g_host_us[2]);
  const Tensor a = f32c(img1, "img1", img1), b = f32c(img2, "img2", a);
  TORCH_CHECK((a.dim() == 3 || a.dim() == 4) && a.sizes() == b.sizes() && a.numel() > 0, "the loss pair expects two [C,H,W] or [B,C,H,W] tensors of equal shape");
  const int64_t o = a.dim() == 4 ? 1 : 0;
  const int B = o ? (int)a.size(0) : 1, C = (int)a.size(o), H = (int)a.size(o + 1), W = (int)a.size(o + 2);
  const DeviceScope dev(a);
  Tensor scratch = empty_bytes(g_abi.ssim_scratch_bytes(B, C, H, W), a);
  Tensor means = at::empty({2}, a.options());
  Tensor dmap = at::empty_like(a);
  check(g_abi.pair_forward(dev.stream, B, C, H, W, fp(a), fp(b), scratch.data_ptr(), fp(dmap)), "l1_ssim_pair_forward");
  return {means, scratch, dmap, a, b};
}

struct LossAffineFn : public torch::autograd::Function<LossAffineFn> {
  static Tensor forward(AutogradContext* ctx, Tensor image, Tensor a, Tensor b, Tensor dmap, Tensor means, Tensor scratch,
                        std::vector<int64_t> ops, std::vector<double> consts, double c_l1, double c_ssim, Tensor host_slot, double ticket,
                        c10::optional<Tensor> unit_grad_) {
    const Tensor unit_grad = unit_grad_.has_value() ? *unit_grad_ : Tensor();
    TORCH_CHECK(g_abi.bound, "mi355gs torch binding: bind() has not been called");
    TORCH_CHECK(ops.size() == consts.size() && !ops.empty() && ops.size() <= MI355GS_LOSS_PROGRAM_MAX, "loss_affine: 1..16 operations");
    TORCH_CHECK(image.numel() == a.numel() && means.numel() == 2, "loss_affine: image and its contiguous copy differ in size");
    const int64_t o = a.dim() == 4 ? 1 : 0;
    const int B = o ? (int)a.size(0) : 1, C = (int)a.size(o), H = (int)a.size(o + 1), W = (int)a.size(o + 2);
    const DeviceScope dev(a);
    int32_t op32[MI355GS_LOSS_PROGRAM_MAX]; float k32[MI355GS_LOSS_PROGRAM_MAX];
    for (size_t i = 0; i < ops.size(); ++i) { op32[i] = (int32_t)ops[i]; k32[i] = (float)consts[i]; }
    Tensor out = at::empty({}, a.options());
    float* host_out = nullptr;
    if (host_slot.defined() && host_slot.numel() >= 2) {
      TORCH_CHECK(host_slot.scalar_type() == at::kFloat && !host_slot.is_cuda() && host_slot.is_contiguous(), "loss_affine: the host slot is float32[2] host memory");
      host_out = host_slot.data_ptr<float>();
    }
    Tensor d;
    const bool with_grad = unit_grad.defined() && unit_grad.numel() == 1;
    if (with_grad) {
      d = at::empty_like(a);
      check(g_abi.program_eval_grad(dev.stream, (int)ops.size(), op32, k32, B, C, H, W, scratch.data_ptr(), fp(means) + 1, fp(means), fp(out), host_out,
                                    (float)ticket, fp(a), fp(b), fp(dmap), (float)c_l1, (float)c_ssim, fp(d)),
            "loss_program_eval_grad");
    } else {
      check(g_abi.program_eval(dev.stream, (int)ops.size(), op32, k32, B, C, H, W, scratch.data_ptr(), fp(means) + 1, fp(means), fp(out), host_out,
                               (float)ticket),
            "loss_program_eval");
    }
    ctx->save_for_backward({a, b, dmap, with_grad ? d : Tensor()});
    ctx->saved_data["c"] = std::vector<double>{c_l1, c_ssim};
    ctx->saved_data["shape"] = image.sizes().vec();
    ctx->saved_data["unit_grad_ptr"] = with_grad ? (int64_t)(uintptr_t)unit_grad.data_ptr() : (int64_t)0;
    return out;
  }
  static variable_list backward(AutogradContext* ctx, variable_list grad_out) {
    HostClock clock(&g_host_us[3]);
    const auto saved = ctx->get_saved_variables();
    const Tensor &a = saved[0], &b = saved[1], &dmap = saved[2];
    const auto c = ctx->saved_data["c"].toDoubleVector();
    Tensor none;
    const int64_t unit_ptr = ctx->saved_data["unit_grad_ptr"].toInt();
    if (unit_ptr != 0 && saved.size() > 3 && saved[3].defined() && (int64_t)(uintptr_t)grad_out[0].data_ptr() == unit_ptr) {
      return {saved[3].view(ctx->saved_data["shape"].toIntVector()), none, none, none, none, none, none, none, none, none, none, none, none};
    }
    const Tensor g = f32c(grad_out[0].reshape({1}), "grad", a);
    const DeviceScope dev(a);
    Tensor d = at::empty_like(a);
    check(g_abi.pair_backward(dev.stream, a.numel(), fp(a), fp(b), fp(dmap), fp(g), (float)c[0], fp(g), (float)c[1], fp(d)), "l1_ssim_pair_backward");
    return {d.view(ctx->saved_data["shape"].toIntVector()), none, none, none, none, none, none, none, none, none, none, none, none};
  }
};

Tensor loss_affine(Tensor image, Tensor a, Tensor b, Tensor dmap, Tensor means, Tensor scratch, std::vector<int64_t> ops,
                   std::vector<double> consts, double c_l1, double c_ssim, Tensor host_slot, double ticket) {
  return LossAffineFn::apply(image, a, b, dmap, means, scratch, ops, consts, c_l1, c_ssim, host_slot, ticket, c10::optional<Tensor>());
}

py::object wait_for_loss(Tensor host_slot, double ticket, int64_t timeout_us) {
  TORCH_CHECK(host_slot.scalar_type() == at::kFloat && !host_slot.is_cuda() && host_slot.numel() >= 2, "wait_for_loss: float32[2] host memory");
  const volatile float* w = host_slot.data_ptr<float>();
  const float want = (float)ticket;
  auto taken_over = [want](float have) {
    if (have == 0.f || have == want) return false;
    float ahead = have - want;
    if (ahead < 0.f) ahead += 16000000.f;
// ... 239 lines not shown
```

Baseline: 3544.

## Fold tile prefix scan into binning scatter kernel and add whole-frame forward entry

The separate scan_tiles launch is skipped when deferred scan is on, which is the default unless deterministic mode is set. The tile-count prefix scan, histogram ordering and segment metadata are instead computed inside the binning kernel via a shared scan body. A new posed_forward_frame entry runs projection and render in one ABI call, and the torch binding uses it for speculative capacity. This removes a kernel launch and a global round trip of tile starts, at the cost of heavier binning blocks and possible redundant per-block scan work. Histogram buckets also grow from the thread count to 1024.

After: 3578 (median of 5 runs). No clear change (+1.0%).

```diff
diff --git a/include/mi355gs.h b/include/mi355gs.h
--- a/include/mi355gs.h
+++ b/include/mi355gs.h
@@ -60,6 +60,9 @@
 int mi355gs_tune_min_units(int min_units);
 
 int mi355gs_tune_deterministic(int on);
+
+int mi355gs_tune_scan_rider(int mode);
+int mi355gs_raster_scan_rider(int W, int H);
 
 int mi355gs_tune_scale_grad(int mode);
 
@@ -129,6 +132,12 @@
                                      const float* rotation, const float* pose, const float* view_identity, const float* projmatrix,
                                      const float* origin, float tanfovx, float tanfovy, int32_t* radii, void* geom, void* tiles,
                                      int32_t* num_rendered, uint8_t* visible, void* grad_scratch, int debug);
+int mi355gs_posed_forward_frame(void* stream, int P, int D, int W, int H, const float* xyz, const float* f_dc, const float* f_rest,
+                                const float* opacity_logit, const float* log_scales, float scale_modifier, const float* rotation,
+                                const float* pose, const float* view_identity, const float* projmatrix, const float* origin,
+                                float tanfovx, float tanfovy, int32_t* radii, void* geom, void* tiles, int32_t* num_rendered,
+                                uint8_t* visible, void* grad_scratch, int64_t capacity, const float* bg, void* binning,
+                                float* out_color, int train, int debug);
 int mi355gs_posed_backward(void* stream, int P, int D, int W, int H, const float* bg, const float* xyz, const float* f_dc,
                            const float* f_rest, const float* opacity_logit, const float* log_scales, float scale_modifier,
                            const float* rotation, const float* pose, const float* view_identity, const float* projmatrix,
diff --git a/instantsplat_amd/_lib.py b/instantsplat_amd/_lib.py
--- a/instantsplat_amd/_lib.py
+++ b/instantsplat_amd/_lib.py
@@ -33,6 +33,8 @@
     "mi355gs_tune_min_units": (c_int, [c_int]),
     "mi355gs_tune_scale_grad": (c_int, [c_int]),
     "mi355gs_tune_deterministic": (c_int, [c_int]),
+    "mi355gs_tune_scan_rider": (c_int, [c_int]),
+    "mi355gs_raster_scan_rider": (c_int, [c_int, c_int]),
     "mi355gs_profile_begin": (c_int, []),
     "mi355gs_profile_set_period": (c_int, [c_int]),
     "mi355gs_profile_work_counters": (c_int, [_P]),
@@ -57,6 +59,8 @@
     "mi355gs_pose_backward": (c_int, [_P, c_int, _P, _P, _P, _P, _P, _P, _P, _P, _P, _P, _P, _P, _P, _P, _P]),
     "mi355gs_posed_forward_preprocess": (c_int, [_P, c_int, c_int, c_int, c_int, _P, _P, _P, _P, _P, c_float, _P, _P, _P, _P, _P,
                                                  c_float, c_float, _P, _P, _P, _P, _P, _P, c_int]),
+    "mi355gs_posed_forward_frame": (c_int, [_P, c_int, c_int, c_int, c_int, _P, _P, _P, _P, _P, c_float, _P, _P, _P, _P, _P,
+                                            c_float, c_float, _P, _P, _P, _P, _P, _P, c_int64, _P, _P, _P, c_int, c_int]),
     "mi355gs_posed_backward": (c_int, [_P, c_int, c_int, c_int, c_int, _P, _P, _P, _P, _P, _P, c_float, _P, _P, _P, _P, _P, c_float,
                                        c_float, _P, _P, _P, c_int64, _P, _P, _P, _P, _P, _P, _P, _P, _P, _P, _P, _P, _P, c_int, c_int, c_int, c_int]),
     "mi355gs_l1_scratch_bytes": (c_size_t, [c_int64]),
diff --git a/instantsplat_amd/csrc/api.hip b/instantsplat_amd/csrc/api.hip
--- a/instantsplat_amd/csrc/api.hip
+++ b/instantsplat_amd/csrc/api.hip
@@ -12,8 +12,9 @@
                              float*, float*, float*, float*, float*, float*, float*, const GsPosed&, float*, bool);
 int gs_launch_mark_visible(hipStream_t, int, const float*, const float*, uint8_t*);
 int gs_launch_scan_tiles(hipStream_t, int, const uint32_t*, uint32_t*, int32_t*, uint32_t*, uint32_t*, uint32_t*, uint32_t*, int);
-int gs_launch_binning(hipStream_t, int, int, int, const float*, const uint2*, const uint32_t*, uint32_t*, uint64_t*, uint32_t*, uint32_t,
-                      const uint32_t*, const uint32_t*, const uint32_t*);
+int gs_launch_binning(hipStream_t, int, int, int, const float*, const uint2*, uint32_t*, uint32_t*, uint64_t*, uint32_t*, uint32_t,
+                      const uint32_t*, const uint32_t*, const uint32_t*, const GsDeferredScan*);
+bool gs_scan_rides_in_scatter(int T);
 int gs_launch_composite_fwd(hipStream_t, int, int, int, int, uint32_t, const uint32_t*, const uint32_t*, const GsRec*, const float*,
                             float*, float*, uint32_t*, const uint32_t*, const uint32_t*, const uint32_t*, uint4*, float4*, uint32_t,
                             const uint32_t*, unsigned long long*, uint32_t, uint32_t*, unsigned long long*, bool);
@@ -89,6 +90,8 @@
 static int g_scale_grad_exact = 0;
 static int g_deterministic = 0;
 GsKnobs gs_knobs() { return GsKnobs{gs_min_units(), g_deterministic}; }
+static int g_scan_rider = 1;
+bool gs_defer_scan(const GsKnobs& knobs) { return g_scan_rider == 2 || (g_scan_rider == 1 && !knobs.det); }
 
 static CamParams make_cam(const float* view, const float* proj, const float* campos, float tanfovx, float tanfovy,
                           float scale_modifier, int W, int H) {
@@ -157,6 +160,7 @@
   gs_launch_count_tiles(stream, P, tl.T, tl.gx, (const uint2*)(g + gl.rect), (uint32_t*)(t + tl.count), (uint32_t*)(g + gl.bin_entries),
                         (uint32_t*)(g + gl.bin_n));
   GS_CHECK_LAUNCH("count_tiles");
+  if (cx.defer_scan) return MI355GS_OK;
   GS_KRANGE("scan_tiles");
   gs_launch_scan_tiles(stream, tl.T, (const uint32_t*)(t + tl.count), (uint32_t*)(t + tl.start), num_rendered,
                        (uint32_t*)(t + tl.order), (uint32_t*)(t + tl.meta), (uint32_t*)(t + tl.seg_first), (uint32_t*)(t + tl.part_first),
@@ -166,7 +170,7 @@
 }
 
 int gs_frame_render(hipStream_t stream, int P, const GsView& vw, const GsFrameBufs& fb, const float* bg, float* out_color, bool train,
-                    int debug) {
+                    int debug, const GsFrameCtx& cx, int32_t* num_rendered) {
   GsRange range(train ? "mi355gs_raster_forward_render" : "mi355gs_raster_forward_render_only");
   const int W = vw.W, H = vw.H;
   if (P < 0 || W <= 0 || H <= 0 || !fb.geom || !fb.tiles || !bg || !out_color) return MI355GS_EINVAL;
@@ -178,11 +182,18 @@
   const char* g = (const char*)fb.geom;
   char* t = (char*)fb.tiles;
   char* b = (char*)fb.binning;
+  if (cx.defer_scan && !num_rendered) return MI355GS_EINVAL;
+  const GsDeferredScan scan = {(const uint32_t*)(t + tl.count), num_rendered, (uint32_t*)(t + tl.order), (uint32_t*)(t + tl.meta),
+                               (uint32_t*)(t + tl.seg_first), (uint32_t*)(t + tl.part_first), fb.knobs.min_units};
+  if (cx.defer_scan && g_ranges_on) {
+    gs_range_push("scan_tiles");
+    gs_range_pop();
+  }
   GS_KRANGE("binning");
   gs_launch_binning(stream, P, tl.T, tl.gx, (const float*)(g + gl.depth), (const uint2*)(g + gl.rect),
-                    (const uint32_t*)(t + tl.start), (uint32_t*)(t + tl.cursor), (uint64_t*)(b + bl.keys),
+                    (uint32_t*)(t + tl.start), (uint32_t*)(t + tl.cursor), (uint64_t*)(b + bl.keys),
                     (uint32_t*)(b + bl.list), cap, (const uint32_t*)(t + tl.order), (const uint32_t*)(g + gl.bin_entries),
-                    (const uint32_t*)(g + gl.bin_n));
+                    (const uint32_t*)(g + gl.bin_n), cx.defer_scan ? &scan : nullptr);
   GS_CHECK_LAUNCH("binning");
   {
     ProfScope prof(train ? 0 : 2, stream);
@@ -330,6 +341,14 @@
   return old;
 }
 
+int mi355gs_tune_scan_rider(int mode) {
+  const int old = g_scan_rider;
+  if (mode >= 0 && mode <= 2) g_scan_rider = mode;
+  return old;
+}
+
+int mi355gs_raster_scan_rider(int W, int H) { return (W > 0 && H > 0 && gs_scan_rides_in_scatter(TilesLayout(W, H).T)) ? 1 : 0; }
+
 int mi355gs_tune_scale_grad(int mode) {
   const int old = g_scale_grad_exact;
   if (mode >= 0) g_scale_grad_exact = mode ? 1 : 0;
diff --git a/instantsplat_amd/csrc/binning.hip b/instantsplat_amd/csrc/binning.hip
--- a/instantsplat_amd/csrc/binning.hip
+++ b/instantsplat_amd/csrc/binning.hip
@@ -16,29 +16,42 @@
 #endif
 constexpr int SCAN_PER_MAX = (int)(SCAN_STAGE_MAX_BYTES / (SCAN_THREADS * 4));
 
-template <bool STAGED>
-__global__ __launch_bounds__(SCAN_THREADS) void k_scan_tiles(int T, const uint32_t* count, uint32_t* start, int32_t* num_rendered,
-                                                               uint32_t* __restrict__ order, uint32_t* __restrict__ meta,
-                                                               uint32_t* __restrict__ seg_first, uint32_t* __restrict__ part_first,
-                                                               uint32_t min_units) {
-  __shared__ uint32_t wave_tot[SCAN_THREADS / GS_WAVE];
-  HIP_DYNAMIC_SHARED(uint32_t, s_stage)
+constexpr int SCAN_BUCKETS = 1024;
+
+struct ScanLds {
+  uint32_t hist[SCAN_BUCKETS];
+  uint32_t wave[4][SCAN_THREADS / GS_WAVE];
+  uint32_t max;
+};
+
+template <int NT, int PER_MAX>
+__device__ __forceinline__ void scan_tiles_body(int T, const uint32_t* count, uint32_t* start, int32_t* num_rendered,
+                                                uint32_t* __restrict__ order, uint32_t* __restrict__ meta,
+                                                uint32_t* __restrict__ seg_first, uint32_t* __restrict__ part_first,
+                                                uint32_t min_units, uint32_t* s_stage, ScanLds& sh) {
+  constexpr bool STAGED = PER_MAX > 0, IN_LDS = PER_MAX < 0;
+  constexpr int NW = NT / GS_WAVE, HB = SCAN_BUCKETS / NT;
+  static_assert(NT % GS_WAVE == 0 && NW <= SCAN_THREADS / GS_WAVE && SCAN_BUCKETS % NT == 0, "workgroup size of the tile scan");
   const int tid = threadIdx.x, lane = tid & 63, wave = tid >> 6;
-  const int per = (T + SCAN_THREADS - 1) / SCAN_THREADS;
-  const int lo = tid * per, hi = min(T, lo + per);
+  const int per = (T + NT - 1) / NT | (IN_LDS ? 1 : 0);
+  const int lo = min(T, tid * per), hi = min(T, lo + per);
   SCAN_STAMP(0);
-  uint32_t own[STAGED ? SCAN_PER_MAX : 1];
+  uint32_t own[STAGED ? PER_MAX : 1];
+  if constexpr (STAGED || IN_LDS) {
+    for (int e = tid; e < T; e += NT) s_stage[e] = count[e];
+    __syncthreads();
+  }
   if constexpr (STAGED) {
-    for (int e = tid; e < T; e += SCAN_THREADS) s_stage[e] = count[e];
-    __syncthreads();
-#pragma unroll
-    for (int k = 0; k < SCAN_PER_MAX; ++k) own[k] = lo + k < hi ? s_stage[lo + k] : 0u;
+#pragma unroll
+    for (int k = 0; k < PER_MAX; ++k) own[k] = lo + k < hi ? s_stage[lo + k] : 0u;
   }
   auto for_own = [&](auto&& f) {
     if constexpr (STAGED) {
 #pragma unroll
-      for (int k = 0; k < SCAN_PER_MAX; ++k)
+      for (int k = 0; k < PER_MAX; ++k)
         if (lo + k < hi) f(lo + k, own[k]);
+    } else if constexpr (IN_LDS) {
+      for (int i = lo; i < hi; ++i) f(i, s_stage[i]);
     } else {
       for (int i = lo; i < hi; ++i) f(i, count[i]);
     }
@@ -48,61 +61,66 @@
       __syncthreads();
       for_own([&](int i, uint32_t c) { s_stage[i] = value(i, c); });
       __syncthreads();
-      for (int e = tid; e < T; e += SCAN_THREADS) out[e] = s_stage[e];
+      for (int e = tid; e < T; e += NT) out[e] = s_stage[e];
     } else {
       for_own([&](int i, uint32_t c) { out[i] = value(i, c); });
+    }
+  };
+  auto across_waves = [&](int row, uint32_t wave_incl, uint32_t& off, uint32_t& tot) {
+    if (lane == 63) sh.wave[row][wave] = wave_incl;
+    __syncthreads();
+    off = 0; tot = 0;
+#pragma unroll
+    for (int w = 0; w < NW; ++w) {
+      const uint32_t v = sh.wave[row][w];
+      if (w < wave) off += v;
+      tot += v;
     }
   };
   SCAN_STAMP(1);
   uint32_t local = 0;
   for_own([&](int, uint32_t c) { local += c; });
   const uint32_t incl = gs_wave_scan_incl_u32(local);
-  if (lane == 63) wave_tot[wave] = incl;
-  __syncthreads();
-  uint32_t wave_off = 0, total = 0;
-#pragma unroll
-  for (int w = 0; w < SCAN_THREADS / GS_WAVE; ++w) {
-    const uint32_t v = wave_tot[w];
-    if (w < wave) wave_off += v;
-    total += v;
+  uint32_t wave_off, total;
+  across_waves(0, incl, wave_off, total);
+  if (tid == 0) {
+    *num_rendered = (int32_t)total;
+    start[T] = total;
   }
   SCAN_STAMP(2);
   if (order) {
-    __shared__ uint32_t hist[SCAN_THREADS];
-    __shared__ uint32_t s_max;
     uint32_t mx = 0;
     for_own([&](int, uint32_t c) { mx = max(mx, c); });
     mx = gs_wave_max_u32(mx);
-    hist[tid] = 0u;
-    if (tid == 0) s_max = 0u;
-    __syncthreads();
-    if (lane == 0) atomicMax(&s_max, mx);
-    __syncthreads();
-    const uint32_t cmax = max(s_max, 1u);
-    const float bscale = (float)(SCAN_THREADS - 1) / (float)cmax;
-    auto bucket = [&](uint32_t c) { return (uint32_t)(SCAN_THREADS - 1) - min((uint32_t)(SCAN_THREADS - 1), (uint32_t)((float)c * bscale)); };
+    for (int b = tid; b < SCAN_BUCKETS; b += NT) sh.hist[b] = 0u;
+    if (tid == 0) sh.max = 0u;
+    __syncthreads();
+    if (lane == 0) atomicMax(&sh.max, mx);
+    __syncthreads();
+    const uint32_t cmax = max(sh.max, 1u);
+    const float bscale = (float)(SCAN_BUCKETS - 1) / (float)cmax;
+    auto bucket = [&](uint32_t c) { return (uint32_t)(SCAN_BUCKETS - 1) - min((uint32_t)(SCAN_BUCKETS - 1), (uint32_t)((float)c * bscale)); };
     SCAN_STAMP(3);
-    for_own([&](int, uint32_t c) { atomicAdd(&hist[bucket(c)], 1u); });
+    for_own([&](int, uint32_t c) { atomicAdd(&sh.hist[bucket(c)], 1u); });
     __syncthreads();
     SCAN_STAMP(4);
-    const uint32_t h = hist[tid];
-    const uint32_t hi_ = gs_wave_scan_incl_u32(h);
-    __shared__ uint32_t hist_wave[SCAN_THREADS / GS_WAVE];
-    if (lane == 63) hist_wave[wave] = hi_;
-    __syncthreads();
-    uint32_t hoff = 0;
-#pragma unroll
-    for (int w = 0; w < SCAN_THREADS / GS_WAVE; ++w)
-      if (w < wave) hoff += hist_wave[w];
-    hist[tid] = hoff + hi_ - h;
+    uint32_t h[HB], hsum = 0;
+#pragma unroll
+    for (int k = 0; k < HB; ++k) { h[k] = sh.hist[tid * HB + k]; hsum += h[k]; }
+    const uint32_t hi_ = gs_wave_scan_incl_u32(hsum);
+    uint32_t hoff, htot;
+    across_waves(1, hi_, hoff, htot);
+    uint32_t hrun = hoff + hi_ - hsum;
+#pragma unroll
+    for (int k = 0; k < HB; ++k) { sh.hist[tid * HB + k] = hrun; hrun += h[k]; }
     __syncthreads();
     SCAN_STAMP(5);
     if constexpr (STAGED) {
-      for_own([&](int i, uint32_t c) { s_stage[atomicAdd(&hist[bucket(c)], 1u)] = (uint32_t)i; });
+      for_own([&](int i, uint32_t c) { s_stage[atomicAdd(&sh.hist[bucket(c)], 1u)] = (uint32_t)i; });
       __syncthreads();
-      for (int e = tid; e < T; e += SCAN_THREADS) order[e] = s_stage[e];
+      for (int e = tid; e < T; e += NT) order[e] = s_stage[e];
     } else {
-      for_own([&](int i, uint32_t c) { order[atomicAdd(&hist[bucket(c)], 1u)] = (uint32_t)i; });
+      for_own([&](int i, uint32_t c) { order[atomicAdd(&sh.hist[bucket(c)], 1u)] = (uint32_t)i; });
     }
     __syncthreads();
     SCAN_STAMP(6);
@@ -118,16 +136,9 @@
     uint32_t lseg = 0, lpart = 0;
     for_own([&](int, uint32_t c) { lseg += units_of(c); lpart += short_of(c); });
     const uint32_t iseg = gs_wave_scan_incl_u32(lseg), ipart = gs_wave_scan_incl_u32(lpart);
-    __shared__ uint32_t seg_wave[SCAN_THREADS / GS_WAVE];
-    __shared__ uint32_t part_wave[SCAN_THREADS / GS_WAVE];
-    if (lane == 63) { seg_wave[wave] = iseg; part_wave[wave] = ipart; }
-    __syncthreads();
-    uint32_t soff = 0, stot = 0, poff = 0, ptot = 0;
-#pragma unroll
-    for (int w = 0; w < SCAN_THREADS / GS_WAVE; ++w) {
-      if (w < wave) { soff += seg_wave[w]; poff += part_wave[w]; }
-      stot += seg_wave[w]; ptot += part_wave[w];
-    }
+    uint32_t soff, stot, poff, ptot;
+    across_waves(2, iseg, soff, stot);
+    across_waves(3, ipart, poff, ptot);
     uint32_t srun = soff + iseg - lseg, prun = poff + ipart - lpart;
     emit(seg_first, [&](int, uint32_t c) { const uint32_t v = srun; srun += units_of(c); return v; });
     emit(part_first, [&](int, uint32_t c) { const uint32_t v = prun; prun += short_of(c); return v; });
@@ -137,11 +148,18 @@
   SCAN_STAMP(7);
   uint32_t run = wave_off + incl - local;
   emit(start, [&](int, uint32_t c) { const uint32_t v = run; run += c; return v; });
-  if (tid == 0) {
-    start[T] = total;
-    *num_rendered = (int32_t)total;
-  }
   SCAN_STAMP(8);
+}
+
+template <bool STAGED>
+__global__ __launch_bounds__(SCAN_THREADS) void k_scan_tiles(int T, const uint32_t* count, uint32_t* start, int32_t* num_rendered,
+                                                               uint32_t* __restrict__ order, uint32_t* __restrict__ meta,
+                                                               uint32_t* __restrict__ seg_first, uint32_t* __restrict__ part_first,
+                                                               uint32_t min_units) {
+  __shared__ ScanLds sh;
+  HIP_DYNAMIC_SHARED(uint32_t, s_stage)
+  scan_tiles_body<SCAN_THREADS, STAGED ? SCAN_PER_MAX : 0>(T, count, start, num_rendered, order, meta, seg_first, part_first, min_units,
+                                                            s_stage, sh);
 }
 
 constexpr int SCAN_CHUNK = 4096;
@@ -286,16 +304,82 @@
   }
 }
 
+__device__ __forceinline__ void scatter_prefix_in_place(uint32_t* bins, int T, uint32_t* s_wave) {
+  const int tid = threadIdx.x, lane = tid & 63, wave = tid >> 6;
+  const int per = ((T + 255) / 256) | 1;
+  const int lo = min(T, tid * per), hi = min(T, lo + per);
+  __syncthreads();
+  uint32_t sum = 0;
+  for (int i = lo; i < hi; ++i) sum += bins[i];
+  const uint32_t incl = gs_wave_scan_incl_u32(sum);
+  if (lane == 63) s_wave[wave] = incl;
+  __syncthreads();
+  uint32_t run = incl - sum;
+#pragma unroll
+  for (int w = 0; w < 4; ++w) run += w < wave ? s_wave[w] : 0u;
+  for (int i = lo; i < hi; ++i) { const uint32_t c = bins[i]; bins[i] = run; run += c; }
+  __syncthreads();
+}
+
+__device__ __forceinline__ void scatter_add_prefix(uint32_t* bins, int T, const uint32_t* __restrict__ tile_count, uint32_t* s_wave) {
+  const int tid = threadIdx.x, lane = tid & 63, wave = tid >> 6;
+  uint32_t base = 0;
+  for (int t0 = 0; t0 < T; t0 += 1024) {
+    uint32_t c[4], sum = 0;
+#pragma unroll
+    for (int j = 0; j < 4; ++j) {
+      const int t = t0 + 4 * tid + j;
+      c[j] = t < T ? tile_count[t] : 0u;
+      sum += c[j];
+    }
+    const uint32_t incl = gs_wave_scan_incl_u32(sum);
+    __syncthreads();
+    if (lane == 63) s_wave[wave] = incl;
+    __syncthreads();
+    uint32_t run = base + incl - sum;
+#pragma unroll
+    for (int w = 0; w < 4; ++w) {
+      run += w < wave ? s_wave[w] : 0u;
+      base += s_wave[w];
+    }
+#pragma unroll
+    for (int j = 0; j < 4; ++j) {
+      const int t = t0 + 4 * tid + j;
+      if (t < T) bins[t] += run;
+      run += c[j];
+    }
+  }
+}
+
+struct ScanRider {
+  int32_t* num_rendered;
+  uint32_t *order, *meta, *seg_first, *part_first;
+  uint32_t min_units;
+};
+
+template <int RIDER>
 __global__ __launch_bounds__(256) void k_scatter_lds(int P, int T, int gx, const float* __restrict__ depths,
-                                                      const uint2* __restrict__ rects, const uint32_t* __restrict__ start,
+                                                      const uint2* __restrict__ rects, uint32_t* start,
                                                       uint32_t* __restrict__ cursor, uint64_t* __restrict__ keys, uint32_t capacity,
-                                                      const uint32_t* __restrict__ entries, const uint32_t* __restrict__ entry_n) {
+                                                      const uint32_t* __restrict__ entries, const uint32_t* __restrict__ entry_n,
+                                                      const uint32_t* tile_count, ScanRider rider) {
   HIP_DYNAMIC_SHARED(uint32_t, s_bins)
-  __shared__ uint32_t s_wide[BIN_CHUNK];
-  __shared__ uint2 s_wide_rect[BIN_CHUNK];
+  struct WideQueue { uint32_t index[BIN_CHUNK]; uint2 rect[BIN_CHUNK]; };
+  __shared__ union Lds { WideQueue wide; ScanLds scan; } s_lds;
   __shared__ uint32_t s_nwide;
+  __shared__ uint32_t s_wave_tot[4];
+  uint32_t* const s_wide = s_lds.wide.index;
+  uint2* const s_wide_rect = s_lds.wide.rect;
   const int tid = threadIdx.x;
-  const int lo = blockIdx.x * BIN_CHUNK, hi = min(P, lo + BIN_CHUNK);
+  if constexpr (RIDER != 0) {
+    if (blockIdx.x == 0) {
+      scan_tiles_body<256, (RIDER > 0 ? RIDER : RIDER == -2 ? -1 : 0)>(T, tile_count, start, rider.num_rendered, rider.order, rider.meta, rider.seg_first,
+                                                     rider.part_first, rider.min_units, s_bins, s_lds.scan);
+      return;
+    }
+  }
+  const int wg = (int)blockIdx.x - (RIDER != 0 ? 1 : 0);
+  const int lo = wg * BIN_CHUNK, hi = min(P, lo + BIN_CHUNK);
   uint2 own[BIN_PER_THREAD];
   uint32_t own_depth[BIN_PER_THREAD];
 #pragma unroll
@@ -304,26 +388,40 @@
     own[j] = rects[ic];
     own_depth[j] = __float_as_uint(depths[ic]);
   }
-  const uint32_t n_entries = entry_n[blockIdx.x];
+  const uint32_t n_entries = entry_n[wg];
+  const uint32_t* mine = entries + (size_t)wg * GS_BIN_ENTRIES;
+  static_assert(GS_BIN_ENTRIES == 1024, "a workgroup's entry list is one round of four entries per thread");
+  if constexpr (RIDER != 0) {
+#pragma unroll 8
+    for (int t = tid; t < T; t += 256) s_bins[t] = tile_count[t];
+  }
   if (n_entries != 0xffffffffu) {
-    const uint32_t* mine = entries + (size_t)blockIdx.x * GS_BIN_ENTRIES;
-    for (uint32_t e0 = 0; e0 < n_entries; e0 += 1024) {
-      uint32_t en[4], r[4], st[4];
-#pragma unroll
-      for (int j = 0; j < 4; ++j) {
-        const uint32_t e = e0 + tid + 256 * j;
-        en[j] = e < n_entries ? mine[e] : 0u;
+    uint32_t en[4], r[4], st[4];
+#pragma unroll
+    for (int j = 0; j < 4; ++j) {
+      const uint32_t e = tid + 256 * j;
+      en[j] = e < n_entries ? mine[e] : 0u;
+    }
+#pragma unroll
+    for (int j = 0; j < 4; ++j) {
+      r[j] = 0u; st[j] = 0u;
+      if (en[j]) {
+        r[j] = atomicAdd(&cursor[en[j] & 0xffffu], en[j] >> 16);
+        if constexpr (RIDER == 0) st[j] = start[en[j] & 0xffffu];
       }
-#pragma unroll
-      for (int j = 0; j < 4; ++j) {
-        r[j] = 0u; st[j] = 0u;
-        if (en[j]) { r[j] = atomicAdd(&cursor[en[j] & 0xffffu], en[j] >> 16); st[j] = start[en[j] & 0xffffu]; }
-      }
+    }
+    if constexpr (RIDER != 0) {
+      scatter_prefix_in_place(s_bins, T, s_wave_tot);
+#pragma unroll
+      for (int j = 0; j < 4; ++j)
+        if (en[j]) s_bins[en[j] & 0xffffu] += r[j];
+    } else {
 #pragma unroll
       for (int j = 0; j < 4; ++j)
         if (en[j]) s_bins[en[j] & 0xffffu] = st[j] + r[j];
     }
   } else {
+    __syncthreads();
     for (int t = tid; t < T; t += 256) s_bins[t] = 0;
     if (tid == 0) s_nwide = 0;
     __syncthreads();
@@ -340,11 +438,21 @@
       for (int j = 0; j < 4; ++j) {
         const int t = t0 + tid + 256 * j;
         r[j] = 0u; st[j] = 0u;
-        if (c[j]) { r[j] = atomicAdd(&cursor[t], c[j]); st[j] = start[t]; }
+        if (c[j]) {
+          r[j] = atomicAdd(&cursor[t], c[j]);
+          if constexpr (RIDER == 0) st[j] = start[t];
+        }
       }
 #pragma unroll
-      for (int j = 0; j < 4; ++j)
-        if (c[j]) s_bins[t0 + tid + 256 * j] = st[j] + r[j];
+      for (int j = 0; j < 4; ++j) {
+        const int t = t0 + tid + 256 * j;
+        if constexpr (RIDER != 0) { if (t < T) s_bins[t] = r[j]; }
+        else if (c[j]) s_bins[t] = st[j] + r[j];
+      }
+    }
+    if constexpr (RIDER != 0) {
+      __syncthreads();
+      scatter_add_prefix(s_bins, T, tile_count, s_wave_tot);
     }
   }
   if (tid == 0) s_nwide = 0;
@@ -674,18 +782,39 @@
   return 0;
 }
 
-int gs_launch_binning(hipStream_t stream, int P, int T, int gx, const float* depths, const uint2* rects, const uint32_t* start,
+bool gs_scan_rides_in_scatter(int T) { return T > 0 && T <= BIN_MAX_LDS_TILES; }
+
+int gs_launch_binning(hipStream_t stream, int P, int T, int gx, const float* depths, const uint2* rects, uint32_t* start,
                       uint32_t* cursor, uint64_t* keys, uint32_t* list, uint32_t capacity, const uint32_t* order, const uint32_t* entries,
-                      const uint32_t* entry_n) {
+                      const uint32_t* entry_n, const GsDeferredScan* scan) {
+  bool ride = false;
+  if (scan) {
+    ride = P > 0 && capacity != 0 && gs_scan_rides_in_scatter(T);
+    if (!ride)
+      gs_launch_scan_tiles(stream, T, scan->count, start, scan->num_rendered, scan->order, scan->meta, scan->seg_first, scan->part_first,
+                           scan->min_units);
+  }
   if (P <= 0 || capacity == 0) return 0;
-  if (T <= BIN_MAX_LDS_TILES)
-    hipLaunchKernelGGL(k_scatter_lds, dim3((P + BIN_CHUNK - 1) / BIN_CHUNK), dim3(256), (size_t)T * 4, stream, P, T, gx, depths, rects,
-                       start, cursor, keys, capacity, entries, entry_n);
+  const int nwg = (P + BIN_CHUNK - 1) / BIN_CHUNK;
+  if (ride) {
+    const ScanRider rider = {scan->num_rendered, scan->order, scan->meta, scan->seg_first, scan->part_first, (uint32_t)scan->min_units};
+    auto launch = [&](auto kernel) {
+      hipLaunchKernelGGL(kernel, dim3(nwg + 1), dim3(256), (size_t)T * 4, stream, P, T, gx, depths, rects, start, cursor, keys, capacity,
+                         entries, entry_n, scan->count, rider);
+    };
+    if (T <= 256) launch(k_scatter_lds<-1>);
+    else if (T <= 256 * 4) launch(k_scatter_lds<4>);
+    else if (T <= 256 * 16) launch(k_scatter_lds<16>);
+    else launch(k_scatter_lds<-2>);
+  } else if (T <= BIN_MAX_LDS_TILES)
+    hipLaunchKernelGGL(k_scatter_lds<0>, dim3(nwg), dim3(256), (size_t)T * 4, stream, P, T, gx, depths, rects, start, cursor, keys,
+                       capacity, entries, entry_n, (const uint32_t*)nullptr, ScanRider{});
   else
-    hipLaunchKernelGGL(k_scatter_direct, dim3((P + 255) / 256), dim3(256), 0, stream, P, gx, depths, rects, start, cursor, keys, capacity);
+    hipLaunchKernelGGL(k_scatter_direct, dim3((P + 255) / 256), dim3(256), 0, stream, P, gx, depths, rects, (const uint32_t*)start, cursor,
+                       keys, capacity);
   {
     GsProfScope prof(4, stream);
-    hipLaunchKernelGGL(k_sort_tiles, dim3(T), dim3(SORT_THREADS), 0, stream, T, start, keys, list, capacity, order);
+    hipLaunchKernelGGL(k_sort_tiles, dim3(T), dim3(SORT_THREADS), 0, stream, T, (const uint32_t*)start, keys, list, capacity, order);
   }
   return 0;
 }
diff --git a/instantsplat_amd/csrc/common.h b/instantsplat_amd/csrc/common.h
--- a/instantsplat_amd/csrc/common.h
+++ b/instantsplat_amd/csrc/common.h
@@ -334,6 +334,12 @@
   float* gate = nullptr;
   bool gate_tail = false;
   bool pose_only = false;
+  bool defer_scan = false;
+};
+struct GsDeferredScan {
+  const uint32_t* count; int32_t* num_rendered;
+  uint32_t *order, *meta, *seg_first, *part_first;
+  int min_units;
 };
 struct GsGradOut { float *means3D, *means2D, *shs, *shs_rest, *colors, *opacities, *scales, *rotations, *cov3D; };
 static inline size_t gs_grad_gate_offset(int P) { return gs_align((size_t)(P > 0 ? P : 1) * sizeof(GsGrad)); }
@@ -349,7 +355,8 @@
 int gs_frame_project(hipStream_t stream, const GsScene& sc, const GsView& vw, const GsFrameBufs& fb, const GsFrameCtx& cx,
                      int32_t* num_rendered, uint8_t* visible, int debug);
 int gs_frame_render(hipStream_t stream, int P, const GsView& vw, const GsFrameBufs& fb, const float* bg, float* out_color, bool train,
-                    int debug);
+                    int debug, const GsFrameCtx& cx = GsFrameCtx(), int32_t* num_rendered = nullptr);
+bool gs_defer_scan(const GsKnobs& knobs);
 int gs_frame_backward(hipStream_t stream, const GsScene& sc, const GsView& vw, const GsFrameBufs& fb, const GsFrameCtx& cx,
                       const float* bg, const float* out_color, const float* dL_dpix, const GsGradOut& out, bool grad_scratch_is_clear,
                       int debug);
diff --git a/instantsplat_amd/csrc/trainer.hip b/instantsplat_amd/csrc/trainer.hip
--- a/instantsplat_amd/csrc/trainer.hip
+++ b/instantsplat_amd/csrc/trainer.hip
@@ -88,6 +88,26 @@
                           cx, num_rendered, visible, debug);
 }
 
+int mi355gs_posed_forward_frame(void* stream, int P, int D, int W, int H, const float* xyz, const float* f_dc, const float* f_rest,
+                                const float* opacity_logit, const float* log_scales, float scale_modifier, const float* rotation,
+                                const float* pose, const float* view_identity, const float* projmatrix, const float* origin,
+                                float tanfovx, float tanfovy, int32_t* radii, void* geom, void* tiles, int32_t* num_rendered,
+                                uint8_t* visible, void* grad_scratch, int64_t capacity, const float* bg, void* binning,
+                                float* out_color, int train, int debug) {
+  GS_RANGE();
+  if (!pose || D < 0 || D > 3 || (D > 0 && !f_rest)) return MI355GS_EINVAL;
+  const GsKnobs knobs = gs_knobs();
+  GsFrameCtx cx;
+  cx.posed.pose = pose;
+  cx.defer_scan = gs_defer_scan(knobs);
+  const GsView vw = {W, H, view_identity, projmatrix, origin, tanfovx, tanfovy};
+  const GsFrameBufs bufs = {geom, tiles, binning, capacity, radii, grad_scratch, knobs};
+  if (int rc = gs_frame_project((hipStream_t)stream, posed_scene(P, D, xyz, f_dc, f_rest, opacity_logit, log_scales, scale_modifier, rotation),
+                                vw, bufs, cx, num_rendered, visible, debug))
+    return rc;
+  return gs_frame_render((hipStream_t)stream, P, vw, bufs, bg, out_color, train != 0, debug, cx, num_rendered);
+}
+
 int mi355gs_posed_backward(void* stream_, int P, int D, int W, int H, const float* bg, const float* xyz, const float* f_dc,
                            const float* f_rest, const float* opacity_logit, const float* log_scales, float scale_modifier,
                            const float* rotation, const float* pose, const float* view_identity, const float* projmatrix,
@@ -186,13 +206,14 @@
   cx.prologue = &pro;
   cx.posed.pose = pose; cx.posed.acc = t->pose_scratch; cx.posed.partial = t->pose_partial;
   cx.gate = t->adam_scratch;
+  cx.defer_scan = gs_defer_scan(t->knobs);
   const int D = sh_degree;
   const GsScene scene = posed_scene(P, D, t->xyz, t->f_dc, t->f_rest, t->opacity, t->scaling, 1.0f, t->rotation);
   const GsView vw = {W, H, t->consts, projmatrix, t->consts + 16, tanfovx, tanfovy};
   const GsFrameBufs bufs = {t->geom, t->tiles, t->binning, t->capacity, t->radii, t->grad_scratch, t->knobs};
   int rc;
   if ((rc = gs_frame_project(stream, scene, vw, bufs, cx, num_rendered_out, nullptr, 0))) return rc;
-  if ((rc = gs_frame_render(stream, P, vw, bufs, bg, t->image, true, 0))) return rc;
+  if ((rc = gs_frame_render(stream, P, vw, bufs, bg, t->image, true, 0, cx, num_rendered_out))) return rc;
   if ((rc = gs_loss_fused(stream, 3, H, W, t->image, gt_image, lambda_dssim, t->dL_dimg, t->ssim_scratch))) return rc;
   const GsGradOut o = {t->g_xyz, t->g_means2D, t->g_fdc, D == 0 ? nullptr : t->g_frest, t->g_colors, t->g_opacity, t->g_scaling, t->g_rot, nullptr};
   if ((rc = gs_frame_backward(stream, scene, vw, bufs, cx, bg, t->image, t->dL_dimg, o, false, 0))) return rc;
diff --git a/instantsplat_amd/csrc_torch/binding.cpp b/instantsplat_amd/csrc_torch/binding.cpp
--- a/instantsplat_amd/csrc_torch/binding.cpp
+++ b/instantsplat_amd/csrc_torch/binding.cpp
@@ -3,6 +3,7 @@
 #include <c10/hip/HIPStream.h>
 
 #include <chrono>
+#include <functional>
 #include <optional>
 #include <map>
 #include <mutex>
@@ -22,6 +23,7 @@
   X(grad_scratch_bytes, mi355gs_raster_grad_scratch_bytes)             \
   X(grad_gate_offset, mi355gs_raster_grad_gate_offset)                 \
   X(posed_forward_preprocess, mi355gs_posed_forward_preprocess)        \
+  X(posed_forward_frame, mi355gs_posed_forward_frame)                  \
   X(forward_preprocess, mi355gs_raster_forward_preprocess)             \
   X(raster_backward, mi355gs_raster_backward)                          \
   X(forward_render, mi355gs_raster_forward_render)                     \
@@ -268,9 +270,10 @@
     radii = at::empty({P}, like.options().dtype(at::kInt));
   }
 
+  using WholeFrame = std::function<void(const FrameForward&, bool)>;
   template <class Project>
   void run(const DeviceScope& dev, const Tensor& like, int P, int W, int H, const Tensor& bg, int64_t capacity, int64_t count_hint,
-           const Project& project) {
+           const Project& project, const WholeFrame& whole_frame = nullptr) {
     color = at::empty({3, H, W}, like.options());
     geom = empty_bytes(g_abi.geom_bytes(P), like);
     tiles = empty_bytes(g_abi.tiles_bytes(W, H), like);
@@ -290,14 +293,25 @@
               "raster_forward_render_only");
       }
     };
-    preprocess();
+    auto speculate = [&](int64_t cap) {
+      if (!whole_frame) {
+        preprocess();
+        stage2(cap);
+        return;
+      }
+      *reinterpret_cast<volatile int32_t*>(count) = -1;
+      binning = empty_bytes(t_backward_follows ? g_abi.binning_bytes(cap, W, H) : g_abi.binning_bytes_render_only(cap, W, H), like);
+      R = cap;
+      whole_frame(*this, t_backward_follows);
+    };
     R = capacity;
     if (R >= 0) {
-      stage2(R);
+      speculate(R);
       return;
     }
     const int64_t guess = count_hint > 0 ? count_hint + count_hint / 2 + 16384 : -1;
-    if (guess > 0) stage2(guess);
+    if (guess > 0) speculate(guess);
+    else preprocess();
     {
       HostClock wait_clock(&g_host_us[5]);
       wait_for_count(count, dev, like);
@@ -348,6 +362,14 @@
                                            P > 0 ? reinterpret_cast<uint8_t*>(visible.data_ptr<bool>()) : nullptr,
                                            frame.scratch.defined() ? frame.scratch.data_ptr() : nullptr, 0),
             "posed_forward_preprocess");
+    }, [&](const FrameForward& frame, bool train) {
+      check(g_abi.posed_forward_frame(dev.stream, P, (int)D, (int)W, (int)H, fp(xyz), fp(f_dc), fp(f_rest), fp(opl), fp(scaling),
+                                      (float)scale_modifier, fp(rot), fp(pose), fp(view), fp(proj), fp(origin), (float)tanfovx,
+                                      (float)tanfovy, frame.radii.data_ptr<int32_t>(), frame.geom.data_ptr(), frame.tiles.data_ptr(), frame.count,
+                                      P > 0 ? reinterpret_cast<uint8_t*>(visible.data_ptr<bool>()) : nullptr,
+                                      frame.scratch.defined() ? frame.scratch.data_ptr() : nullptr, frame.R, fp(bg), frame.binning.data_ptr(),
+                                      fp(frame.color), train ? 1 : 0, 0),
+            "posed_forward_frame");
     });
     ctx->saved_data["dims"] = std::vector<int64_t>{P, D, W, H, f.R};
     ctx->saved_data["scalars"] = std::vector<double>{tanfovx, tanfovy, scale_modifier};
```
